# 1275468127/Medical-SAM2

Measured on AMD Instinct MI355X. Metric: slices/sec @1024^2 (Hiera-S), higher is better.
Workload: dtype bf16; 1 GPU; configs[1]: sam2_hiera_s 2D (train_2d SAM2 sub-sequence, forward), b=4 x 1024x1024 per GPU, 16-entry memory bank with 4 sampled memories per slice, one click per slice; forward_image -> memory_attention -> prompt encoder -> mask decoder -> memory encoder; hip_graph=True, weights=random name-keyed init

## Files before the change

### include/msam2_hip.h

```cpp
#ifndef MSAM2_HIP_H
#define MSAM2_HIP_H

#include <stddef.h>
#include <stdint.h>

#ifdef __cplusplus
extern "C" {
#endif

const char* msam2_last_error(void);

int msam2_version(void);

int msam2_operand_is_fp16(void);

int msam2_graph_begin(void* stream);

int msam2_graph_end(void* stream, void** graph_exec_out);

int msam2_graph_launch(void* graph_exec, void* stream);

int msam2_graph_destroy(void* graph_exec);

int msam2_event_create(void** ev);

int msam2_event_record(void* ev, void* stream);

int msam2_event_elapsed_ms(void* start, void* stop, float* ms);

int msam2_event_destroy(void* ev);

int msam2_gemm_nt(const void* A, int64_t lda, const void* B, int64_t ldb, const float* bias, const void* residual, int64_t ldr, void* C, int64_t ldc, int out_is_16bit, int64_t M, int64_t N, int64_t K, void* stream);

int msam2_gemm(const void* A, int64_t lda, const void* W, int64_t ldw, const float* bias, const float* colscale, const void* residual, int64_t ldr, int res_is_16bit, int64_t res_mod, void* C, int64_t ldc, int out_is_16bit, int64_t M, int64_t N, int64_t K, int act, void* stream);

int msam2_gemm_tokens(const float* A, int64_t lda, const float* A2, int64_t add_cols, const void* W, int64_t ldw, const float* bias, const float* residual, int64_t ldr, void* C, int64_t ldc, int out_is_16bit, int64_t M, int64_t N, int64_t K, int act, void* stream);

int msam2_gemm_pool2x2(const void* A, int64_t lda, const void* W, int64_t ldw, const float* bias, float* C, int64_t ldc, int64_t B, int64_t H, int64_t Wimg, int64_t N, int64_t K, void* stream);

int msam2_gemm_qkv_pool2x2(const void* A, int64_t lda, const void* W, int64_t ldw, const float* bias, void* QKV, int64_t ldc, void* Q2, int64_t ldq, int64_t B, int64_t H, int64_t Wimg, int64_t N, int64_t K, int64_t q_cols, void* stream);

int msam2_gemm_rope(const void* A, int64_t lda, const void* W, int64_t ldw, const float* bias, void* C, int64_t ldc, int64_t M, int64_t N, int64_t K, const float* rope_cos, const float* rope_sin, int64_t rope_cols, int64_t head_dim, int64_t rows_per_batch, int64_t n_rope, int64_t n_pos, void* stream);

size_t msam2_attention_workspace_bytes(int64_t Bz, int64_t H, int64_t Lq, int64_t D, int splits);

int msam2_attention_merge(void* o, const int64_t* o_strides, int64_t B, int64_t H, int64_t Lq, int64_t Lk, int64_t D, int splits, void* workspace, size_t workspace_bytes, void* stream);

int msam2_attention_fwd(const void* q, const int64_t* q_strides, const void* k, const int64_t* k_strides, const void* v, const int64_t* v_strides, void* o, const int64_t* o_strides, int64_t B, int64_t H, int64_t Lq, int64_t Lk, int64_t D, float scale, int splits, void* workspace, size_t workspace_bytes, void* stream);

int msam2_attention_fwd_lse(const void* q, const int64_t* q_strides, const void* k, const int64_t* k_strides, const void* v, const int64_t* v_strides, void* o, const int64_t* o_strides, int64_t B, int64_t H, int64_t Lq, int64_t Lk, int64_t D, float scale, int splits, void* workspace, size_t workspace_bytes, float* lse, void* stream);

int msam2_attention_fwd_lse_dropout(const void* q, const int64_t* q_strides, const void* k, const int64_t* k_strides, const void* v, const int64_t* v_strides, void* o, const int64_t* o_strides, int64_t B, int64_t H, int64_t Lq, int64_t Lk, int64_t D, float scale, int splits, void* workspace, size_t workspace_bytes, float* lse, float p, uint64_t seed, uint64_t offset, const void* seed_dev, void* stream);

int msam2_attention_kv64_fwd(const void* q, const int64_t* q_strides, const void* k, const int64_t* k_strides, const void* v, const int64_t* v_strides, void* o, const int64_t* o_strides, int64_t B, int64_t H, int64_t Lq, int64_t Lk, float scale, int splits, void* workspace, size_t workspace_bytes, void* stream);

int msam2_attention_effective_splits(int64_t Lk, int splits);

int msam2_attention_kv64_partial(const void* q, const int64_t* q_strides, const void* k, const int64_t* k_strides, const void* v, const int64_t* v_strides, int64_t B, int64_t H, int64_t Lq, int64_t Lk, float scale, int splits, int split_begin, int split_count, void* workspace, size_t workspace_bytes, void* stream);

int msam2_attention_kv64_dyn_fwd(const void* q, const int64_t* q_strides, const void* k, const int64_t* k_strides, const void* v, const int64_t* v_strides, void* o, const int64_t* o_strides, int64_t B, int64_t H, int64_t Lq, int64_t Lk, const void* key_count_dev, float scale, int splits, void* workspace, size_t workspace_bytes, void* stream);

int msam2_attention_kv64_dyn_partial(const void* q, const int64_t* q_strides, const void* k, const int64_t* k_strides, const void* v, const int64_t* v_strides, int64_t B, int64_t H, int64_t Lq, int64_t Lk, const void* key_count_dev, float scale, int splits, int split_begin, int split_count, void* workspace, size_t workspace_bytes, void* stream);

int msam2_window_attention_fwd(const void* q, int64_t q_token_stride, int64_t q_head_stride, int64_t hq, int64_t wq, int64_t ws_q, const void* k, const void* v, int64_t kv_token_stride, int64_t kv_head_stride, int64_t hk, int64_t wk, int64_t ws_k, const float* kpad, const float* vpad, void* o, int64_t o_token_stride, int64_t o_head_stride, int64_t B, int64_t H, int64_t D, float scale, void* stream);

int msam2_attention_small_fwd(const void* q, int64_t q_bs, int64_t q_ts, const void* k, int64_t k_bs, int64_t k_ts, const void* v, int64_t v_bs, int64_t v_ts, void* o, int64_t o_bs, int64_t o_ts, int64_t B, int64_t H, int64_t Lq, int64_t Lk, int64_t D, float scale, void* stream);

size_t msam2_attention_bwd_workspace_bytes(int64_t B, int64_t H, int64_t Lq, int64_t D);

int msam2_attention_bwd(const void* q, const int64_t* q_strides, const void* k, const int64_t* k_strides, const void* v, const int64_t* v_strides, const void* o, const int64_t* o_strides, const float* lse, const float* d_o, const int64_t* do_strides, float* dq, const int64_t* dq_strides, float* dk, const int64_t* dk_strides, float* dv, const int64_t* dv_strides, void* workspace, size_t workspace_bytes, int64_t B, int64_t H, int64_t Lq, int64_t Lk, int64_t D, float scale, void* stream);

int msam2_attention_bwd_dropout(const void* q, const int64_t* q_strides, const void* k, const int64_t* k_strides, const void* v, const int64_t* v_strides, const void* o, const int64_t* o_strides, const float* lse, const float* d_o, const int64_t* do_strides, float* dq, const int64_t* dq_strides, float* dk, const int64_t* dk_strides, float* dv, const int64_t* dv_strides, void* workspace, size_t workspace_bytes, int64_t B, int64_t H, int64_t Lq, int64_t Lk, int64_t D, float scale, float p, uint64_t seed, uint64_t offset, const void* seed_dev, void* stream);

int msam2_layernorm(const void* x, int in_is_16bit, int64_t ldx, const float* weight, const float* bias, void* y, int out_is_16bit, int64_t ldy, int64_t rows, int64_t C, float eps, int act, void* stream);

int msam2_layernorm_dual(const float* x, int64_t ldx, const float* weight, const float* bias, float* y, int64_t ldy, void* y16, int64_t ldy16, int64_t rows, int64_t C, float eps, void* stream);

int msam2_add_cast(const void* a, int a_is_16bit, int64_t a_s0, int64_t a_s1, const void* b, int b_is_16bit, int64_t b_s0, int64_t b_s1, float alpha, void* out, int out_is_16bit, int64_t D0, int64_t D1, int64_t C, void* stream);

int msam2_maxpool2x2(const void* x, int in_is_16bit, int64_t ldx, void* y, int out_is_16bit, int64_t ldy, int64_t B, int64_t H, int64_t W, int64_t C, void* stream);

int msam2_upsample2x_add(void* y, const void* top, int64_t B, int64_t H, int64_t W, int64_t C, void* stream);

int msam2_rope_table(float* cos_out, float* sin_out, int64_t side, int64_t D, float theta, void* stream);

int msam2_rope_inplace(void* x, int64_t batch_stride, int64_t ld, int64_t B, int64_t L, int64_t n_rope, int64_t n_pos, int64_t D, const float* cos_t, const float* sin_t, void* stream);

int msam2_bilinear_upsample(const float* x, float* y, int64_t planes, int64_t h, int64_t w, int64_t H, int64_t W, void* stream);

int msam2_sine_pos_2d(float* out, int64_t h, int64_t w, int64_t C, float temperature, void* stream);

int msam2_fourier_pe_grid(float* out, const float* gauss, int64_t h, int64_t w, int64_t C, void* stream);

int msam2_hiera_pos_embed(float* out, const float* pos_embed, const float* pos_embed_window, int64_t C, int64_t bh, int64_t bw, int64_t h, int64_t w, int64_t window, void* stream);

int msam2_aa_downsample(const float* x, float* y, int64_t planes, int64_t H, int64_t W, int64_t factor, float in_scale, float in_bias, void* stream);

int msam2_gate_rows(float* x, const float* score, float value, int64_t B, int64_t row_len, void* stream);

int msam2_any_positive(const float* x, float* out, int64_t B, int64_t row_len, void* stream);

int msam2_image_prep(const uint8_t* img_hwc, float* out_chw, int64_t H, int64_t W, int64_t S, const float* mean3, const float* std3, void* stream);

int msam2_non_overlap(const float* masks, float* out, int64_t n_obj, int64_t pixels, void* stream);

int msam2_seg_counts(const float* pred, const float* gt, const float* thresholds, int64_t n_thresholds, int64_t planes, int64_t pixels, int* counts, void* stream);

int msam2_im2col_patch7x7s4(const float* img, void* out, int64_t B, int64_t S, void* stream);

int msam2_patch_embed7x7s4(const float* img, const void* w_perm, const float* bias, const float* pos, float* out, int64_t B, int64_t S, int64_t E, void* stream);

int msam2_im2col3x3s2(const void* x, void* out, int64_t B, int64_t H, int64_t W, int64_t C, int64_t ld, void* stream);

int msam2_conv3x3s2_ln_gelu(const void* x, int in_is_16bit, const float* weight, const float* bias, const float* ln_w, const float* ln_b, void* y, int64_t B, int64_t H, int64_t W, int64_t Cin, int64_t Cout, int mask_mode, float mask_scale, float mask_bias, void* stream);

int msam2_dwconv7x7_ln(const float* x, const float* weight_tap_major, const float* bias, const float* ln_w, const float* ln_b, void* y, int64_t B, int64_t H, int64_t W, int64_t C, void* stream);

int msam2_convt2x2_shuffle(const void* gemm_out, const float* bias, const void* skip, const float* ln_w, const float* ln_b, void* y, int64_t B, int64_t h, int64_t w, int64_t C, void* stream);

int msam2_convt2x2_shuffle_f32skip(const void* gemm_out, const float* bias, const float* skip, const float* ln_w, const float* ln_b, void* y, int64_t B, int64_t h, int64_t w, int64_t C, void* stream);

int msam2_convt2x2_shuffle_shared(const void* gemm_out, const float* bias, const void* skip, int skip_is_16bit, const float* ln_w, const float* ln_b, void* y, int64_t B, int64_t h, int64_t w, int64_t C, int64_t skip_batch_stride, void* stream);

int msam2_hyper_masks(const float* hyper, const void* upscaled, float* masks, int64_t n, int64_t K, int64_t P, int64_t C, void* stream);

int msam2_prompt_points(const float* xy, const int* labels, const float* gauss, const float* point_emb, const float* not_a_point, float* out, int64_t n_points, int64_t C, float image_size, void* stream);

int msam2_prompt_points_padded(const float* xy, const int* labels, const float* gauss, const float* point_emb, const float* not_a_point, float* out, int64_t n_sets, int64_t P, int64_t n_pad, int64_t C, float image_size, void* stream);

int msam2_select_mask(const float* masks, const float* ious, const float* obj_scores, float* low_res, int* sel, float* iou_sel, int64_t n, int64_t P, int multimask, int dynamic_stability, float delta, float thresh, void* stream);

int msam2_gather_rows(const float* x, const int* sel, float* y, int64_t n, int64_t T, int64_t C, int64_t offset, void* stream);

int msam2_obj_ptr_mix(float* ptr, const float* obj_scores, const float* no_obj_ptr, int64_t n, int64_t C, void* stream);

int msam2_space_to_depth(const void* x, int in_is_16bit, void* out, int64_t B, int64_t H, int64_t W, int64_t C, int64_t k, int64_t ld, void* stream);

int msam2_token_mlp3(const float* hs, int64_t hs_batch_stride, int64_t hs_token_stride, const int* token_index, const void* w1, const float* b1, const void* w2, const float* b2, const void* w3, const float* b3, const int* out_dim, const int* sigmoid_flag, float* out, int64_t G, int64_t B, int64_t C, void* stream);

int msam2_token_mlp3_packed(const float* hs, int64_t hs_batch_stride, int64_t hs_token_stride, const int* token_index, const void* w1, const float* b1, const void* w2, const float* b2, const void* w3, const float* b3, const int* out_dim, const int* sigmoid_flag, float* out, const int* out_offset, const int* out_stride, int64_t G, int64_t B, int64_t C, void* stream);

size_t msam2_cc_workspace_bytes(int64_t N, int64_t H, int64_t W);

int msam2_cc_label(const uint8_t* img, int32_t* labels, int32_t* counts, int64_t N, int64_t H, int64_t W, void* workspace, size_t workspace_bytes, void* stream);

size_t msam2_fill_holes_workspace_bytes(int64_t N, int64_t H, int64_t W);

int msam2_fill_components(float* mask, int64_t N, int64_t H, int64_t W, int max_area, float threshold, int above, float fill_value, void* workspace, size_t workspace_bytes, void* stream);

int msam2_fill_holes(float* mask, int64_t N, int64_t H, int64_t W, int max_area, void* workspace, size_t workspace_bytes, void* stream);

int msam2_transpose16(const void* in, int64_t ldi, void* out, int64_t ldo, int64_t rows, int64_t cols, void* stream);

int msam2_gemm_tt(const void* A, int64_t lda, const void* B, int64_t ldb, float* C, int64_t ldc, float* a_colsum, int64_t M, int64_t N, int64_t K, void* stream);

int msam2_gemm_tt_acc(const void* A, int64_t lda, const void* B, int64_t ldb, float* C, int64_t ldc, float* a_colsum, int64_t M, int64_t N, int64_t K, void* stream);

int msam2_colsum(const void* x, int x_is_16bit, int64_t ldx, float* out, int64_t rows, int64_t cols, void* stream);

int msam2_act_bwd(const void* pre, int pre_is_16bit, const void* dy, int dy_is_16bit, void* out, int64_t n, int act, void* stream);

int msam2_layernorm_bwd(const float* x, int64_t ldx, const void* dy, int dy_is_16bit, int64_t ldd, const float* gamma, float* dx, int64_t ldo, float* dgamma, float* dbeta, int64_t rows, int64_t C, float eps, const float* add, int64_t ld_add, void* stream);

int msam2_softmax_rows(const float* s, int64_t ld_s, void* p, int64_t ld_p, int64_t rows, int64_t cols, float scale, void* stream);

int msam2_softmax_bwd_rows(const void* p, int64_t ld_p, const float* dp, int64_t ld_dp, void* ds, int64_t ld_ds, int64_t rows, int64_t cols, float scale, void* stream);

int msam2_convt2x2_gather(const void* gemm_out, const float* bias, const void* skip, float* z, int64_t B, int64_t h, int64_t w, int64_t C, void* stream);

int msam2_convt2x2_scatter_grad(const void* dz, int dz_is_16bit, void* dg, int64_t B, int64_t h, int64_t w, int64_t C, void* stream);

int msam2_dwconv7x7(const float* x, const float* w_tap_major, const float* bias, float* y, int64_t B, int64_t H, int64_t W, int64_t C, int flip, void* stream);

int msam2_dwconv7x7_wgrad(const float* x, const float* dy, float* dw_tap_major, int64_t B, int64_t H, int64_t W, int64_t C, void* stream);

int msam2_col2im3x3s2(const float* dcols, int64_t ld, float* dx, int64_t B, int64_t H, int64_t W, int64_t C, void* stream);

int msam2_bilinear_upsample_bwd(const float* dy, float* dx, int64_t planes, int64_t h, int64_t w, int64_t H, int64_t W, void* stream);

int msam2_bce_logits(const float* logits, const float* target, float* dlogits, float* loss, int64_t n, float pos_weight, void* stream);

int msam2_adam_step(float* param, const float* grad, float* exp_avg, float* exp_avg_sq, int64_t n, float lr, float beta1, float beta2, float eps, int64_t step, void* stream);

int msam2_adam_step_multi(void* const* params, const void* const* grads, void* const* exp_avg, void* const* exp_avg_sq, const int64_t* numel, int64_t count, float lr, float beta1, float beta2, float eps, int64_t step, float grad_scale, float weight_decay, void* step_counter, void* skipped_counter, void* stream);

int msam2_attention_small_bwd(const void* q, int64_t q_bs, int64_t q_ts, const void* k, int64_t k_bs, int64_t k_ts, const void* v, int64_t v_bs, int64_t v_ts, const float* d_o, float* dq, float* dk, float* dv, int64_t B, int64_t H, int64_t Lq, int64_t Lk, int64_t D, float scale, void* stream);

int msam2_maxpool2x2_bwd(const void* x, int x_is_16bit, int64_t ldx, const float* dy, int64_t lddy, float* dx, int64_t lddx, int64_t B, int64_t H, int64_t W, int64_t C, void* stream);

int msam2_window_move(void* img, int64_t ld_img, void* win, const void* fill, int64_t B, int64_t H, int64_t W, int64_t heads, int64_t D, int64_t ws, int elem_bytes, int to_windows, void* stream);

int msam2_window_unpartition_cvt(void* img16, int64_t ld_img, const float* win, int64_t B, int64_t H, int64_t W, int64_t heads, int64_t D, int64_t ws, void* stream);

int msam2_window_pad_colsum(const float* win, float* out, int64_t B, int64_t H, int64_t W, int64_t heads, int64_t D, int64_t ws, void* stream);

int msam2_sumpool2x2(const float* dy, float* out, int64_t B, int64_t H, int64_t W, int64_t C, void* stream);

size_t msam2_hiera_pos_embed_bwd_workspace_bytes(int64_t C, int64_t bw, int64_t h, int64_t window);

int msam2_hiera_pos_embed_bwd(const float* d_table, float* d_pos_embed, float* d_pos_embed_window, int64_t C, int64_t bh, int64_t bw, int64_t h, int64_t w, int64_t window, void* workspace, size_t workspace_bytes, void* stream);

int msam2_dropout(const void* x, int x_is_16bit, int64_t ldx, const float* residual, int64_t ldr, void* y, int y_is_16bit, int64_t ldy, int64_t rows, int64_t cols, float p, uint64_t seed, uint64_t offset, const void* seed_dev, void* stream);

int msam2_counter_bump(void* counter_u64, void* snapshot_u64, void* stream);

int msam2_mlp_fused_permute_w2(const void* w2, void* w2p, int64_t dim, int64_t hidden, void* stream);

int msam2_ln_mlp_residual_supported(int64_t dim);

int msam2_ln_mlp_residual_fwd(const float* x, int64_t T, int64_t dim, const float* ln_w, const float* ln_b, float eps, const void* w1, const float* b1, const void* w2p, const float* b2, float* out, void* stream);

int msam2_ln_mlp_residual_fwd_dual(const float* x, int64_t T, int64_t dim, const float* ln_w, const float* ln_b, float eps, const void* w1, const float* b1, const void* w2p, const float* b2, float* out, void* out16, void* stream);

size_t msam2_mask_stats_workspace_bytes(int64_t M);

int msam2_mask_stats(const float* logits, int64_t M, int64_t lh, int64_t lw, int64_t h, int64_t w, float thr, float thr_hi, float thr_lo, int* counts, int* boxes, void* workspace, size_t workspace_bytes, void* stream);

int msam2_mask_rle_runs(const float* logits, int64_t M, int64_t lh, int64_t lw, int64_t h, int64_t w, int64_t x0, int64_t y0, int64_t H, int64_t W, float thr, int* runs, void* stream);

int msam2_mask_rle(const float* logits, int64_t M, int64_t lh, int64_t lw, int64_t h, int64_t w, int64_t x0, int64_t y0, int64_t H, int64_t W, float thr, const int64_t* offsets, int* counts, void* stream);

size_t msam2_box_nms_workspace_bytes(int64_t K);

int msam2_box_nms(const float* boxes, const float* scores, int64_t K, float iou_thr, int64_t* keep, int* n_keep, void* workspace, size_t workspace_bytes, void* stream);

int msam2_bank_dots_chain(int64_t K, int vec);

size_t msam2_bank_dots_workspace_bytes(int64_t R, int64_t Cn);

int msam2_bank_dots(const float* x, const int64_t* x_strides, int64_t R, const float* ya, const int64_t* ya_strides, int64_t rows_a, const float* yb, const int64_t* yb_strides, int64_t rows_b, int64_t n_ch, int64_t n_px, float* dots, float* xx, float* yy, void* workspace, size_t workspace_bytes, void* stream);

// ... 37 lines not shown
```

### medical-sam2_amd/_lib.py

```python
from __future__ import annotations

import ctypes
import os
import subprocess

_HERE = os.path.dirname(os.path.abspath(__file__))
LIB_PATH = os.environ.get("MSAM2_LIB_PATH") or os.path.join(_HERE, "libmsam2_hip.so")

c_p = ctypes.c_void_p
c_i = ctypes.c_int
c_l = ctypes.c_int64
c_f = ctypes.c_float
c_z = ctypes.c_size_t
c_d = ctypes.c_double

SIGNATURES = {
    "msam2_version": (c_i, []),
    "msam2_last_error": (ctypes.c_char_p, []),
    "msam2_operand_is_fp16": (c_i, []),
    "msam2_gemm": (c_i, [c_p, c_l, c_p, c_l, c_p, c_p, c_p, c_l, c_i, c_l, c_p, c_l, c_i, c_l, c_l, c_l, c_i, c_p]),
    "msam2_gemm_pool2x2": (c_i, [c_p, c_l, c_p, c_l, c_p, c_p, c_l, c_l, c_l, c_l, c_l, c_l, c_p]),
    "msam2_gemm_qkv_pool2x2": (c_i, [c_p, c_l, c_p, c_l, c_p, c_p, c_l, c_p, c_l, c_l, c_l, c_l, c_l, c_l, c_l, c_p]),
    "msam2_gemm_tokens": (c_i, [c_p, c_l, c_p, c_l, c_p, c_l, c_p, c_p, c_l, c_p, c_l, c_i, c_l, c_l, c_l, c_i, c_p]),
    "msam2_gemm_rope": (c_i, [c_p, c_l, c_p, c_l, c_p, c_p, c_l, c_l, c_l, c_l, c_p, c_p, c_l, c_l, c_l, c_l, c_l, c_p]),
    "msam2_ln_mlp_residual_supported": (c_i, [c_l]),
    "msam2_mlp_fused_permute_w2": (c_i, [c_p, c_p, c_l, c_l, c_p]),
    "msam2_ln_mlp_residual_fwd": (c_i, [c_p, c_l, c_l, c_p, c_p, c_f, c_p, c_p, c_p, c_p, c_p, c_p]),
    "msam2_ln_mlp_residual_fwd_dual": (c_i, [c_p, c_l, c_l, c_p, c_p, c_f, c_p, c_p, c_p, c_p, c_p, c_p, c_p]),
    "msam2_layernorm": (c_i, [c_p, c_i, c_l, c_p, c_p, c_p, c_i, c_l, c_l, c_l, c_f, c_i, c_p]),
    "msam2_layernorm_dual": (c_i, [c_p, c_l, c_p, c_p, c_p, c_l, c_p, c_l, c_l, c_l, c_f, c_p]),
    "msam2_attention_workspace_bytes": (c_z, [c_l, c_l, c_l, c_l, c_i]),
    "msam2_attention_fwd": (c_i, [c_p, c_p, c_p, c_p, c_p, c_p, c_p, c_p, c_l, c_l, c_l, c_l, c_l, c_f, c_i, c_p, c_z, c_p]),
    "msam2_attention_fwd_lse": (c_i, [c_p, c_p, c_p, c_p, c_p, c_p, c_p, c_p, c_l, c_l, c_l, c_l, c_l, c_f, c_i, c_p, c_z, c_p, c_p]),
    "msam2_attention_fwd_lse_dropout": (c_i, [c_p, c_p, c_p, c_p, c_p, c_p, c_p, c_p, c_l, c_l, c_l, c_l, c_l, c_f, c_i, c_p, c_z, c_p, c_f,
                                              ctypes.c_uint64, ctypes.c_uint64, c_p, c_p]),
    "msam2_attention_kv64_fwd": (c_i, [c_p, c_p, c_p, c_p, c_p, c_p, c_p, c_p, c_l, c_l, c_l, c_l, c_f, c_i, c_p, c_z, c_p]),
    "msam2_attention_kv64_partial": (c_i, [c_p, c_p, c_p, c_p, c_p, c_p, c_l, c_l, c_l, c_l, c_f, c_i, c_i, c_i, c_p, c_z, c_p]),
    "msam2_attention_kv64_dyn_fwd": (c_i, [c_p, c_p, c_p, c_p, c_p, c_p, c_p, c_p, c_l, c_l, c_l, c_l, c_p, c_f, c_i, c_p, c_z, c_p]),
    "msam2_attention_kv64_dyn_partial": (c_i, [c_p, c_p, c_p, c_p, c_p, c_p, c_l, c_l, c_l, c_l, c_p, c_f, c_i, c_i, c_i, c_p, c_z, c_p]),
    "msam2_attention_effective_splits": (c_i, [c_l, c_i]),
    "msam2_attention_merge": (c_i, [c_p, c_p, c_l, c_l, c_l, c_l, c_l, c_i, c_p, c_z, c_p]),
    "msam2_window_attention_fwd": (c_i, [c_p, c_l, c_l, c_l, c_l, c_l, c_p, c_p, c_l, c_l, c_l, c_l, c_l, c_p, c_p, c_p, c_l, c_l,
                                         c_l, c_l, c_l, c_f, c_p]),
    "msam2_attention_small_fwd": (c_i, [c_p, c_l, c_l, c_p, c_l, c_l, c_p, c_l, c_l, c_p, c_l, c_l, c_l, c_l, c_l, c_l, c_l, c_f,
                                        c_p]),
    "msam2_add_cast": (c_i, [c_p, c_i, c_l, c_l, c_p, c_i, c_l, c_l, c_f, c_p, c_i, c_l, c_l, c_l, c_p]),
    "msam2_maxpool2x2": (c_i, [c_p, c_i, c_l, c_p, c_i, c_l, c_l, c_l, c_l, c_l, c_p]),
    "msam2_upsample2x_add": (c_i, [c_p, c_p, c_l, c_l, c_l, c_l, c_p]),
    "msam2_rope_table": (c_i, [c_p, c_p, c_l, c_l, c_f, c_p]),
    "msam2_rope_inplace": (c_i, [c_p, c_l, c_l, c_l, c_l, c_l, c_l, c_l, c_p, c_p, c_p]),
    "msam2_bilinear_upsample": (c_i, [c_p, c_p, c_l, c_l, c_l, c_l, c_l, c_p]),
    "msam2_sine_pos_2d": (c_i, [c_p, c_l, c_l, c_l, c_f, c_p]),
    "msam2_fourier_pe_grid": (c_i, [c_p, c_p, c_l, c_l, c_l, c_p]),
    "msam2_hiera_pos_embed": (c_i, [c_p, c_p, c_p, c_l, c_l, c_l, c_l, c_l, c_l, c_p]),
    "msam2_im2col_patch7x7s4": (c_i, [c_p, c_p, c_l, c_l, c_p]),
    "msam2_patch_embed7x7s4": (c_i, [c_p, c_p, c_p, c_p, c_p, c_l, c_l, c_l, c_p]),
    "msam2_im2col3x3s2": (c_i, [c_p, c_p, c_l, c_l, c_l, c_l, c_l, c_p]),
    "msam2_conv3x3s2_ln_gelu": (c_i, [c_p, c_i, c_p, c_p, c_p, c_p, c_p, c_l, c_l, c_l, c_l, c_l, c_i, c_f, c_f, c_p]),
    "msam2_dwconv7x7_ln": (c_i, [c_p, c_p, c_p, c_p, c_p, c_p, c_l, c_l, c_l, c_l, c_p]),
    "msam2_convt2x2_shuffle": (c_i, [c_p, c_p, c_p, c_p, c_p, c_p, c_l, c_l, c_l, c_l, c_p]),
    "msam2_convt2x2_shuffle_f32skip": (c_i, [c_p, c_p, c_p, c_p, c_p, c_p, c_l, c_l, c_l, c_l, c_p]),
    "msam2_space_to_depth": (c_i, [c_p, c_i, c_p, c_l, c_l, c_l, c_l, c_l, c_l, c_p]),
    "msam2_aa_downsample": (c_i, [c_p, c_p, c_l, c_l, c_l, c_l, c_f, c_f, c_p]),
    "msam2_gate_rows": (c_i, [c_p, c_p, c_f, c_l, c_l, c_p]),
    "msam2_any_positive": (c_i, [c_p, c_p, c_l, c_l, c_p]),
    "msam2_transpose16": (c_i, [c_p, c_l, c_p, c_l, c_l, c_l, c_p]),
    "msam2_colsum": (c_i, [c_p, c_i, c_l, c_p, c_l, c_l, c_p]),
    "msam2_act_bwd": (c_i, [c_p, c_i, c_p, c_i, c_p, c_l, c_i, c_p]),
    "msam2_layernorm_bwd": (c_i, [c_p, c_l, c_p, c_i, c_l, c_p, c_p, c_l, c_p, c_p, c_l, c_l, c_f, c_p, c_l, c_p]),
    "msam2_softmax_rows": (c_i, [c_p, c_l, c_p, c_l, c_l, c_l, c_f, c_p]),
    "msam2_softmax_bwd_rows": (c_i, [c_p, c_l, c_p, c_l, c_p, c_l, c_l, c_l, c_f, c_p]),
    "msam2_convt2x2_gather": (c_i, [c_p, c_p, c_p, c_p, c_l, c_l, c_l, c_l, c_p]),
    "msam2_convt2x2_scatter_grad": (c_i, [c_p, c_i, c_p, c_l, c_l, c_l, c_l, c_p]),
    "msam2_bce_logits": (c_i, [c_p, c_p, c_p, c_p, c_l, c_f, c_p]),
    "msam2_attention_bwd_workspace_bytes": (c_z, [c_l, c_l, c_l, c_l]),
    "msam2_attention_bwd": (c_i, [c_p, c_p, c_p, c_p, c_p, c_p, c_p, c_p, c_p, c_p, c_p, c_p, c_p, c_p, c_p, c_p, c_p, c_p, c_z,
                                  c_l, c_l, c_l, c_l, c_l, c_f, c_p]),
    "msam2_attention_bwd_dropout": (c_i, [c_p, c_p, c_p, c_p, c_p, c_p, c_p, c_p, c_p, c_p, c_p, c_p, c_p, c_p, c_p, c_p, c_p, c_p, c_z,
                                          c_l, c_l, c_l, c_l, c_l, c_f, c_f, ctypes.c_uint64, ctypes.c_uint64, c_p, c_p]),
    "msam2_dwconv7x7": (c_i, [c_p, c_p, c_p, c_p, c_l, c_l, c_l, c_l, c_i, c_p]),
    "msam2_dwconv7x7_wgrad": (c_i, [c_p, c_p, c_p, c_l, c_l, c_l, c_l, c_p]),
    "msam2_col2im3x3s2": (c_i, [c_p, c_l, c_p, c_l, c_l, c_l, c_l, c_p]),
    "msam2_gemm_nt": (c_i, [c_p, c_l, c_p, c_l, c_p, c_p, c_l, c_p, c_l, c_i, c_l, c_l, c_l, c_p]),
    "msam2_gemm_tt": (c_i, [c_p, c_l, c_p, c_l, c_p, c_l, c_p, c_l, c_l, c_l, c_p]),
    "msam2_window_unpartition_cvt": (c_i, [c_p, c_l, c_p, c_l, c_l, c_l, c_l, c_l, c_l, c_p]),
    "msam2_window_pad_colsum": (c_i, [c_p, c_p, c_l, c_l, c_l, c_l, c_l, c_l, c_p]),
    "msam2_gemm_tt_acc": (c_i, [c_p, c_l, c_p, c_l, c_p, c_l, c_p, c_l, c_l, c_l, c_p]),
    "msam2_bilinear_upsample_bwd": (c_i, [c_p, c_p, c_l, c_l, c_l, c_l, c_l, c_p]),
    "msam2_maxpool2x2_bwd": (c_i, [c_p, c_i, c_l, c_p, c_l, c_p, c_l, c_l, c_l, c_l, c_l, c_p]),
    "msam2_window_move": (c_i, [c_p, c_l, c_p, c_p, c_l, c_l, c_l, c_l, c_l, c_l, c_i, c_i, c_p]),
    "msam2_sumpool2x2": (c_i, [c_p, c_p, c_l, c_l, c_l, c_l, c_p]),
    "msam2_hiera_pos_embed_bwd": (c_i, [c_p, c_p, c_p, c_l, c_l, c_l, c_l, c_l, c_l, c_p, c_z, c_p]),
    "msam2_hiera_pos_embed_bwd_workspace_bytes": (c_z, [c_l, c_l, c_l, c_l]),
    "msam2_dropout": (c_i, [c_p, c_i, c_l, c_p, c_l, c_p, c_i, c_l, c_l, c_l, c_f, ctypes.c_uint64, ctypes.c_uint64, c_p, c_p]),
    "msam2_counter_bump": (c_i, [c_p, c_p, c_p]),
    "msam2_adam_step": (c_i, [c_p, c_p, c_p, c_p, c_l, c_f, c_f, c_f, c_f, c_l, c_p]),
    "msam2_adam_step_multi": (c_i, [c_p, c_p, c_p, c_p, c_p, c_l, c_f, c_f, c_f, c_f, c_l, c_f, c_f, c_p, c_p, c_p]),
    "msam2_attention_small_bwd": (c_i, [c_p, c_l, c_l, c_p, c_l, c_l, c_p, c_l, c_l, c_p, c_p, c_p, c_p, c_l, c_l, c_l, c_l, c_l, c_f, c_p]),
    "msam2_seg_counts": (c_i, [c_p, c_p, c_p, c_l, c_l, c_l, c_p, c_p]),
    "msam2_non_overlap": (c_i, [c_p, c_p, c_l, c_l, c_p]),
    "msam2_token_mlp3": (c_i, [c_p, c_l, c_l, c_p, c_p, c_p, c_p, c_p, c_p, c_p, c_p, c_p, c_p, c_l, c_l, c_l, c_p]),
    "msam2_hyper_masks": (c_i, [c_p, c_p, c_p, c_l, c_l, c_l, c_l, c_p]),
    "msam2_prompt_points": (c_i, [c_p, c_p, c_p, c_p, c_p, c_p, c_l, c_l, c_f, c_p]),
    "msam2_prompt_points_padded": (c_i, [c_p, c_p, c_p, c_p, c_p, c_p, c_l, c_l, c_l, c_l, c_f, c_p]),
    "msam2_token_mlp3_packed": (c_i, [c_p, c_l, c_l, c_p, c_p, c_p, c_p, c_p, c_p, c_p, c_p, c_p, c_p, c_p, c_p, c_l, c_l, c_l, c_p]),
    "msam2_select_mask": (c_i, [c_p, c_p, c_p, c_p, c_p, c_p, c_l, c_l, c_i, c_i, c_f, c_f, c_p]),
    "msam2_gather_rows": (c_i, [c_p, c_p, c_p, c_l, c_l, c_l, c_l, c_p]),
    "msam2_obj_ptr_mix": (c_i, [c_p, c_p, c_p, c_l, c_l, c_p]),
    "msam2_convt2x2_shuffle_shared": (c_i, [c_p, c_p, c_p, c_i, c_p, c_p, c_p, c_l, c_l, c_l, c_l, c_l, c_p]),
    "msam2_mask_stats_workspace_bytes": (c_z, [c_l]),
    "msam2_mask_stats": (c_i, [c_p, c_l, c_l, c_l, c_l, c_l, c_f, c_f, c_f, c_p, c_p, c_p, c_z, c_p]),
    "msam2_mask_rle_runs": (c_i, [c_p, c_l, c_l, c_l, c_l, c_l, c_l, c_l, c_l, c_l, c_f, c_p, c_p]),
    "msam2_mask_rle": (c_i, [c_p, c_l, c_l, c_l, c_l, c_l, c_l, c_l, c_l, c_l, c_f, c_p, c_p, c_p]),
    "msam2_box_nms_workspace_bytes": (c_z, [c_l]),
    "msam2_box_nms": (c_i, [c_p, c_p, c_l, c_f, c_p, c_p, c_p, c_z, c_p]),
    "msam2_bank_dots_chain": (c_i, [c_l, c_i]),
    "msam2_bank_dots_workspace_bytes": (c_z, [c_l, c_l]),
    "msam2_bank_dots": (c_i, [c_p, c_p, c_l, c_p, c_p, c_l, c_p, c_p, c_l, c_l, c_l, c_p, c_p, c_p, c_p, c_z, c_p]),
    "msam2_bank_sample": (c_i, [c_p, c_l, c_p, c_p, c_p, c_l, c_l, c_p, c_l, c_l, c_p, c_p, c_p]),
    "msam2_bank_gather": (c_i, [c_p, c_p, c_p, c_p, c_l, c_l, c_l, c_l, c_l, c_l, c_p, c_p, c_p]),
    "msam2_bank_decide": (c_i, [c_p, c_p, c_p, c_l, c_l, c_p, c_p, c_l, c_l, c_i, c_p, c_p, c_p, c_p]),
    "msam2_bank_commit": (c_i, [c_p, c_l, c_p, c_p, c_p, c_p, c_l, c_p, c_p, c_l, c_l, c_l, c_p, c_p, c_p, c_p]),
    "msam2_label_slices": (c_i, [c_p, c_p, c_l, c_l, c_l, c_l, c_l, c_l, c_f, c_p, c_l, c_p, c_i, c_p, c_p, c_p]),
    "msam2_label_stats": (c_i, [c_p, c_p, c_l, c_l, c_l, c_l, c_p, c_p, c_p]),
    "msam2_label_pick": (c_i, [c_p, c_p, c_p, c_p, c_p, c_p, c_l, c_l, c_l, c_l, c_p, c_p]),
    "msam2_label_components_workspace_bytes": (c_z, [c_l, c_l, c_l]),
    "msam2_label_components": (c_i, [c_p, c_l, c_l, c_l, c_i, c_p, c_p, c_p, c_z, c_p]),
    "msam2_label_clean_workspace_bytes": (c_z, [c_l]),
    "msam2_label_clean": (c_i, [c_p, c_p, c_p, c_p, c_l, c_p, ctypes.c_uint32, c_p, c_p, c_p, c_z, c_l, c_l, c_l, c_p]),
    "msam2_label_overlap": (c_i, [c_p, c_p, c_p, c_l, c_l, c_l, c_l, c_p, c_p]),
    "msam2_label_edt_workspace_bytes": (c_z, [c_l, c_l, c_l]),
    "msam2_label_edt": (c_i, [c_p, c_l, c_l, c_l, c_i, c_i, c_p, c_d, c_d, c_d, c_p, c_p, c_z, c_p]),
    "msam2_label_surface_distances_workspace_bytes": (c_z, [c_p, c_l]),
    "msam2_label_surface_distances": (c_i, [c_p, c_p, c_l, c_l, c_l, c_p, c_p, c_p, c_p, c_l, c_d, c_d, c_d, c_p, c_l, c_p, c_p, c_z, c_p]),
    "msam2_cc_workspace_bytes": (c_z, [c_l, c_l, c_l]),
    "msam2_cc_label": (c_i, [c_p, c_p, c_p, c_l, c_l, c_l, c_p, c_z, c_p]),
    "msam2_fill_holes_workspace_bytes": (c_z, [c_l, c_l, c_l]),
    "msam2_fill_holes": (c_i, [c_p, c_l, c_l, c_l, c_i, c_p, c_z, c_p]),
    "msam2_fill_components": (c_i, [c_p, c_l, c_l, c_l, c_i, c_f, c_i, c_f, c_p, c_z, c_p]),
    "msam2_image_prep": (c_i, [c_p, c_p, c_l, c_l, c_l, ctypes.POINTER(c_f), ctypes.POINTER(c_f), c_p]),
    "msam2_graph_begin": (c_i, [c_p]),
    "msam2_graph_end": (c_i, [c_p, ctypes.POINTER(c_p)]),
    "msam2_graph_launch": (c_i, [c_p, c_p]),
    "msam2_graph_destroy": (c_i, [c_p]),
    "msam2_event_create": (c_i, [ctypes.POINTER(c_p)]),
    "msam2_event_record": (c_i, [c_p, c_p]),
    "msam2_event_elapsed_ms": (c_i, [c_p, c_p, ctypes.POINTER(c_f)]),
    "msam2_event_destroy": (c_i, [c_p]),
}


def build(force: bool = False) -> str:
    if force and os.path.exists(LIB_PATH):
        os.remove(LIB_PATH)
    subprocess.check_call(["make", "-s", "-C", os.path.join(_HERE, "csrc")])
    return LIB_PATH


_lib = None


def lib() -> ctypes.CDLL:
    global _lib
    if _lib is None:
        if not os.path.exists(LIB_PATH):
            raise RuntimeError(
                f"{LIB_PATH} is missing: the MI355X HIP library is the only compute path of this package. "
                "Build it with `python -c 'import __graft_entry__ as g; g.build()'` (or `make -C medical-sam2_amd/csrc`).")
        L = ctypes.CDLL(LIB_PATH)
        for name, (res, args) in SIGNATURES.items():
            fn = getattr(L, name)
            fn.restype = res
            fn.argtypes = args
        _lib = L
    return _lib


class Msam2Error(RuntimeError):
    pass


def check(rc: int) -> None:
    if rc != 0:
        raise Msam2Error(lib().msam2_last_error().decode())
```

### medical-sam2_amd/csrc/elementwise.hip

```cpp
#include "common.h"
#include <type_traits>

template <typename T>
struct Vec4 {};
template <>
struct Vec4<float> {
  typedef f32x4 type;
};
template <>
struct Vec4<op16> {
  typedef op16x4 type;
};

template <typename TI, typename TO, int CHUNKS>
__global__ void layernorm_kernel(const TI* __restrict__ x, int64_t ldx, const float* __restrict__ w, const float* __restrict__ b,
                                 TO* __restrict__ y, int64_t ldy, int64_t rows, int C, float eps, int act, op16* __restrict__ y2 = nullptr,
                                 int64_t ldy2 = 0) {
  typedef typename Vec4<TI>::type VI;
  typedef typename Vec4<TO>::type VO;
  const int64_t row = (((int64_t)blockIdx.x * blockDim.x + threadIdx.x) >> 4);
  const int l16 = threadIdx.x & 15;
  const bool live = row < rows;
  const int nch = C >> 2;
  const TI* xr = x + (live ? row : 0) * ldx;
// ... 71 lines not shown
}

template <typename TI, typename TO>
__global__ void layernorm_scalar_kernel(const TI* __restrict__ x, int64_t ldx, const float* __restrict__ w,
                                        const float* __restrict__ b, TO* __restrict__ y, int64_t ldy, int64_t rows, int C,
                                        float eps, int act) {
  const int64_t row = ((int64_t)blockIdx.x * blockDim.x + threadIdx.x) >> 6;
  const int lane = threadIdx.x & 63;
  if (row >= rows) return;
  const TI* xr = x + row * ldx;
  float v[16];
  float s = 0.f;
#pragma unroll
  for (int i = 0; i < 16; ++i) {
    const int c = lane + i * 64;
    v[i] = (c < C) ? (float)xr[c] : 0.f;
    s += v[i];
  }
  const float mean = wave_sum(s) / C;
  float q = 0.f;
#pragma unroll
  for (int i = 0; i < 16; ++i) {
    const int c = lane + i * 64;
    const float d = (c < C) ? v[i] - mean : 0.f;
    q += d * d;
  }
  const float rstd = 1.0f / sqrtf(wave_sum(q) / C + eps);
  TO* yr = y + row * ldy;
#pragma unroll
  for (int i = 0; i < 16; ++i) {
    const int c = lane + i * 64;
    if (c < C) {
      float o = (v[i] - mean) * rstd * w[c] + b[c];
      if (act == 1) o = gelu_erf_as(o);
      yr[c] = f2out<TO>(o);
    }
  }
}

template <typename TI, typename TO>
static void layernorm_vec_launch(const TI* x, int64_t ldx, const float* w, const float* b, TO* y, int64_t ldy, int64_t rows, int C, float eps, int act,
                                 op16* y2, int64_t ldy2, hipStream_t s) {
  const dim3 grid(cdiv(rows * 16, 256)), block(256);
  const int chunks = (C / 4 + 15) / 16;
  auto launch = [&](auto ch) {
    hipLaunchKernelGGL((layernorm_kernel<TI, TO, decltype(ch)::value>), grid, block, 0, s, x, ldx, w, b, y, ldy, rows, C, eps, act, y2, ldy2);
  };
  if (chunks <= 2) launch(std::integral_constant<int, 2>{});
  else if (chunks <= 4) launch(std::integral_constant<int, 4>{});
  else if (chunks <= 6) launch(std::integral_constant<int, 6>{});
  else if (chunks <= 12) launch(std::integral_constant<int, 12>{});
  else launch(std::integral_constant<int, 16>{});
}

extern "C" int msam2_layernorm(const void* x, int in_is_16bit, int64_t ldx, const float* weight, const float* bias, void* y,
                               int out_is_16bit, int64_t ldy, int64_t rows, int64_t C, float eps, int act, void* stream) {
  MSAM2_REQUIRE(x && y && weight && bias, "layernorm: null tensor");
  MSAM2_REQUIRE(rows > 0 && C > 0 && C <= 1024, "layernorm: rows=%lld C=%lld unsupported (C<=1024)", (long long)rows, (long long)C);
  hipStream_t s = (hipStream_t)stream;
  const bool vec = (C % 4 == 0) && vec_ok(4, in_is_16bit ? 2 : 4, ldx, x) && vec_ok(4, out_is_16bit ? 2 : 4, ldy, y) && vec_ok(4, 4, weight, bias);
  with_type(in_is_16bit, [&](auto ti) {
    with_type(out_is_16bit, [&](auto to) {
      using TI = decltype(ti);
      using TO = decltype(to);
      if (vec) {
        layernorm_vec_launch((const TI*)x, ldx, weight, bias, (TO*)y, ldy, rows, (int)C, eps, act, nullptr, 0, s);
      } else {
        hipLaunchKernelGGL((layernorm_scalar_kernel<TI, TO>), dim3(cdiv(rows * 64, 256)), dim3(256), 0, s, (const TI*)x, ldx, weight, bias, (TO*)y, ldy,
                           rows, (int)C, eps, act);
      }
    });
  });
  return msam2_check_launch("layernorm");
}

extern "C" int msam2_layernorm_dual(const float* x, int64_t ldx, const float* weight, const float* bias, float* y, int64_t ldy, void* y16,
                                    int64_t ldy16, int64_t rows, int64_t C, float eps, void* stream) {
  MSAM2_REQUIRE(x && y && y16 && weight && bias, "layernorm_dual: null tensor");
  MSAM2_REQUIRE(rows > 0 && C > 0 && C <= 1024 && C % 4 == 0 && vec_ok(4, 4, ldx, ldy) && vec_ok(4, 2, ldy16),
                "layernorm_dual: rows=%lld C=%lld unsupported (C <= 1024, multiples of 4)", (long long)rows, (long long)C);
  MSAM2_REQUIRE(vec_ok(4, 4, x, y, weight, bias) && vec_ok(4, 2, y16), "layernorm_dual: alignment");
  layernorm_vec_launch(x, ldx, weight, bias, y, ldy, rows, (int)C, eps, 0, (op16*)y16, ldy16, (hipStream_t)stream);
  return msam2_check_launch("layernorm_dual");
}

template <typename TA, typename TB, typename TO>
__global__ void add_cast_kernel(const TA* __restrict__ a, int64_t a_s0, int64_t a_s1, const TB* __restrict__ b, int64_t b_s0,
                                int64_t b_s1, float alpha, TO* __restrict__ out, int64_t D0, int64_t D1, int C) {
  const int64_t total = D0 * D1 * C;
  for (int64_t i = (int64_t)blockIdx.x * blockDim.x + threadIdx.x; i < total; i += (int64_t)gridDim.x * blockDim.x) {
    const int c = i % C;
    const int64_t rj = i / C;
    const int64_t j = rj % D1, r = rj / D1;
    float v = (float)a[r * a_s0 + j * a_s1 + c];
    if (b) v += alpha * (float)b[r * b_s0 + j * b_s1 + c];
    out[i] = f2out<TO>(v);
  }
}

template <typename TA, typename TB, typename TO>
__global__ void add_cast_vec_kernel(const TA* __restrict__ a, int64_t a_s0, int64_t a_s1, const TB* __restrict__ b, int64_t b_s0,
                                    int64_t b_s1, float alpha, TO* __restrict__ out, unsigned D0, unsigned D1, unsigned C4) {
  typedef typename Vec4<TA>::type VA;
  typedef typename Vec4<TB>::type VB;
  typedef typename Vec4<TO>::type VO;
  const unsigned rows = D0 * D1;
  const unsigned total = rows * C4;
  for (unsigned i = blockIdx.x * blockDim.x + threadIdx.x; i < total; i += gridDim.x * blockDim.x) {
    const unsigned g = i % C4, rj = i / C4;
    const unsigned j = rj % D1, r = rj / D1;
    const VA va = *reinterpret_cast<const VA*>(a + r * a_s0 + j * a_s1 + g * 4);
    float v[4];
#pragma unroll
    for (int e = 0; e < 4; ++e) v[e] = (float)va[e];
    if (b) {
      const VB vb = *reinterpret_cast<const VB*>(b + r * b_s0 + j * b_s1 + g * 4);
#pragma unroll
      for (int e = 0; e < 4; ++e) v[e] += alpha * (float)vb[e];
    }
    VO o;
#pragma unroll
    for (int e = 0; e < 4; ++e) o[e] = f2out<TO>(v[e]);
    *reinterpret_cast<VO*>(out + (int64_t)i * 4) = o;
  }
}

extern "C" int msam2_add_cast(const void* a, int a_is_16bit, int64_t a_s0, int64_t a_s1, const void* b, int b_is_16bit, int64_t b_s0,
                              int64_t b_s1, float alpha, void* out, int out_is_16bit, int64_t D0, int64_t D1, int64_t C,
                              void* stream) {
  MSAM2_REQUIRE(a && out, "add_cast: null tensor");
  MSAM2_REQUIRE(D0 > 0 && D1 > 0 && C > 0, "add_cast: empty volume");
  const int64_t total = D0 * D1 * C;
  hipStream_t s = (hipStream_t)stream;
  const bool vec = (C % 4 == 0) && total / 4 < (1ll << 31) && vec_ok(4, a_is_16bit ? 2 : 4, a_s0, a_s1, a) && vec_ok(4, out_is_16bit ? 2 : 4, out) &&
                   (!b || vec_ok(4, b_is_16bit ? 2 : 4, b_s0, b_s1, b));
  with_type(a_is_16bit, [&](auto ta) {
    with_type(b_is_16bit, [&](auto tb) {
      with_type(out_is_16bit, [&](auto to) {
        using TA = decltype(ta);
        using TB = decltype(tb);
        using TO = decltype(to);
        if (vec)
          hipLaunchKernelGGL((add_cast_vec_kernel<TA, TB, TO>), dim3(grid1d(total / 4, 16384)), dim3(256), 0, s, (const TA*)a, a_s0, a_s1, (const TB*)b,
                             b_s0, b_s1, alpha, (TO*)out, (unsigned)D0, (unsigned)D1, (unsigned)(C / 4));
        else
          hipLaunchKernelGGL((add_cast_kernel<TA, TB, TO>), dim3(grid1d(total, 8192)), dim3(256), 0, s, (const TA*)a, a_s0, a_s1, (const TB*)b, b_s0,
                             b_s1, alpha, (TO*)out, D0, D1, (int)C);
      });
    });
  });
  return msam2_check_launch("add_cast");
}

template <typename TI, typename TO>
__global__ void maxpool2x2_kernel(const TI* __restrict__ x, int64_t ldx, TO* __restrict__ y, int64_t ldy, int B, int H, int W,
                                  int C) {
  const int Ho = H / 2, Wo = W / 2;
  const int64_t total = (int64_t)B * Ho * Wo * C;
  for (int64_t i = (int64_t)blockIdx.x * blockDim.x + threadIdx.x; i < total; i += (int64_t)gridDim.x * blockDim.x) {
    const int c = i % C;
    int64_t t = i / C;
    const int xo = t % Wo;
    t /= Wo;
    const int yo = t % Ho;
    const int b = t / Ho;
    const int64_t base = ((int64_t)b * H + 2 * yo) * W + 2 * xo;
    const float v0 = (float)x[base * ldx + c], v1 = (float)x[(base + 1) * ldx + c];
    const float v2 = (float)x[(base + W) * ldx + c], v3 = (float)x[(base + W + 1) * ldx + c];
    y[(((int64_t)b * Ho + yo) * Wo + xo) * ldy + c] = f2out<TO>(fmaxf(fmaxf(v0, v1), fmaxf(v2, v3)));
  }
}

extern "C" int msam2_maxpool2x2(const void* x, int in_is_16bit, int64_t ldx, void* y, int out_is_16bit, int64_t ldy, int64_t B,
                                int64_t H, int64_t W, int64_t C, void* stream) {
  MSAM2_REQUIRE(x && y, "maxpool2x2: null tensor");
  MSAM2_REQUIRE(B > 0 && C > 0 && H > 0 && W > 0 && H % 2 == 0 && W % 2 == 0, "maxpool2x2: H, W must be even");
  const int64_t total = B * (H / 2) * (W / 2) * C;
  with_type(in_is_16bit, [&](auto ti) {
    with_type(out_is_16bit, [&](auto to) {
      using TI = decltype(ti);
      using TO = decltype(to);
      hipLaunchKernelGGL((maxpool2x2_kernel<TI, TO>), dim3(grid1d(total, 8192)), dim3(256), 0, (hipStream_t)stream, (const TI*)x, ldx, (TO*)y, ldy, (int)B,
                         (int)H, (int)W, (int)C);
    });
  });
  return msam2_check_launch("maxpool2x2");
}

__global__ void upsample2x_add_kernel(float* __restrict__ y, const float* __restrict__ top, int B, int H, int W, int C) {
  const int64_t total = (int64_t)B * H * W * C;
  for (int64_t i = (int64_t)blockIdx.x * blockDim.x + threadIdx.x; i < total; i += (int64_t)gridDim.x * blockDim.x) {
    const int c = i % C;
    int64_t t = i / C;
    const int xx = t % W;
    t /= W;
    const int yy = t % H;
    const int b = t / H;
    y[i] += top[(((int64_t)b * (H / 2) + yy / 2) * (W / 2) + xx / 2) * C + c];
  }
}

__global__ void upsample2x_add4_kernel(float* __restrict__ y, const float* __restrict__ top, unsigned B, unsigned H, unsigned W, unsigned C4) {
  const unsigned total = B * H * W * C4;
  for (unsigned i = blockIdx.x * blockDim.x + threadIdx.x; i < total; i += gridDim.x * blockDim.x) {
    const unsigned t0 = i / C4, c = i - t0 * C4;
    const unsigned t1 = t0 / W, xx = t0 - t1 * W;
    const unsigned b = t1 / H, yy = t1 - b * H;
    const f32x4 a = *reinterpret_cast<const f32x4*>(y + (int64_t)i * 4);
    const f32x4 tp = *reinterpret_cast<const f32x4*>(top + ((int64_t)(b * (H / 2) + yy / 2) * (W / 2) + xx / 2) * (C4 * 4) + c * 4);
    *reinterpret_cast<f32x4*>(y + (int64_t)i * 4) = a + tp;
  }
}

extern "C" int msam2_upsample2x_add(void* y, const void* top, int64_t B, int64_t H, int64_t W, int64_t C, void* stream) {
  MSAM2_REQUIRE(y && top, "upsample2x_add: null tensor");
  MSAM2_REQUIRE(H % 2 == 0 && W % 2 == 0 && B > 0 && C > 0, "upsample2x_add: bad shape");
  const int64_t total = B * H * W * C;
  if (C % 4 == 0 && total / 4 < (1ll << 31) && vec_ok(4, 4, y, top)) {
    hipLaunchKernelGGL(upsample2x_add4_kernel, dim3(grid1d(total / 4, 16384)), dim3(256), 0, (hipStream_t)stream,
                       (float*)y, (const float*)top, (unsigned)B, (unsigned)H, (unsigned)W, (unsigned)(C / 4));
    return msam2_check_launch("upsample2x_add");
  }
  hipLaunchKernelGGL(upsample2x_add_kernel, dim3(grid1d(total, 8192)), dim3(256), 0,
                     (hipStream_t)stream, (float*)y, (const float*)top, (int)B, (int)H, (int)W, (int)C);
  return msam2_check_launch("upsample2x_add");
}

__global__ void rope_table_kernel(float* __restrict__ cs, float* __restrict__ sn, int side, int D, float theta) {
  const int n_pairs = D / 2, nq = D / 4;
  const int64_t total = (int64_t)side * side * n_pairs;
  for (int64_t i = (int64_t)blockIdx.x * blockDim.x + threadIdx.x; i < total; i += (int64_t)gridDim.x * blockDim.x) {
    const int pr = i % n_pairs;
    const int pos = i / n_pairs;
    const int f = pr % nq;
    const float freq = 1.0f / powf(theta, (float)(4 * f) / (float)D);
    const float t = (pr < nq) ? (float)(pos % side) : (float)(pos / side);
    const float ang = t * freq;
    cs[i] = cosf(ang);
    sn[i] = sinf(ang);
  }
}

extern "C" int msam2_rope_table(float* cos_out, float* sin_out, int64_t side, int64_t D, float theta, void* stream) {
  MSAM2_REQUIRE(cos_out && sin_out && side > 0 && D % 4 == 0, "rope_table: bad arguments");
  hipLaunchKernelGGL(rope_table_kernel, dim3(256), dim3(256), 0, (hipStream_t)stream, cos_out, sin_out, (int)side, (int)D, theta);
  return msam2_check_launch("rope_table");
}

__global__ void rope_inplace_kernel(op16* __restrict__ x, int64_t bs, int64_t ld, int B, int L, int n_rope, int n_pos, int D,
                                    const float* __restrict__ cs, const float* __restrict__ sn) {
  const int hp = D / 2;
  const int64_t total = (int64_t)B * n_rope * hp;
  for (int64_t i = (int64_t)blockIdx.x * blockDim.x + threadIdx.x; i < total; i += (int64_t)gridDim.x * blockDim.x) {
    const int pr = i % hp;
    int64_t t = i / hp;
    const int l = t % n_rope;
    const int b = t / n_rope;
    op16x2* px = reinterpret_cast<op16x2*>(x + b * bs + (int64_t)l * ld) + pr;
    const op16x2 v = *px;
    const float re = (float)v[0], im = (float)v[1];
    const int pos = l % n_pos;
    const float c = cs[(int64_t)pos * hp + pr], s = sn[(int64_t)pos * hp + pr];
    op16x2 o;
    o[0] = f2op(re * c - im * s);
    o[1] = f2op(re * s + im * c);
    *px = o;
  }
}

extern "C" int msam2_rope_inplace(void* x, int64_t batch_stride, int64_t ld, int64_t B, int64_t L, int64_t n_rope, int64_t n_pos,
                                  int64_t D, const float* cos_t, const float* sin_t, void* stream) {
  MSAM2_REQUIRE(x && cos_t && sin_t, "rope: null tensor");
  MSAM2_REQUIRE(D % 4 == 0 && ld % 2 == 0 && batch_stride % 2 == 0 && n_rope >= 0 && n_rope <= L && n_pos > 0, "rope: bad shape");
  if (n_rope == 0) return MSAM2_OK;
  const int64_t total = B * n_rope * (D / 2);
  hipLaunchKernelGGL(rope_inplace_kernel, dim3(grid1d(total, 8192)), dim3(256), 0,
                     (hipStream_t)stream, (op16*)x, batch_stride, ld, (int)B, (int)L, (int)n_rope, (int)n_pos, (int)D, cos_t, sin_t);
  return msam2_check_launch("rope_inplace");
}

__device__ __forceinline__ float bilerp(float p00, float p01, float p10, float p11, float lx, float ly) {
  const float top = __builtin_fmaf(lx, p01, (1.f - lx) * p00);
  const float bot = __builtin_fmaf(lx, p11, (1.f - lx) * p10);
  return __builtin_fmaf(1.f - ly, top, ly * bot);
}

__global__ void bilinear_kernel(const float* __restrict__ x, float* __restrict__ y, int P, int h, int w, int H, int W) {
  const float sy = (float)h / H, sx = (float)w / W;
  const int64_t total = (int64_t)P * H * W;
  for (int64_t i = (int64_t)blockIdx.x * blockDim.x + threadIdx.x; i < total; i += (int64_t)gridDim.x * blockDim.x) {
    const int X = i % W;
    int64_t t = i / W;
    const int Y = t % H;
    const int pl = t / H;
    float fy = fmaxf((Y + 0.5f) * sy - 0.5f, 0.f), fx = fmaxf((X + 0.5f) * sx - 0.5f, 0.f);
    const int y0 = (int)fy, x0 = (int)fx;
    const int y1 = min(y0 + 1, h - 1), x1 = min(x0 + 1, w - 1);
    const float ly = fy - y0, lx = fx - x0;
    const float* p = x + (int64_t)pl * h * w;
    y[i] = bilerp(p[y0 * w + x0], p[y0 * w + x1], p[y1 * w + x0], p[y1 * w + x1], lx, ly);
  }
}

__global__ void bilinear4_kernel(const float* __restrict__ x, float* __restrict__ y, int P, int h, int w, int H, int W) {
  const float sy = (float)h / H, sx = (float)w / W;
  const int W4 = W >> 2;
// ... 276 lines not shown
```

### medical-sam2_amd/csrc/gemm.hip

```cpp
#include "common.h"
#include <stdlib.h>

struct GemmParams {
  const op16* A;
  const op16* W;
  const float* bias;
  const float* colscale;
  const void* res;
  void* C;
  int64_t lda, ldw, ldr, ldc;
  int64_t res_mod;
  int M, N, K;
  int act;
  int res_is_16bit;
  int out_is_16bit;
  const float* rope_cos;
  const float* rope_sin;
  int rope_cols, rope_D, rope_period, rope_n, rope_npos;
  int pool_H, pool_W;
  void* Q2;
  int64_t ldq;
  int poolq_cols;
  const float* A32;
  const float* A2;
// ... 1392 lines not shown
        const int su = min(st + u, s1 - 1);
        a[u] = load_a(su);
        w[u] = *reinterpret_cast<const op16x8*>(wp + su * 16);
      }
#pragma unroll
      for (int u = 0; u < U; ++u)
        if (st + u < s1) acc = MSAM2_MFMA_32x32x16(a[u], w[u], acc, 0, 0, 0);
    }
  };
  if (per <= 4) run(std::integral_constant<int, 4>{});
  else run(std::integral_constant<int, 8>{});
#pragma unroll
  for (int e = 0; e < 16; ++e) part[wave][(e & 3) + 8 * (e >> 2) + 4 * h][r] = acc[e];
  int rowv[4], colv[4];
  float bv[4], cv[4], rv[4];
#pragma unroll
  for (int t = 0; t < 4; ++t) {
    const int idx = t * 256 + tid;
    rowv[t] = idx >> 5;
    colv[t] = idx & 31;
    bv[t] = 0.f; cv[t] = 1.f; rv[t] = 0.f;
  }
  if (p.bias) {
#pragma unroll
    for (int t = 0; t < 4; ++t) bv[t] = p.bias[min(n0 + colv[t], (int64_t)p.N - 1)];
  }
  if (p.colscale) {
#pragma unroll
    for (int t = 0; t < 4; ++t) cv[t] = p.colscale[min(n0 + colv[t], (int64_t)p.N - 1)];
  }
  if (p.res) {
    int64_t at[4];
#pragma unroll
    for (int t = 0; t < 4; ++t) {
      const int rc = min(rowv[t], p.M - 1);
      const int64_t rr = p.res_mod > 0 ? (int64_t)((unsigned)rc % (unsigned)p.res_mod) : rc;
      at[t] = rr * p.ldr + min(n0 + colv[t], (int64_t)p.N - 1);
    }
    if (p.res_is_16bit) {
#pragma unroll
      for (int t = 0; t < 4; ++t) rv[t] = op2f(reinterpret_cast<const op16*>(p.res)[at[t]]);
    } else {
#pragma unroll
      for (int t = 0; t < 4; ++t) rv[t] = reinterpret_cast<const float*>(p.res)[at[t]];
    }
  }
  __syncthreads();
#pragma unroll
  for (int t = 0; t < 4; ++t) {
    const int row = rowv[t], col = colv[t];
    const int64_t n = n0 + col;
    if (row < p.M && n < p.N) {
      float x = part[0][row][col] + part[1][row][col] + part[2][row][col] + part[3][row][col] + bv[t];
      if (p.act == 1) x = gelu_erf(x);
      else if (p.act == 2) x = fmaxf(x, 0.f);
      else if (p.act == 3) x = 1.f / (1.f + __expf(-x));
      x = x * cv[t] + rv[t];
      if (p.out_is_16bit) reinterpret_cast<op16*>(p.C)[(int64_t)row * p.ldc + n] = f2op(x);
      else reinterpret_cast<float*>(p.C)[(int64_t)row * p.ldc + n] = x;
    }
  }
}

template <int BM, int BN, int WM, int WN>
static void launch_gemm(const GemmParams& p, hipStream_t s) {
  dim3 grid(cdiv(p.N, BN), cdiv(p.M, BM));
  hipLaunchKernelGGL((gemm_kernel<BM, BN, WM, WN>), grid, dim3(WM * WN * 64), 0, s, p);
}

__global__ __launch_bounds__(256) void gemm_zero_kernel(float* __restrict__ C, int64_t ldc, int M, int N) {
  const int64_t total = (int64_t)M * N;
  for (int64_t i = (int64_t)blockIdx.x * 256 + threadIdx.x; i < total; i += (int64_t)gridDim.x * 256) C[(i / N) * ldc + i % N] = 0.f;
}

static int gemm_launch(const void* A, int64_t lda, const void* W, int64_t ldw, const float* bias, const float* colscale,
                       const void* residual, int64_t ldr, int res_is_16bit, int64_t res_mod, void* C, int64_t ldc, int out_is_16bit,
                       int64_t M, int64_t N, int64_t K, int act, void* stream, const float* rope_cos, const float* rope_sin,
                       int rope_cols, int rope_D, int rope_period, int rope_n, int rope_npos, int pool_H = 0, int pool_W = 0,
                       void* Q2 = nullptr, int64_t ldq = 0, int poolq_cols = 0) {
  MSAM2_REQUIRE(A && W && C, "gemm: null operand");
  MSAM2_REQUIRE(M > 0 && N > 0 && K > 0, "gemm: empty problem M=%lld N=%lld K=%lld", (long long)M, (long long)N, (long long)K);
  MSAM2_REQUIRE(K % 8 == 0 && lda % 8 == 0 && ldw % 8 == 0, "gemm: K, lda, ldw must be multiples of 8 (16-byte rows)");
  MSAM2_REQUIRE(((uintptr_t)A & 15) == 0 && ((uintptr_t)W & 15) == 0, "gemm: A and W must be 16-byte aligned");
  MSAM2_REQUIRE(M < (1ll << 31) && N < (1ll << 31), "gemm: M/N too large");
  MSAM2_REQUIRE(act >= 0 && act <= 3, "gemm: bad activation %d", act);
  GemmParams p;
  p.A = (const op16*)A; p.W = (const op16*)W; p.bias = bias; p.colscale = colscale; p.res = residual; p.C = C;
  p.lda = lda; p.ldw = ldw; p.ldr = ldr; p.ldc = ldc; p.res_mod = res_mod;
  p.M = (int)M; p.N = (int)N; p.K = (int)K; p.act = act; p.res_is_16bit = res_is_16bit; p.out_is_16bit = out_is_16bit;
  p.rope_cos = rope_cos; p.rope_sin = rope_sin; p.rope_cols = rope_cols; p.rope_D = rope_D; p.rope_period = rope_period;
  p.rope_n = rope_n; p.rope_npos = rope_npos;
  p.pool_H = pool_H; p.pool_W = pool_W;
  p.Q2 = Q2; p.ldq = ldq; p.poolq_cols = poolq_cols;
  p.A32 = nullptr; p.A2 = nullptr; p.add_cols = 0;
  p.ksplit_tiles = 0;
  {
    const char* e = getenv("MSAM2_NT_BYTES");
    const long long thr = e ? atoll(e) : (30ll << 20);
    const char* e32 = getenv("MSAM2_NT_BYTES_F32");
    const long long thr32 = e32 ? atoll(e32) : (1ll << 60);
    p.store_nt = out_is_16bit ? ((long long)M * N * 2 > thr) : ((long long)M * N * 4 > thr32);
  }
  hipStream_t s = (hipStream_t)stream;
  const char* force = getenv("MSAM2_GEMM_V1");
  const char* var = getenv("MSAM2_GEMM_VARIANT");
  const bool dma_ok = !(force && force[0] == '1') && M >= 256 && N >= 96 && (N % 128 == 0 || N >= 256 || N % 64 != 0 || K >= 192) &&
                      M * lda * 2 < (1ll << 31) && N * ldw * 2 < (1ll << 31);
  const int tiles = cdiv(p.N, 128) * cdiv(p.M, 128);
  if (!out_is_16bit && act == 0 && !colscale && !residual && !rope_cos && pool_W == 0 &&
      (int64_t)cdiv(p.M, 128) * cdiv(p.N, 128) <= 32 && K >= 4096 && !getenv("MSAM2_NO_SPLITK")) {
    const int nk_all = cdiv(p.K, GEMM_BK);
    int splits = (int)min((int64_t)64, (int64_t)(512 / (cdiv(p.M, 128) * cdiv(p.N, 128))));
    splits = max(1, min(splits, nk_all / 8));
    if (splits > 1) {
      p.ksplit_tiles = cdiv(nk_all, splits);
      hipLaunchKernelGGL(gemm_zero_kernel, dim3((unsigned)min((int64_t)1024, cdiv((int64_t)M * N, (int64_t)256))), dim3(256), 0, s, (float*)C, ldc,
                         (int)M, (int)N);
      dim3 grid(cdiv(p.N, 128), cdiv(p.M, 128), cdiv(nk_all, p.ksplit_tiles));
      hipLaunchKernelGGL((gemm_kernel<128, 128, 2, 2>), grid, dim3(256), 0, s, p);
      return msam2_check_launch("gemm(split-K)");
    }
  }
  {
    const char* ew = getenv("MSAM2_GEMM_WSTAT");
    const int wstat_mode = ew ? atoi(ew) : -1;
    const bool want = wstat_mode == 1 || wstat_mode == 2 || wstat_mode < 0 || (wstat_mode == 3 && (act == 0 || act == 2));
    if (want && !var && dma_ok && wstat_mode < 0 && gemm_try_wstat256(p, s)) return msam2_check_launch("gemm(w-stationary, 256 rows)");
    if (want && !var && dma_ok && gemm_try_wstat(p, s, wstat_mode == 2)) return msam2_check_launch("gemm(w-stationary)");
  }
  const int vv = var ? atoi(var) : (tiles <= 256 && K >= 1024 ? 8 : (K % 64 == 0 && K >= 384 ? 2 : 5));
  if (dma_ok && K % 32 == 0 && vv == 6) {
    hipLaunchKernelGGL((gemm_wide_kernel<256, 128, 3, 2>), dim3(cdiv(p.N, 128) * cdiv(p.M, 256)), dim3(256), 0, s, p);
  } else if (dma_ok && K % 32 == 0 && vv == 8) {
    hipLaunchKernelGGL((gemm_wide_kernel<128, 128, 3, 3>), dim3(tiles), dim3(256), 0, s, p);
  } else if (dma_ok && K % 32 == 0 && vv == 9) {
    hipLaunchKernelGGL((gemm_wide_kernel<256, 128, 2, 2>), dim3(cdiv(p.N, 128) * cdiv(p.M, 256)), dim3(256), 0, s, p);
  } else if (dma_ok && K % 32 == 0 && vv == 10) {
    hipLaunchKernelGGL((gemm_wide_kernel<128, 128, 2, 4>), dim3(tiles), dim3(256), 0, s, p);
  } else if (dma_ok && K % 32 == 0 && vv == 11) {
    hipLaunchKernelGGL((gemm_wide_kernel<128, 128, 4, 2>), dim3(tiles), dim3(256), 0, s, p);
  } else if (dma_ok && K % 64 == 0 && vv == 2) {
    hipLaunchKernelGGL(gemm_glds_kernel, dim3(tiles), dim3(256), 0, s, p);
  } else if (dma_ok && K % 32 == 0) {
    hipLaunchKernelGGL((gemm_glds32_kernel<2, 4>), dim3(tiles), dim3(256), 0, s, p);
  } else if (M <= 32 && K % 16 == 0) {
    hipLaunchKernelGGL((gemm_skinny_kernel<false>), dim3(cdiv(p.N, 32)), dim3(256), 0, s, p);
  } else if (M <= 32) launch_gemm<32, 128, 1, 4>(p, s);
  else if (N <= 32) launch_gemm<128, 32, 4, 1>(p, s);
  else if (N <= 64 || (N % 128 != 0 && N % 64 == 0 && N < 512)) launch_gemm<128, 64, 2, 2>(p, s);
  else launch_gemm<128, 128, 2, 2>(p, s);
  return msam2_check_launch("gemm");
}

__global__ __launch_bounds__(256, 2) void gemm_nt_kernel(GemmParams p) {
  constexpr int BM = 128, BN = 128, BK = 64, A_BYTES = BM * BK * 2, STAGE_BYTES = A_BYTES + BK * BN * 2;
  __shared__ __attribute__((aligned(1024))) unsigned char lds[2 * STAGE_BYTES];
  const int tid = threadIdx.x;
  const int wave = __builtin_amdgcn_readfirstlane(tid >> 6), lane = tid & 63;
  const int wm = wave >> 1, wn = wave & 1;
  const int r = lane & 31, h = lane >> 5, li = lane & 15;
  const int n_tiles_n = (p.N + BN - 1) / BN, n_tiles_m = (p.M + BM - 1) / BM;
  const int nwg = n_tiles_n * n_tiles_m;
  const int bid = xcd_tile_order(blockIdx.x, nwg);
  const int64_t m0 = (int64_t)(bid / n_tiles_n) * BM;
  const int n0 = (bid % n_tiles_n) * BN;

  const auto a_rsrc = raw_rsrc(p.A);
  const auto w_rsrc = raw_rsrc(p.W);
  unsigned offsA[4], offsW[4];
#pragma unroll
  for (int i = 0; i < 4; ++i) {
    const int row = Img128::piece_row(wave * 4 + i, lane), chunk = Img128::src_chunk(row, lane);
    offsA[i] = (unsigned)(min(m0 + row, (int64_t)p.M - 1) * p.lda * 2 + chunk * 16);
    const int krow = 4 * (4 * wave + i) + (lane >> 4);
    const int col = ((lane & 15) ^ ((krow & 3) << 2)) * 8;
    offsW[i] = (unsigned)(krow * p.ldw * 2 + (n0 + (n0 + col < p.N ? col : 0)) * 2);
  }
  auto issue_piece = [&](int kt, int stage, int i) {
    unsigned char* base = lds + stage * STAGE_BYTES + wave * 4096;
    if (i < 4)
      glds16(a_rsrc, base + i * 1024, offsA[i], (unsigned)kt * BK * 2);
    else
      glds16(w_rsrc, base + A_BYTES + (i - 4) * 1024, offsW[i - 4], (unsigned)kt * BK * (unsigned)p.ldw * 2u);
  };

  f32x16 acc[2][2];
  zero_acc(acc);

  int offA[2], swzA[2];
#pragma unroll
  for (int i = 0; i < 2; ++i) {
    const int ra = wm * 64 + i * 32 + r;
    offA[i] = ra * Img128::ROW_BYTES;
    swzA[i] = Img128::swz(ra);
  }
  const int vq = li >> 2, vp = li & 3, cgrp = (lane >> 4) & 1;
  const int t_row = (8 * h + vq) * 256 + ((vp & 1) << 3);
  const int t_sw = vq << 2, t_c0 = 2 * cgrp + (vp >> 1);
  auto bfrag = [&](const unsigned char* slab, int ks, int cb) -> op16x8 {
    return lds_read_tr16_pair(slab + t_row + (16 * ks) * 256 + (((cb * 4 + t_c0) ^ t_sw) << 4), 4 * 256);
  };

  const int nk = p.K / BK;
#pragma unroll
  for (int i = 0; i < 8; ++i) issue_piece(0, 0, i);
  for (int kt = 0; kt < nk; ++kt) {
    const int st = kt & 1;
    wait_vmcnt<0>();
    __builtin_amdgcn_s_barrier();
    const unsigned char* sa = lds + st * STAGE_BYTES;
    const unsigned char* sb = sa + A_BYTES;
    op16x8 af[4][2], bfr[4][2];
#pragma unroll
    for (int ks = 0; ks < 4; ++ks) {
      const int c = 2 * ks + h;
#pragma unroll
      for (int i = 0; i < 2; ++i) {
        af[ks][i] = *reinterpret_cast<const op16x8*>(sa + offA[i] + ((c ^ swzA[i]) << 4));
        bfr[ks][i] = bfrag(sb, ks, wn * 2 + i);
      }
    }
    __builtin_amdgcn_sched_barrier(0);
#pragma unroll
    for (int ks = 0; ks < 4; ++ks) {
#pragma unroll
      for (int i = 0; i < 2; ++i)
#pragma unroll
        for (int j = 0; j < 2; ++j) acc[i][j] = MSAM2_MFMA_32x32x16(af[ks][i], bfr[ks][j], acc[i][j], 0, 0, 0);
      if (kt + 1 < nk) {
        issue_piece(kt + 1, st ^ 1, 2 * ks);
        issue_piece(kt + 1, st ^ 1, 2 * ks + 1);
      }
      __builtin_amdgcn_sched_barrier(0);
    }
  }
  __builtin_amdgcn_s_barrier();
  gemm_epilogue<2, 2>(p, acc, reinterpret_cast<float*>(lds) + wave * 32 * 68, m0 + wm * 64, n0 + wn * 64, lane);
}

extern "C" int msam2_gemm_nt(const void* A, int64_t lda, const void* B, int64_t ldb, const float* bias, const void* residual, int64_t ldr,
                             void* C, int64_t ldc, int out_is_16bit, int64_t M, int64_t N, int64_t K, void* stream) {
  MSAM2_REQUIRE(A && B && C && M > 0 && N > 0 && K > 0, "gemm_nt: bad arguments");
  MSAM2_REQUIRE(K % 64 == 0 && N % 8 == 0 && lda % 8 == 0 && ldb % 8 == 0 && ((uintptr_t)A & 15) == 0 && ((uintptr_t)B & 15) == 0,
                "gemm_nt: K %% 64 == 0, N / lda / ldb multiples of 8 and 16-byte aligned operands");
  MSAM2_REQUIRE(M * lda * 2 < (1ll << 31) && K * ldb * 2 < (1ll << 31) && lda >= K && ldb >= N && ldc >= N, "gemm_nt: bad sizes");
  GemmParams p = {};
  p.A = (const op16*)A; p.W = (const op16*)B; p.bias = bias; p.res = residual; p.C = C;
  p.lda = lda; p.ldw = ldb; p.ldr = ldr; p.ldc = ldc;
  p.M = (int)M; p.N = (int)N; p.K = (int)K; p.out_is_16bit = out_is_16bit;
  p.rope_period = 1; p.rope_npos = 1;
  hipLaunchKernelGGL(gemm_nt_kernel, dim3((unsigned)(cdiv(N, 128) * cdiv(M, 128))), dim3(256), 0, (hipStream_t)stream, p);
  return msam2_check_launch("gemm_nt");
}

extern "C" int msam2_gemm(const void* A, int64_t lda, const void* W, int64_t ldw, const float* bias, const float* colscale,
                          const void* residual, int64_t ldr, int res_is_16bit, int64_t res_mod, void* C, int64_t ldc, int out_is_16bit,
                          int64_t M, int64_t N, int64_t K, int act, void* stream) {
  return gemm_launch(A, lda, W, ldw, bias, colscale, residual, ldr, res_is_16bit, res_mod, C, ldc, out_is_16bit, M, N, K, act, stream,
                     nullptr, nullptr, 0, 0, 1, 0, 1);
}

extern "C" int msam2_gemm_tokens(const float* A, int64_t lda, const float* A2, int64_t add_cols, const void* W, int64_t ldw,
                                 const float* bias, const float* residual, int64_t ldr, void* C, int64_t ldc, int out_is_16bit,
                                 int64_t M, int64_t N, int64_t K, int act, void* stream) {
  MSAM2_REQUIRE(A && W && C, "gemm_tokens: null operand");
  MSAM2_REQUIRE(M > 0 && M <= 32 && N > 0 && K > 0 && K % 16 == 0, "gemm_tokens: needs 1 <= M <= 32 rows and K %% 16 == 0");
  MSAM2_REQUIRE(lda % 4 == 0 && ((uintptr_t)A & 15) == 0 && (!A2 || ((uintptr_t)A2 & 15) == 0) && ldw % 8 == 0 && ((uintptr_t)W & 15) == 0,
                "gemm_tokens: 16-byte aligned rows");
  MSAM2_REQUIRE(add_cols >= 0 && (add_cols % 32 == 0 || add_cols >= N) && act >= 0 && act <= 3,
                "gemm_tokens: add_cols must be a multiple of 32 (or >= N: every column)");
  GemmParams p = {};
  p.A32 = A; p.A2 = A2; p.add_cols = (int)(add_cols > N ? N + 31 : add_cols); p.lda = lda;
  p.W = (const op16*)W; p.ldw = ldw; p.bias = bias; p.res = residual; p.ldr = ldr; p.C = C; p.ldc = ldc;
  p.M = (int)M; p.N = (int)N; p.K = (int)K; p.act = act; p.out_is_16bit = out_is_16bit;
  hipLaunchKernelGGL((gemm_skinny_kernel<true>), dim3(cdiv(p.N, 32)), dim3(256), 0, (hipStream_t)stream, p);
  return msam2_check_launch("gemm_tokens");
}

extern "C" int msam2_gemm_pool2x2(const void* A, int64_t lda, const void* W, int64_t ldw, const float* bias, float* C, int64_t ldc,
                                  int64_t B, int64_t H, int64_t Wimg, int64_t N, int64_t K, void* stream) {
  MSAM2_REQUIRE(B > 0 && H > 0 && Wimg > 0 && H % 2 == 0 && Wimg % 2 == 0, "gemm_pool2x2: H and W must be even");
  const int64_t M = B * H * Wimg;
  MSAM2_REQUIRE(M >= 256 && (M / 4) * ldc * 4 < (1ll << 31) && M * lda * 2 < (1ll << 31), "gemm_pool2x2: problem out of the 32-bit offset range");
  return gemm_launch(A, lda, W, ldw, bias, nullptr, nullptr, 0, 0, 0, C, ldc, 0, M, N, K, 0, stream, nullptr, nullptr, 0, 0, 1, 0, 1,
                     (int)H, (int)Wimg);
}

extern "C" int msam2_gemm_qkv_pool2x2(const void* A, int64_t lda, const void* W, int64_t ldw, const float* bias, void* QKV, int64_t ldc,
                                      void* Q2, int64_t ldq, int64_t B, int64_t H, int64_t Wimg, int64_t N, int64_t K, int64_t q_cols,
                                      void* stream) {
  MSAM2_REQUIRE(QKV && Q2, "gemm_qkv_pool2x2: null output");
  MSAM2_REQUIRE(B > 0 && H > 0 && Wimg > 0 && H % 2 == 0 && Wimg % 2 == 0, "gemm_qkv_pool2x2: H and W must be even");
  MSAM2_REQUIRE(q_cols > 0 && q_cols % 32 == 0 && q_cols <= N && N % 2 == 0 && ldc % 2 == 0 && ldq % 2 == 0 &&
                    ((uintptr_t)QKV & 3) == 0 && ((uintptr_t)Q2 & 3) == 0,
                "gemm_qkv_pool2x2: q_cols must be a multiple of 32; outputs 4-byte aligned with even strides");
  const int64_t M = B * H * Wimg;
  MSAM2_REQUIRE(M >= 256 && M * ldc * 2 < (1ll << 31) && M * lda * 2 < (1ll << 31), "gemm_qkv_pool2x2: problem out of the 32-bit offset range");
  return gemm_launch(A, lda, W, ldw, bias, nullptr, nullptr, 0, 0, 0, QKV, ldc, 1, M, N, K, 0, stream, nullptr, nullptr, 0, 0, 1, 0, 1,
                     (int)H, (int)Wimg, Q2, ldq, (int)q_cols);
}

extern "C" int msam2_gemm_rope(const void* A, int64_t lda, const void* W, int64_t ldw, const float* bias, void* C, int64_t ldc,
                               int64_t M, int64_t N, int64_t K, const float* rope_cos, const float* rope_sin, int64_t rope_cols,
                               int64_t head_dim, int64_t rows_per_batch, int64_t n_rope, int64_t n_pos, void* stream) {
  MSAM2_REQUIRE(rope_cos && rope_sin, "gemm_rope: null table");
  MSAM2_REQUIRE(head_dim > 0 && head_dim % 4 == 0 && rope_cols >= 0 && rope_cols <= N && rope_cols % head_dim == 0,
// ... 10 lines not shown
```

### medical-sam2_amd/modeling/memory.py

```python
from __future__ import annotations

import copy
import math
from typing import Optional, Tuple

import torch
import torch.nn as nn

from .. import ops
from .common import OP16, F32, WeightCache, attn_splits, nchw_view, to_bf16, tokens_of, v_f32, w_bf16
from .encoder import MLP


import os as _os
_FUSED_ROPE = _os.environ.get("MSAM2_NO_FUSED_ROPE") is None
_FOLD_V = _os.environ.get("MSAM2_NO_VALUE_FOLD") is None
_BATCH_K_PROJ = _os.environ.get("MSAM2_BATCHED_KPROJ") is not None


class LayerNorm2d(nn.Module):

    def __init__(self, num_channels: int, eps: float = 1e-6) -> None:
        super().__init__()
        self.weight = nn.Parameter(torch.ones(num_channels))
# ... 58 lines not shown
        self._tables = {}

    def table(self, n_q: int, device) -> Tuple[torch.Tensor, torch.Tensor]:
        side = int(round(math.sqrt(n_q)))
        assert side * side == n_q, "RoPE attention expects a square token grid"
        key = (side, str(device))
        if key not in self._tables:
            self._tables[key] = ops.rope_table(side, self.internal_dim // self.num_heads, float(self.rope_theta), device)
        return self._tables[key]

    def proj_rope(self, which: str, x_bf16: torch.Tensor, B: int, rows_per_batch: int, n_rope: int, tab, out: Optional[torch.Tensor] = None) -> torch.Tensor:
        lin = getattr(self, which + "_proj")
        w, b = w_bf16(self._wc, which + "w", lin.weight), v_f32(self._wc, which + "b", lin.bias)
        M = x_bf16.shape[0]
        if _FUSED_ROPE and M >= 256 and rows_per_batch >= 128 and tab[0].shape[0] >= 128 and n_rope > 0 and M * self.internal_dim * 4 < 2 ** 31:
            return ops.gemm_rope(x_bf16, w, b, tab, rope_cols=self.internal_dim, head_dim=self.internal_dim // self.num_heads,
                                 rows_per_batch=rows_per_batch, n_rope=n_rope, out=out).view(B, rows_per_batch, -1)
        y = ops.gemm(x_bf16, w, b, out=out).view(B, rows_per_batch, -1)
        ops.rope_(y, n_rope, tab)
        return y

    def proj_rope_key_range(self, mem_k: torch.Tensor, n_ptr_tokens: int, tab, valid_keys: int, eff: int, share: Tuple[int, int]) -> torch.Tensor:
        B, Nk, _ = mem_k.shape
        n_pos = tab[0].shape[0]
        tiles_total = -(-valid_keys // 32)
        tiles_per = -(-tiles_total // eff)
        k0 = min(share[0] * tiles_per * 32, valid_keys)
        k1 = min(share[1] * tiles_per * 32, valid_keys)
        r0, r1 = (k0 // n_pos) * n_pos, min(-(-k1 // n_pos) * n_pos, Nk)
        kk = torch.empty(B, Nk, self.internal_dim, dtype=OP16, device=mem_k.device)
        if r1 > r0:
            n_rope = max(0, min(Nk - n_ptr_tokens, r1) - r0)
            for b in range(B):
                self.proj_rope("k", mem_k[b, r0:r1], 1, r1 - r0, n_rope, tab, out=kk[b, r0:r1])
        return kk

    def folds_values(self) -> bool:
        return _FOLD_V and self.kv_in_dim == 64 and self.internal_dim == 256 and self.num_heads == 1

    def out_folded(self, o64: torch.Tensor, residual: Optional[torch.Tensor], out_dtype=F32) -> torch.Tensor:
        ps = [self.out_proj.weight, self.out_proj.bias, self.v_proj.weight, self.v_proj.bias]
        w = self._wc.get("ovw", ps, lambda: (self.out_proj.weight.detach().float() @ self.v_proj.weight.detach().float()).to(OP16).contiguous())
        b = self._wc.get("ovb", ps, lambda: (self.out_proj.weight.detach().float() @ self.v_proj.bias.detach().float()
                                             + self.out_proj.bias.detach().float()).contiguous())
        return ops.gemm(o64, w, b, residual=residual, out_dtype=out_dtype)

    def core_folded(self, q: torch.Tensor, k: torch.Tensor, mem_v: torch.Tensor, key_count: Optional[torch.Tensor] = None) -> torch.Tensor:
        from .. import parallel
        B, Lq, C = q.shape
        Lk = k.shape[1]
        q4, k4, v4 = (q.view(B, Lq, 1, C).permute(0, 2, 1, 3), k.view(B, Lk, 1, C).permute(0, 2, 1, 3),
                      mem_v.reshape(B, Lk, 1, 64).permute(0, 2, 1, 3))
        splits = attn_splits(B, 1, Lq, Lk)
        kvs = parallel.current_kv_split()
        eff = ops.attention_effective_splits(Lk, splits) if kvs is not None else 1
        if eff > 1:
            ws = ops.attention_workspace(B, 1, Lq, 64, eff, q.device)
            s0, s1 = kvs.share(eff)
            ops.attention_kv64_partial(q4, k4, v4, splits=eff, split_begin=s0, split_count=s1 - s0, workspace=ws, key_count=key_count)
            kvs.exchange(ws, eff, B * Lq)
            o = torch.empty(B, Lq, 1, 64, dtype=OP16, device=q.device).permute(0, 2, 1, 3)
            ops.attention_merge(o, Lk, eff, ws)
        else:
            o = ops.attention_kv64(q4, k4, v4, splits=splits, key_count=key_count)
        return o.permute(0, 2, 1, 3).reshape(B * Lq, 64)

    def forward(self, q: torch.Tensor, k: torch.Tensor, v: torch.Tensor, num_k_exclude_rope: int = 0) -> torch.Tensor:
        assert not (self.training and self.dropout_p > 0.0), "attention dropout (train mode) is outside the forward hot path"
        B, Lq, _ = q.shape
        Lk = k.shape[1]
        if Lq != Lk:
            assert self.rope_k_repeat
        flat = lambda t: to_bf16(t.reshape(-1, t.shape[-1]).contiguous())
        tab = self.table(Lq, q.device)
        qp = self.proj_rope("q", flat(q), B, Lq, Lq, tab)
        kp = self.proj_rope("k", flat(k), B, Lk, Lk - num_k_exclude_rope, tab)
        vp = self.proj("v", flat(v)).view(B, Lk, -1)
        return self.out(self.core(qp, kp, vp), None).view(B, Lq, -1)


class MemoryAttentionLayer(nn.Module):

    def __init__(self, activation: str, cross_attention: nn.Module, d_model: int, dim_feedforward: int, dropout: float,
                 pos_enc_at_attn: bool, pos_enc_at_cross_attn_keys: bool, pos_enc_at_cross_attn_queries: bool,
                 self_attention: nn.Module):
        super().__init__()
        assert activation == "relu" and not pos_enc_at_attn and pos_enc_at_cross_attn_keys and not pos_enc_at_cross_attn_queries, \
            "HIP path implements the YAML's layer wiring (relu; pos enc only on cross-attn keys)"
        self.d_model, self.dim_feedforward, self.dropout_value = d_model, dim_feedforward, dropout
        self.self_attn = self_attention
        self.cross_attn_image = cross_attention
        self.linear1 = nn.Linear(d_model, dim_feedforward)
        self.dropout = nn.Dropout(dropout)
        self.linear2 = nn.Linear(dim_feedforward, d_model)
        self.norm1, self.norm2, self.norm3 = nn.LayerNorm(d_model), nn.LayerNorm(d_model), nn.LayerNorm(d_model)
        self.dropout1, self.dropout2, self.dropout3 = nn.Dropout(dropout), nn.Dropout(dropout), nn.Dropout(dropout)
        self.activation_str = activation
        self.pos_enc_at_attn = pos_enc_at_attn
        self.pos_enc_at_cross_attn_queries = pos_enc_at_cross_attn_queries
        self.pos_enc_at_cross_attn_keys = pos_enc_at_cross_attn_keys
        self._wc = WeightCache()

    def _ln(self, name: str, x: torch.Tensor) -> torch.Tensor:
        n = getattr(self, name)
        return ops.layernorm(x, v_f32(self._wc, name + "w", n.weight), v_f32(self._wc, name + "b", n.bias), n.eps)

    def run(self, x: torch.Tensor, mem_k: torch.Tensor, mem_v: torch.Tensor, B: int, L: int, n_ptr_tokens: int,
            key_count: Optional[torch.Tensor] = None, kk: Optional[torch.Tensor] = None) -> torch.Tensor:
        wc, sa, ca = self._wc, self.self_attn, self.cross_attn_image
        C = self.d_model
        Nk = mem_k.shape[1]
        tab = sa.table(L, x.device)
        t = self._ln("norm1", x)
        w_qkv = w_bf16(wc, "sqkv", sa.q_proj.weight, sa.k_proj.weight, sa.v_proj.weight)
        b_qkv = v_f32(wc, "sqkvb", sa.q_proj.bias, sa.k_proj.bias, sa.v_proj.bias)
        fused_rope = _FUSED_ROPE and B * L >= 256 and L >= 128 and sa.num_heads == 1 and B * L * 3 * C * 4 < 2 ** 31
        if fused_rope:
            qkv = ops.gemm_rope(t, w_qkv, b_qkv, tab, rope_cols=2 * C, head_dim=C, rows_per_batch=L, n_rope=L).view(B, L, 3 * C)
        else:
            qkv = ops.gemm(t, w_qkv, b_qkv).view(B, L, 3 * C)
        q, k, v = qkv[:, :, :C], qkv[:, :, C:2 * C], qkv[:, :, 2 * C:]
        if not fused_rope:
            ops.rope_(q, L, tab)
            ops.rope_(k, L, tab)
        x = sa.out(sa.core(q, k, v), x)
        t = self._ln("norm2", x)
        q = ca.proj_rope("q", t, B, L, L, tab)
        from .. import parallel
        kvs = parallel.current_kv_split()
        eff = ops.attention_effective_splits(Nk, attn_splits(B, 1, L, Nk)) if (kvs is not None and ca.folds_values()) else 1
        valid = Nk if key_count is None else (kvs.host_key_count if kvs is not None else None)
        if kk is not None:
            pass
        elif eff > 1 and valid is not None and (Nk - n_ptr_tokens) % tab[0].shape[0] == 0:
            kk = ca.proj_rope_key_range(mem_k, n_ptr_tokens, tab, int(valid), eff, kvs.share(eff))
        else:
            kk = ca.proj_rope("k", mem_k.reshape(B * Nk, -1), B, Nk, Nk - n_ptr_tokens, tab)
        if ca.folds_values():
            x = ca.out_folded(ca.core_folded(q, kk, mem_v, key_count), x)
        else:
            if key_count is not None:
                raise RuntimeError("a padded memory bank (key_count) needs the value-folded cross-attention (MSAM2_NO_VALUE_FOLD is set)")
            vv = ca.proj("v", mem_v.reshape(B * Nk, -1)).view(B, Nk, C)
            x = ca.out(ca.core(q, kk, vv), x)
        t = self._ln("norm3", x)
        h = ops.gemm(t, w_bf16(wc, "f1", self.linear1.weight), v_f32(wc, "f1b", self.linear1.bias), act=ops.ACT_RELU)
        return ops.gemm(h, w_bf16(wc, "f2", self.linear2.weight), v_f32(wc, "f2b", self.linear2.bias), residual=x, out_dtype=F32)

    def forward(self, tgt, memory, pos: Optional[torch.Tensor] = None, query_pos: Optional[torch.Tensor] = None,
                num_k_exclude_rope: int = 0) -> torch.Tensor:
        assert not self.training or self.dropout_value == 0.0, \
            "train-mode dropout runs through MemoryAttention.forward / training.* (backward.memory_attention_forward_saved), not a bare layer"
        B, L, C = tgt.shape
        mem_k = ops.add_cast(memory, pos, 1.0, OP16)
        mem_v = ops.add_cast(memory, None, 1.0, OP16)
        x = ops.add_cast(tgt, None, 1.0, F32).reshape(B * L, C)
        return self.run(x, mem_k, mem_v, B, L, num_k_exclude_rope).view(B, L, C)


class MemoryAttention(nn.Module):

    def __init__(self, d_model: int, pos_enc_at_input: bool, layer: nn.Module, num_layers: int, batch_first: bool = True):
        super().__init__()
        assert batch_first
        self.d_model = d_model
        self.layers = nn.ModuleList([copy.deepcopy(layer) for _ in range(num_layers)])
        self.num_layers = num_layers
        self.norm = nn.LayerNorm(d_model)
        self.pos_enc_at_input = pos_enc_at_input
        self.batch_first = batch_first
        self._wc = WeightCache()
        self.dropout_seed = 0
        self._dropout_calls = 0
        self._drop_ctr = None
        self._drop_ctr_host = -1

    def next_dropout(self):
        p = float(self.layers[0].dropout_value) if len(self.layers) else 0.0
        if not self.training or p <= 0.0:
            return None
        dev = self.norm.weight.device
        if self._drop_ctr is None or self._drop_ctr.device != dev or self._drop_ctr_host != self._dropout_calls:
            if torch.cuda.is_current_stream_capturing():
                raise RuntimeError("the first train-mode forward of a MemoryAttention must run eagerly (it creates the device-side dropout counter)")
            self._drop_ctr = torch.full((1,), int(self._dropout_calls), dtype=torch.int64, device=dev)
        snap = torch.empty(1, dtype=torch.int64, device=dev)
        ops.counter_bump(self._drop_ctr, snap)
        self._dropout_calls += 1
        self._drop_ctr_host = self._dropout_calls
        return p, ops.DeviceSeed(int(self.dropout_seed) << 32, snap)

    def _project_all_keys(self, mem_k: torch.Tensor, B: int, L: int, n_ptr_tokens: int) -> Optional[torch.Tensor]:
        from .. import parallel
        n = len(self.layers)
        Nk = mem_k.shape[1]
        cas = [l.cross_attn_image for l in self.layers]
        if not (_BATCH_K_PROJ and n > 1 and parallel.current_kv_split() is None and all(isinstance(c, RoPEAttention) and c.folds_values() for c in cas)):
            return None
        C = cas[0].internal_dim
        tab = cas[0].table(L, mem_k.device)
        M = B * Nk
        if not (_FUSED_ROPE and M >= 256 and Nk >= 128 and tab[0].shape[0] >= 128 and Nk - n_ptr_tokens > 0 and M * n * C * 4 < 2 ** 31
                and len({(c.rope_theta, c.num_heads) for c in cas}) == 1):
            return None
        w = w_bf16(self._wc, "kall", *[c.k_proj.weight for c in cas])
        b = v_f32(self._wc, "kallb", *[c.k_proj.bias for c in cas])
        out = ops.gemm_rope(mem_k.reshape(M, -1), w, b, tab, rope_cols=n * C, head_dim=C // cas[0].num_heads, rows_per_batch=Nk,
                            n_rope=Nk - n_ptr_tokens)
        return out.view(B, Nk, n, C)

    def forward(self, curr: torch.Tensor, memory: torch.Tensor, curr_pos: Optional[torch.Tensor] = None,
                memory_pos: Optional[torch.Tensor] = None, num_obj_ptr_tokens: int = 0, key_count: Optional[torch.Tensor] = None):
        if isinstance(curr, list):
            assert isinstance(curr_pos, list) and len(curr) == len(curr_pos) == 1
            curr, curr_pos = curr[0], curr_pos[0]
        assert curr.shape[1] == memory.shape[1], "Batch size must be the same for curr and memory"
        L, B, C = curr.shape
        from .. import autograd as ag
        if ag.active(self) and key_count is None:
            pos = curr_pos if (curr_pos is not None and self.pos_enc_at_input) else torch.zeros_like(curr)
            return ag.memory_attention(self, curr, pos, memory, memory_pos, num_obj_ptr_tokens)
        drop = self.next_dropout()
        if drop is not None:
            from .. import backward as bwd
            assert key_count is None, "padded memory banks are an inference-path feature"
            zero = torch.zeros_like(curr) if curr_pos is None or not self.pos_enc_at_input else curr_pos
            return bwd.memory_attention_forward_saved(self, curr, zero, memory, memory_pos, num_obj_ptr_tokens, dropout=drop)[0]
        use_pos = self.pos_enc_at_input and curr_pos is not None
        x = ops.add_cast(curr.transpose(0, 1), curr_pos.transpose(0, 1) if use_pos else None, 0.1, F32).reshape(B * L, C)
        mem_bf = memory.transpose(0, 1)
        mem_k = ops.add_cast(mem_bf, memory_pos.transpose(0, 1), 1.0, OP16)
        mem_v = ops.add_cast(mem_bf, None, 1.0, OP16)
        kk_all = self._project_all_keys(mem_k, B, L, num_obj_ptr_tokens)
        for i, layer in enumerate(self.layers):
            x = layer.run(x, mem_k, mem_v, B, L, num_obj_ptr_tokens, key_count, None if kk_all is None else kk_all[:, :, i])
        y = ops.layernorm(x, v_f32(self._wc, "nw", self.norm.weight), v_f32(self._wc, "nb", self.norm.bias), self.norm.eps,
                          out_dtype=F32)
        return y.view(B, L, C).transpose(0, 1)


class MaskDownSampler(nn.Module):

    def __init__(self, embed_dim=256, kernel_size=4, stride=4, padding=0, total_stride=16, activation=nn.GELU):
        super().__init__()
        assert (kernel_size, stride, padding, total_stride) == (3, 2, 1, 16) and activation is nn.GELU, \
            "HIP path implements the YAML's k3/s2/p1 mask down-sampler"
        num_layers = int(math.log2(total_stride) // math.log2(stride))
        self.encoder = nn.Sequential()
        cin = 1
        for _ in range(num_layers):
            cout = cin * (stride ** 2)
            self.encoder.append(nn.Conv2d(cin, cout, kernel_size=kernel_size, stride=stride, padding=padding))
            self.encoder.append(LayerNorm2d(cout))
            self.encoder.append(activation())
            cin = cout
        self.encoder.append(nn.Conv2d(cin, embed_dim, kernel_size=1))
        self._wc = WeightCache()

    def run(self, mask: torch.Tensor, mode: int, scale: float, bias: float) -> torch.Tensor:
        n, _, S, _ = mask.shape
        wc, enc = self._wc, self.encoder
        f = lambda key, p: v_f32(wc, key, p)
        h = mask.to(F32).contiguous().reshape(n * S * S, 1)
        conv, ln = enc[0], enc[1]
        h = ops.conv3x3s2_ln_gelu(h, n, S, S, wc.get("cw0", [conv.weight], lambda: conv.weight.detach().float().contiguous()),
                                  f("cb0", conv.bias), f("lw0", ln.weight), f("lb0", ln.bias), mode, scale, bias)
        side = S // 2
        for j in range(1, 4):
            conv, ln = enc[3 * j], enc[3 * j + 1]
            cols = ops.im2col3x3s2(h, n, side, side)

            def pack(c=conv, ld=cols.shape[1]):
                w = c.weight.detach().permute(0, 2, 3, 1).reshape(c.weight.shape[0], -1)
                out = torch.zeros(w.shape[0], ld, dtype=OP16, device=w.device)
                out[:, : w.shape[1]] = w.to(OP16)
                return out
            g = ops.gemm(cols, wc.get(f"cw{j}", [conv.weight], pack), f(f"cb{j}", conv.bias), out_dtype=F32)
            h = ops.layernorm(g, f(f"lw{j}", ln.weight), f(f"lb{j}", ln.bias), ln.eps, act=ops.ACT_GELU)
            side //= 2
        return ops.gemm(h, w_bf16(wc, "pw", enc[12].weight), f("pb", enc[12].bias), out_dtype=F32)

    def forward(self, x: torch.Tensor) -> torch.Tensor:
        n, _, S, _ = x.shape
        return nchw_view(self.run(x, 0, 0.0, 0.0), n, S // 16, S // 16)


class CXBlock(nn.Module):

    def __init__(self, dim, kernel_size=7, padding=3, drop_path=0.0, layer_scale_init_value=1e-6, use_dwconv=True):
        super().__init__()
        assert kernel_size == 7 and padding == 3 and use_dwconv and drop_path == 0.0 and layer_scale_init_value > 0
        self.dwconv = nn.Conv2d(dim, dim, kernel_size=7, padding=3, groups=dim)
        self.norm = LayerNorm2d(dim, eps=1e-6)
        self.pwconv1 = nn.Linear(dim, 4 * dim)
        self.act = nn.GELU()
        self.pwconv2 = nn.Linear(4 * dim, dim)
        self.gamma = nn.Parameter(layer_scale_init_value * torch.ones(dim), requires_grad=True)
        self._wc = WeightCache()

    def run(self, x: torch.Tensor, n: int, H: int, W: int) -> torch.Tensor:
        wc = self._wc
        C = x.shape[1]
        wt = wc.get("dw", [self.dwconv.weight], lambda: self.dwconv.weight.detach().reshape(C, 49).t().float().contiguous())
        h = ops.dwconv7x7_ln(x, n, H, W, wt, v_f32(wc, "dwb", self.dwconv.bias), v_f32(wc, "lw", self.norm.weight),
                             v_f32(wc, "lb", self.norm.bias))
        h = ops.gemm(h, w_bf16(wc, "w1", self.pwconv1.weight), v_f32(wc, "b1", self.pwconv1.bias), act=ops.ACT_GELU)
        return ops.gemm(h, w_bf16(wc, "w2", self.pwconv2.weight), v_f32(wc, "b2", self.pwconv2.bias),
                        colscale=v_f32(wc, "g", self.gamma), residual=x, out_dtype=F32)

    def forward(self, x: torch.Tensor) -> torch.Tensor:
        n, C, H, W = x.shape
        return nchw_view(self.run(tokens_of(x.to(F32)), n, H, W), n, H, W)


class Fuser(nn.Module):

    def __init__(self, layer, num_layers, dim=None, input_projection=False):
        super().__init__()
        assert not input_projection, "SAM2 configs use no input projection in the fuser"
        self.proj = nn.Identity()
        self.layers = nn.ModuleList([copy.deepcopy(layer) for _ in range(num_layers)])

    def run(self, x, n, H, W):
        for layer in self.layers:
            x = layer.run(x, n, H, W)
        return x

    def forward(self, x: torch.Tensor) -> torch.Tensor:
        n, C, H, W = x.shape
        return nchw_view(self.run(tokens_of(x.to(F32)), n, H, W), n, H, W)


class MemoryEncoder(nn.Module):

    def __init__(self, out_dim, mask_downsampler, fuser, position_encoding, in_dim=256):
        super().__init__()
        self.mask_downsampler = mask_downsampler
        self.pix_feat_proj = nn.Conv2d(in_dim, in_dim, kernel_size=1)
        self.fuser = fuser
        self.position_encoding = position_encoding
        self.out_proj = nn.Identity()
        if out_dim != in_dim:
            self.out_proj = nn.Conv2d(in_dim, out_dim, kernel_size=1)
        self._wc = WeightCache()

    def run(self, pix_tokens: torch.Tensor, mask: torch.Tensor, mode: int, scale: float, bias: float, n: int, H: int, W: int):
        wc = self._wc
        m = self.mask_downsampler.run(mask, mode, scale, bias)
        x = ops.gemm(to_bf16(pix_tokens), w_bf16(wc, "pw", self.pix_feat_proj.weight), v_f32(wc, "pb", self.pix_feat_proj.bias),
                     residual=m, out_dtype=F32)
        x = self.fuser.run(x, n, H, W)
        if isinstance(self.out_proj, nn.Identity):
            return x
        return ops.gemm(to_bf16(x), w_bf16(wc, "ow", self.out_proj.weight), v_f32(wc, "ob", self.out_proj.bias), out_dtype=F32)

    def forward(self, pix_feat: torch.Tensor, masks: torch.Tensor, skip_mask_sigmoid: bool = False):
        n, C, H, W = pix_feat.shape
        y = self.run(tokens_of(pix_feat), masks, 0 if skip_mask_sigmoid else 1, 1.0, 0.0, n, H, W)
        x = nchw_view(y, n, H, W)
        pos = self.position_encoding(x).to(x.dtype)
        return {"vision_features": x, "vision_pos_enc": [pos]}
```

### medical-sam2_amd/modeling/sam_heads.py

```python
from __future__ import annotations

from typing import List, Optional, Tuple, Type

import torch
import torch.nn as nn

from .. import ops
from .common import OP16, F32, WeightCache, nchw_view, to_bf16, tokens_of, v_f32, w_bf16
from .encoder import MLP
from .memory import Attention, LayerNorm2d
from .position import PositionEmbeddingRandom


class PromptEncoder(nn.Module):

    def __init__(self, embed_dim: int, image_embedding_size: Tuple[int, int], input_image_size: Tuple[int, int],
                 mask_in_chans: int, activation: Type[nn.Module] = nn.GELU) -> None:
        super().__init__()
        self.embed_dim = embed_dim
        self.input_image_size = input_image_size
        self.image_embedding_size = image_embedding_size
        self.pe_layer = PositionEmbeddingRandom(embed_dim // 2)
        self.num_point_embeddings: int = 4
        self.point_embeddings = nn.ModuleList([nn.Embedding(1, embed_dim) for _ in range(self.num_point_embeddings)])
# ... 41 lines not shown
        h = ops.layernorm(h, f("lw0", md[1].weight), f("lb0", md[1].bias), md[1].eps, act=ops.ACT_GELU)
        h = ops.space_to_depth(h, n, H // 2, W // 2, 2)
        h = ops.gemm(h, patch_w(md[3], "w1"), f("b1", md[3].bias), out_dtype=F32)
        h = ops.layernorm(h, f("lw1", md[4].weight), f("lb1", md[4].bias), md[4].eps, act=ops.ACT_GELU)
        return ops.gemm(h, w_bf16(wc, "w2", md[6].weight), f("b2", md[6].bias), out_dtype=F32)

    def _get_batch_size(self, points, boxes, masks) -> int:
        if points is not None:
            return points[0].shape[0]
        if boxes is not None:
            return boxes.shape[0]
        if masks is not None:
            return masks.shape[0]
        return 1

    def forward(self, points: Optional[Tuple[torch.Tensor, torch.Tensor]], boxes: Optional[torch.Tensor],
                masks: Optional[torch.Tensor], batch_size=-1) -> Tuple[torch.Tensor, torch.Tensor]:
        bs = self._get_batch_size(points, boxes, masks)
        dev = self.no_mask_embed.weight.device
        xy_parts, lab_parts = [], []
        n_pad = 0
        if points is not None:
            coords, labels = points
            xy_parts.append(coords.to(F32))
            lab_parts.append(labels.to(torch.int32))
            if boxes is None:
                n_pad = 1
        if boxes is not None:
            xy_parts.append(boxes.to(F32).reshape(-1, 2, 2))
            lab_parts.append(torch.tensor([[2, 3]], dtype=torch.int32, device=dev).expand(bs, 2))
        if len(xy_parts) == 1:
            sparse = self._points(xy_parts[0].contiguous(), lab_parts[0].contiguous(), n_pad)
        elif xy_parts:
            sparse = self._points(torch.cat(xy_parts, 1).contiguous(), torch.cat(lab_parts, 1).contiguous())
        else:
            sparse = torch.empty((bs, 0, self.embed_dim), device=dev)
        h, w = self.image_embedding_size
        if masks is not None:
            dense = nchw_view(self._embed_masks_tokens(masks), bs, h, w)
        else:
            dense = self.no_mask_embed.weight.reshape(1, -1, 1, 1).expand(bs, -1, h, w)
        return sparse, dense


def _image_side_projections(wc: WeightCache, key: str, keys_b: torch.Tensor, key_pe: torch.Tensor, L: int, lins, with_pe):
    ws = [l.weight for l in lins]
    W = w_bf16(wc, key + "w", *ws)
    b = v_f32(wc, key + "b", *[l.bias for l in lins])

    def build_pe():
        R = ops.gemm(to_bf16(key_pe.contiguous()), W, None, out_dtype=F32)
        col = 0
        for l, use in zip(lins, with_pe):
            if not use:
                R[:, col: col + l.out_features] = 0.0
            col += l.out_features
        return R
    R = wc.get(key + "pe", ws + [key_pe], build_pe)
    return ops.gemm(keys_b, W, b, residual=R, res_mod=L)


class TwoWayAttentionBlock(nn.Module):

    def __init__(self, embedding_dim: int, num_heads: int, mlp_dim: int = 2048, activation: Type[nn.Module] = nn.ReLU,
                 attention_downsample_rate: int = 2, skip_first_layer_pe: bool = False) -> None:
        super().__init__()
        self.self_attn = Attention(embedding_dim, num_heads)
        self.norm1 = nn.LayerNorm(embedding_dim)
        self.cross_attn_token_to_image = Attention(embedding_dim, num_heads, downsample_rate=attention_downsample_rate)
        self.norm2 = nn.LayerNorm(embedding_dim)
        self.mlp = MLP(embedding_dim, mlp_dim, embedding_dim, num_layers=2, activation=activation)
        self.norm3 = nn.LayerNorm(embedding_dim)
        self.norm4 = nn.LayerNorm(embedding_dim)
        self.cross_attn_image_to_token = Attention(embedding_dim, num_heads, downsample_rate=attention_downsample_rate)
        self.skip_first_layer_pe = skip_first_layer_pe
        self._wc = WeightCache()

    def _ln(self, name, x):
        n = getattr(self, name)
        return ops.layernorm(x, v_f32(self._wc, name + "w", n.weight), v_f32(self._wc, name + "b", n.bias), n.eps, out_dtype=F32)

    def run(self, queries, keys, query_pe, key_pe, B, T, L, keys_b=None):
        C = queries.shape[1]
        q3 = lambda t, n: t.view(B, n, -1)
        sa, ca, ia, wc = self.self_attn, self.cross_attn_token_to_image, self.cross_attn_image_to_token, self._wc
        fused = B * T <= 32 and C % 32 == 0 and sa.internal_dim % 32 == 0 and ia.internal_dim % 32 == 0
        if fused:
            Ci = sa.internal_dim
            qkv = ops.gemm_tokens(queries, w_bf16(wc, "sqkv", sa.q_proj.weight, sa.k_proj.weight, sa.v_proj.weight),
                                  v_f32(wc, "sqkvb", sa.q_proj.bias, sa.k_proj.bias, sa.v_proj.bias),
                                  addend=None if self.skip_first_layer_pe else query_pe, add_cols=2 * Ci).view(B, T, 3 * Ci)
            o = sa.core(qkv[:, :, :Ci], qkv[:, :, Ci:2 * Ci], qkv[:, :, 2 * Ci:])
            queries = sa.out(o, None if self.skip_first_layer_pe else queries)
        elif self.skip_first_layer_pe:
            qb = to_bf16(queries)
            queries = sa.out(sa.core(q3(sa.proj("q", qb), T), q3(sa.proj("k", qb), T), q3(sa.proj("v", qb), T)), None)
        else:
            qb = ops.add_cast(queries.view(1, B * T, C), query_pe.view(1, B * T, C), 1.0, OP16)[0]
            queries = sa.out(sa.core(q3(sa.proj("q", qb), T), q3(sa.proj("k", qb), T), q3(sa.proj("v", to_bf16(queries)), T)), queries)
        queries = self._ln("norm1", queries)
        if keys_b is None:
            keys_b = to_bf16(keys)
        Cc, Ci2 = ca.internal_dim, ia.internal_dim
        kvq = _image_side_projections(wc, "ikvq", keys_b, key_pe, L, [ca.k_proj, ca.v_proj, ia.q_proj], [True, False, True])
        k_img, v_img, q_img = kvq[:, :Cc], kvq[:, Cc:2 * Cc], kvq[:, 2 * Cc:2 * Cc + Ci2]
        if fused:
            qp = ops.gemm_tokens(queries, w_bf16(wc, "cqw", ca.q_proj.weight), v_f32(wc, "cqb", ca.q_proj.bias), addend=query_pe,
                                 add_cols=ca.internal_dim)
        else:
            qp = ca.proj("q", ops.add_cast(queries.view(1, B * T, C), query_pe.view(1, B * T, C), 1.0, OP16)[0])
        o = ca.core(q3(qp, T), q3(k_img, L), q3(v_img, L))
        queries = self._ln("norm2", ca.out(o, queries))
        if fused and self.mlp.num_layers == 2:
            l1, l2 = self.mlp.layers
            hmid = ops.gemm_tokens(queries, w_bf16(wc, "m1w", l1.weight), v_f32(wc, "m1b", l1.bias), act=self.mlp._act_code)
            queries = self._ln("norm3", ops.gemm(hmid, w_bf16(wc, "m2w", l2.weight), v_f32(wc, "m2b", l2.bias), residual=queries, out_dtype=F32))
        else:
            queries = self._ln("norm3", self.mlp.run(to_bf16(queries), residual=queries, out_dtype=F32))
        if fused:
            Cd = ia.internal_dim
            kv = ops.gemm_tokens(queries, w_bf16(wc, "ikv", ia.k_proj.weight, ia.v_proj.weight), v_f32(wc, "ikvb", ia.k_proj.bias, ia.v_proj.bias),
                                 addend=query_pe, add_cols=Cd).view(B, T, 2 * Cd)
            o = ia.core(q3(q_img, L), kv[:, :, :Cd], kv[:, :, Cd:])
        else:
            qb = ops.add_cast(queries.view(1, B * T, C), query_pe.view(1, B * T, C), 1.0, OP16)[0]
            o = ia.core(q3(q_img, L), q3(ia.proj("k", qb), T), q3(ia.proj("v", to_bf16(queries)), T))
        n4 = self.norm4
        keys, keys16 = ops.layernorm_dual(ia.out(o, keys), v_f32(wc, "norm4w", n4.weight), v_f32(wc, "norm4b", n4.bias), n4.eps)
        return queries, keys, keys16

    def forward(self, queries, keys, query_pe, key_pe):
        B, T, C = queries.shape
        L = keys.shape[1]
        assert key_pe.shape[0] == 1 or B == 1, "key_pe is the batch-shared dense position encoding"
        q, k, _ = self.run(queries.to(F32).reshape(B * T, C).contiguous(), keys.to(F32).reshape(B * L, C).contiguous(),
                           query_pe.to(F32).reshape(B * T, C).contiguous(), key_pe.to(F32).reshape(-1, C)[:L].contiguous(), B, T, L)
        return q.view(B, T, C), k.view(B, L, C)


class TwoWayTransformer(nn.Module):

    def __init__(self, depth: int, embedding_dim: int, num_heads: int, mlp_dim: int, activation: Type[nn.Module] = nn.ReLU,
                 attention_downsample_rate: int = 2) -> None:
        super().__init__()
        self.depth, self.embedding_dim, self.num_heads, self.mlp_dim = depth, embedding_dim, num_heads, mlp_dim
        self.layers = nn.ModuleList([
            TwoWayAttentionBlock(embedding_dim=embedding_dim, num_heads=num_heads, mlp_dim=mlp_dim, activation=activation,
                                 attention_downsample_rate=attention_downsample_rate, skip_first_layer_pe=(i == 0))
            for i in range(depth)])
        self.final_attn_token_to_image = Attention(embedding_dim, num_heads, downsample_rate=attention_downsample_rate)
        self.norm_final_attn = nn.LayerNorm(embedding_dim)
        self._wc = WeightCache()

    def run(self, keys, key_pe, tokens, B, T, L):
        C = tokens.shape[1]
        queries, qpe = tokens, tokens
        keys16 = None
        for layer in self.layers:
            queries, keys, keys16 = layer.run(queries, keys, qpe, key_pe, B, T, L, keys16)
        if keys16 is None:
            keys16 = to_bf16(keys)
        self._keys16 = keys16
        fa = self.final_attn_token_to_image
        kv_img = _image_side_projections(self._wc, "fkv", keys16, key_pe, L, [fa.k_proj, fa.v_proj], [True, False])
        Cf = fa.internal_dim
        q3 = lambda t, n: t.view(B, n, -1)
        if B * T <= 32 and fa.internal_dim % 32 == 0:
            qp = ops.gemm_tokens(queries, w_bf16(self._wc, "fqw", fa.q_proj.weight), v_f32(self._wc, "fqb", fa.q_proj.bias), addend=qpe,
                                 add_cols=fa.internal_dim)
        else:
            qp = fa.proj("q", ops.add_cast(queries.view(1, B * T, C), qpe.view(1, B * T, C), 1.0, OP16)[0])
        o = fa.core(q3(qp, T), q3(kv_img[:, :Cf], L), q3(kv_img[:, Cf:], L))
        n = self.norm_final_attn
        queries = ops.layernorm(fa.out(o, queries), v_f32(self._wc, "nw", n.weight), v_f32(self._wc, "nb", n.bias), n.eps, out_dtype=F32)
        return queries, keys

    def forward(self, image_embedding, image_pe, point_embedding):
        B, C, h, w = image_embedding.shape
        T = point_embedding.shape[1]
        keys = tokens_of(image_embedding.to(F32))
        pe = tokens_of(image_pe.to(F32))[: h * w]
        q, k = self.run(keys, pe, point_embedding.to(F32).reshape(B * T, C).contiguous(), B, T, h * w)
        return q.view(B, T, C), k.view(B, h * w, C)


class MaskDecoder(nn.Module):

    def __init__(self, *, transformer_dim: int, transformer: nn.Module, num_multimask_outputs: int = 3,
                 activation: Type[nn.Module] = nn.GELU, iou_head_depth: int = 3, iou_head_hidden_dim: int = 256,
                 use_high_res_features: bool = False, iou_prediction_use_sigmoid=False, dynamic_multimask_via_stability=False,
                 dynamic_multimask_stability_delta=0.05, dynamic_multimask_stability_thresh=0.98, pred_obj_scores: bool = False,
                 pred_obj_scores_mlp: bool = False, use_multimask_token_for_obj_ptr: bool = False) -> None:
        super().__init__()
        assert num_multimask_outputs == 3 and use_high_res_features and pred_obj_scores and pred_obj_scores_mlp, \
            "HIP path implements the SAM2 YAML decoder (3 multimasks, high-res skips, object-score MLP)"
        self.transformer_dim, self.transformer = transformer_dim, transformer
        self.num_multimask_outputs = num_multimask_outputs
        self.iou_token = nn.Embedding(1, transformer_dim)
        self.num_mask_tokens = num_multimask_outputs + 1
        self.mask_tokens = nn.Embedding(self.num_mask_tokens, transformer_dim)
        self.pred_obj_scores = pred_obj_scores
        self.obj_score_token = nn.Embedding(1, transformer_dim)
        self.use_multimask_token_for_obj_ptr = use_multimask_token_for_obj_ptr
        self.output_upscaling = nn.Sequential(
            nn.ConvTranspose2d(transformer_dim, transformer_dim // 4, kernel_size=2, stride=2), LayerNorm2d(transformer_dim // 4),
            activation(), nn.ConvTranspose2d(transformer_dim // 4, transformer_dim // 8, kernel_size=2, stride=2), activation())
        self.use_high_res_features = use_high_res_features
        self.conv_s0 = nn.Conv2d(transformer_dim, transformer_dim // 8, kernel_size=1, stride=1)
        self.conv_s1 = nn.Conv2d(transformer_dim, transformer_dim // 4, kernel_size=1, stride=1)
        self.output_hypernetworks_mlps = nn.ModuleList(
            [MLP(transformer_dim, transformer_dim, transformer_dim // 8, 3) for _ in range(self.num_mask_tokens)])
        self.iou_prediction_head = MLP(transformer_dim, iou_head_hidden_dim, self.num_mask_tokens, iou_head_depth,
                                       sigmoid_output=iou_prediction_use_sigmoid)
        self.pred_obj_score_head = MLP(transformer_dim, transformer_dim, 1, 3)
        self.dynamic_multimask_via_stability = dynamic_multimask_via_stability
        self.dynamic_multimask_stability_delta = dynamic_multimask_stability_delta
        self.dynamic_multimask_stability_thresh = dynamic_multimask_stability_thresh
        self._wc = WeightCache()

    def conv_s(self, which: int, tokens_bf16: torch.Tensor, out_dtype=OP16) -> torch.Tensor:
        c = self.conv_s0 if which == 0 else self.conv_s1
        return ops.gemm(tokens_bf16, w_bf16(self._wc, f"cs{which}w", c.weight), v_f32(self._wc, f"cs{which}b", c.bias), out_dtype=out_dtype)

    def predict_masks_tokens(self, src_tokens: torch.Tensor, pe_tokens: torch.Tensor, sparse: torch.Tensor, feat_s0: torch.Tensor,
                             feat_s1: torch.Tensor, B: int, h: int, w: int, shared_skips: bool = False):
        wc = self._wc
        C = self.transformer_dim
        out_tok = wc.get("otok", [self.obj_score_token.weight, self.iou_token.weight, self.mask_tokens.weight],
                         lambda: torch.cat([self.obj_score_token.weight, self.iou_token.weight, self.mask_tokens.weight], 0).detach().float())
        T = out_tok.shape[0] + sparse.shape[1]
        tokens = torch.cat([out_tok.unsqueeze(0).expand(B, -1, -1), sparse], 1)
        hs, keys = self.transformer.run(src_tokens, pe_tokens, tokens.view(B * T, C), B, T, h * w)
        hs = hs.view(B, T, C)
        up = self.output_upscaling
        dc1_w = wc.get("dc1", [up[0].weight], lambda: up[0].weight.detach().permute(2, 3, 1, 0).reshape(-1, C).to(OP16).contiguous())
        keys16 = getattr(self.transformer, "_keys16", None)
        if keys16 is None or keys16.shape != keys.shape:
            keys16 = to_bf16(keys)
        self.transformer._keys16 = None
        g = ops.gemm(keys16, dc1_w)
        shuffle = ops.convt2x2_shuffle_shared if shared_skips else ops.convt2x2_shuffle
        u = shuffle(g, v_f32(wc, "dc1b", up[0].bias), feat_s1, v_f32(wc, "lnw", up[1].weight), v_f32(wc, "lnb", up[1].bias), B, h, w)
        dc2_w = wc.get("dc2", [up[3].weight], lambda: up[3].weight.detach().permute(2, 3, 1, 0).reshape(-1, C // 4).to(OP16).contiguous())
        g = ops.gemm(u, dc2_w)
        u = shuffle(g, v_f32(wc, "dc2b", up[3].bias), feat_s0, None, None, B, 2 * h, 2 * w)
        heads = list(self.output_hypernetworks_mlps) + [self.iou_prediction_head, self.pred_obj_score_head]
        fusable = C == 256 and self.pred_obj_scores and all(
            m.num_layers == 3 and m._act_code == ops.ACT_RELU and m.layers[0].in_features == C and m.layers[0].out_features == C
            and m.layers[1].out_features == C and m.layers[2].out_features <= C for m in heads)
        if fusable:
            G = len(heads)
            params = [t for m in heads for l in m.layers for t in (l.weight, l.bias)]

            def pack():
                dev = hs.device
                w1 = torch.stack([m.layers[0].weight.detach() for m in heads]).to(OP16).contiguous()
                w2 = torch.stack([m.layers[1].weight.detach() for m in heads]).to(OP16).contiguous()
                w3 = torch.zeros(G, C, C, dtype=OP16, device=dev)
                b3 = torch.zeros(G, C, dtype=F32, device=dev)
                for gi, m in enumerate(heads):
                    n = m.layers[2].out_features
                    w3[gi, :n] = m.layers[2].weight.detach().to(OP16)
                    b3[gi, :n] = m.layers[2].bias.detach().float()
                b1 = torch.stack([m.layers[0].bias.detach() for m in heads]).float().contiguous()
                b2 = torch.stack([m.layers[1].bias.detach() for m in heads]).float().contiguous()
                return w1, b1, w2, b2, w3, b3

            def consts():
                dev = hs.device
                nm_ = self.num_mask_tokens
                return (torch.tensor([2 + i for i in range(nm_)] + [1, 0], dtype=torch.int32, device=dev),
                        torch.tensor([m.layers[2].out_features for m in heads], dtype=torch.int32, device=dev),
                        torch.tensor([int(m.sigmoid_output) for m in heads], dtype=torch.int32, device=dev))
            tok, od, sg = wc.get("heads_const", [], consts)
            w1, b1, w2, b2, w3, b3 = wc.get("heads", params, pack)
            nm = self.num_mask_tokens
            n_hyper, n_iou, n_obj = C // 8, heads[nm].layers[2].out_features, heads[nm + 1].layers[2].out_features

            def layout():
                dev = hs.device
                off = [g * n_hyper for g in range(nm)] + [B * nm * n_hyper, B * nm * n_hyper + B * n_iou]
                ld = [nm * n_hyper] * nm + [n_iou, n_obj]
                return torch.tensor(off, dtype=torch.int32, device=dev), torch.tensor(ld, dtype=torch.int32, device=dev)
            off, ld = wc.get(f"heads_layout{B}", [], layout)
            y = ops.token_mlp3(hs, tok, w1, b1, w2, b2, w3, b3, od, sg, packed=(off, ld, B * (nm * n_hyper + n_iou + n_obj)))
            hyper = y[: B * nm * n_hyper].view(B, nm, n_hyper)
            iou = y[B * nm * n_hyper: B * (nm * n_hyper + n_iou)].view(B, n_iou)
            obj = y[B * (nm * n_hyper + n_iou):].view(B, n_obj)
        else:
            hyper = torch.empty(B, self.num_mask_tokens, C // 8, dtype=F32, device=u.device)
            for i, m in enumerate(self.output_hypernetworks_mlps):
                hyper[:, i] = m.run(to_bf16(hs[:, 2 + i].contiguous()))
            iou = self.iou_prediction_head.run(to_bf16(hs[:, 1].contiguous()))
            obj = self.pred_obj_score_head.run(to_bf16(hs[:, 0].contiguous()))
        masks = ops.hyper_masks(hyper, u, B, 16 * h * w).view(B, self.num_mask_tokens, 4 * h, 4 * w)
        return masks, iou, hs[:, 2:2 + self.num_mask_tokens], obj

    def predict_masks(self, image_embeddings, image_pe, sparse_prompt_embeddings, dense_prompt_embeddings, repeat_image,
                      cell_nums=None, high_res_features=None):
        n_sets = sparse_prompt_embeddings.shape[0]
        from .. import autograd as ag
        shared = (n_sets > 1 and image_embeddings.shape[0] == 1 and high_res_features is not None
                  and all(f.shape[0] == 1 for f in high_res_features) and self.transformer_dim // 8 in (32, 64)
                  and (cell_nums is None or torch.as_tensor(cell_nums).reshape(-1).tolist() == [n_sets]) and not ag.active(self))
        if shared:
            _, C, h, w = image_embeddings.shape
            B = n_sets
            e3 = tokens_of(image_embeddings.to(F32)).view(1, h * w, C).expand(B, h * w, C)
            dense = dense_prompt_embeddings.to(F32).expand(B, C, h, w)
            if dense.stride(2) == 0 and dense.stride(3) == 0:
                d3 = dense[:, :, 0, 0].unsqueeze(1).expand(B, h * w, C)
            else:
                d3 = tokens_of(dense).view(B, h * w, C)
            src = ops.add_cast(e3, d3, 1.0, F32).view(B * h * w, C)
            pe = tokens_of(image_pe.to(F32))[: h * w]
            f0, f1 = high_res_features
            skip = lambda f: tokens_of(f) if (f.dtype == F32 and f.shape[1] in (32, 64)) else to_bf16(tokens_of(f))
            return self.predict_masks_tokens(src, pe, sparse_prompt_embeddings.to(F32), skip(f0), skip(f1), B, h, w, shared_skips=True)
        if image_embeddings.shape[0] != n_sets:
            if cell_nums is not None:
                cn = torch.as_tensor(cell_nums, device=image_embeddings.device).reshape(-1).long()
                if cn.numel() != image_embeddings.shape[0] or int(cn.sum()) != n_sets:
                    raise RuntimeError(f"cell_nums {cn.tolist()} does not split {n_sets} prompt sets over {image_embeddings.shape[0]} images")
                image_embeddings = torch.repeat_interleave(image_embeddings, cn, dim=0)
            elif image_embeddings.shape[0] == 1:
                image_embeddings = image_embeddings.expand(n_sets, -1, -1, -1)
            else:
                raise RuntimeError(f"The size of tensor a ({image_embeddings.shape[0]}) must match the size of tensor b ({n_sets}) at non-singleton dimension 0")
            hr = []
            for f in high_res_features:
                if f.shape[0] == 1:
                    f = f.expand(n_sets, -1, -1, -1)
                elif f.shape[0] != n_sets:
                    raise RuntimeError(f"The size of tensor a ({n_sets}) must match the size of tensor b ({f.shape[0]}) at non-singleton dimension 0")
                hr.append(f)
            high_res_features = hr
        B, C, h, w = image_embeddings.shape
        assert sparse_prompt_embeddings.shape[0] == B, "one prompt set per (repeated) image embedding"
        if ag.active(self):
            src = tokens_of(image_embeddings.to(F32)).view(B, h * w, C) + tokens_of(dense_prompt_embeddings.to(F32).expand(B, C, h, w)).view(B, h * w, C)
            f0, f1 = high_res_features
            return ag.mask_decoder(self, src.reshape(B * h * w, C), tokens_of(image_pe.to(F32))[: h * w].detach(), sparse_prompt_embeddings.to(F32),
                                   tokens_of(f0), tokens_of(f1), B, h, w)
        emb = image_embeddings.to(F32)
        dense = dense_prompt_embeddings.to(F32).expand(B, C, h, w)
        e3 = tokens_of(emb).view(B, h * w, C)
        if dense.stride(2) == 0 and dense.stride(3) == 0:
            d3 = dense[:, :, 0, 0].unsqueeze(1).expand(B, h * w, C)
        else:
            d3 = tokens_of(dense).view(B, h * w, C)
        src = ops.add_cast(e3, d3, 1.0, F32).view(B * h * w, C)
        pe = tokens_of(image_pe.to(F32))[: h * w]
        f0, f1 = high_res_features
        skip = lambda f: tokens_of(f) if (f.dtype == F32 and f.shape[1] in (32, 64)) else to_bf16(tokens_of(f))
        return self.predict_masks_tokens(src, pe, sparse_prompt_embeddings.to(F32), skip(f0), skip(f1), B, h, w)

    def forward(self, image_embeddings, image_pe, sparse_prompt_embeddings, dense_prompt_embeddings, multimask_output: bool,
                repeat_image: bool, cell_nums=None, high_res_features: Optional[List[torch.Tensor]] = None):
        masks, iou_pred, mask_tokens_out, object_score_logits = self.predict_masks(
            image_embeddings, image_pe, sparse_prompt_embeddings, dense_prompt_embeddings, repeat_image, cell_nums, high_res_features)
        if multimask_output:
            masks, iou_pred = masks[:, 1:, :, :], iou_pred[:, 1:]
        elif self.dynamic_multimask_via_stability and not self.training:
            nb = object_score_logits.shape[0]
            obj_pos = self._wc.get(f"ones{nb}", [], lambda: torch.ones(nb, dtype=F32, device=object_score_logits.device))
            low, sel, iou_sel = ops.select_mask(masks.contiguous(), iou_pred.contiguous(), obj_pos, False, True,
                                                self.dynamic_multimask_stability_delta, self.dynamic_multimask_stability_thresh)
            masks, iou_pred = low, iou_sel
        else:
            masks, iou_pred = masks[:, 0:1, :, :], iou_pred[:, 0:1]
        if multimask_output and self.use_multimask_token_for_obj_ptr:
            sam_tokens_out = mask_tokens_out[:, 1:]
        else:
            sam_tokens_out = mask_tokens_out[:, 0:1]
        return masks, iou_pred, sam_tokens_out, object_score_logits
```

### medical-sam2_amd/ops.py

```python
from __future__ import annotations

import ctypes
import math
from typing import Optional, Tuple

import torch

from ._lib import check, lib

OP16 = torch.float16 if lib().msam2_operand_is_fp16() else torch.bfloat16

F32 = torch.float32
ACT_NONE, ACT_GELU, ACT_RELU, ACT_SIGMOID = 0, 1, 2, 3


def _stream() -> int:
    return torch.cuda.current_stream().cuda_stream


def _p(t: Optional[torch.Tensor]):
    return None if t is None else t.data_ptr()


def _is_bf16(t: torch.Tensor) -> int:
    if t.dtype == OP16:
        return 1
    if t.dtype == F32:
        return 0
    raise TypeError(f"expected {OP16} or fp32 tensor, got {t.dtype}")


def _req(cond: bool, msg: str):
    if not cond:
        raise ValueError(msg)


def gemm(a: torch.Tensor, w: torch.Tensor, bias: Optional[torch.Tensor] = None, *, act: int = ACT_NONE,
         colscale: Optional[torch.Tensor] = None, residual: Optional[torch.Tensor] = None, res_mod: int = 0,
         out_dtype: torch.dtype = OP16, out: Optional[torch.Tensor] = None) -> torch.Tensor:
    _req(a.dim() == 2 and w.dim() == 2 and a.shape[1] == w.shape[1], f"gemm shapes {tuple(a.shape)} x {tuple(w.shape)}")
    _req(a.dtype == OP16 and w.dtype == OP16, "gemm operands must be 16-bit (ops.OP16)")
    _req(a.stride(1) == 1 and w.stride(1) == 1, "gemm operands must be K-contiguous")
    M, K = a.shape
    N = w.shape[0]
    if out is None:
        out = torch.empty(M, N, dtype=out_dtype, device=a.device)
    _req(out.stride(1) == 1 and out.shape == (M, N), "gemm out must be [M,N] row-major")
    if residual is not None:
        _req(residual.dim() == 2 and residual.stride(1) == 1 and residual.shape[1] == N, "gemm residual must be [*,N]")
    check(lib().msam2_gemm(_p(a), a.stride(0), _p(w), w.stride(0), _p(bias), _p(colscale), _p(residual),
                                residual.stride(0) if residual is not None else 0,
                                _is_bf16(residual) if residual is not None else 0, res_mod, _p(out), out.stride(0),
                                _is_bf16(out), M, N, K, act, _stream()))
    return out


def gemm_tokens(a: torch.Tensor, w: torch.Tensor, bias: Optional[torch.Tensor] = None, *, addend: Optional[torch.Tensor] = None,
                add_cols: int = 0, act: int = ACT_NONE, residual: Optional[torch.Tensor] = None, out_dtype: torch.dtype = OP16) -> torch.Tensor:
    _req(a.dim() == 2 and a.dtype == F32 and a.stride(1) == 1 and a.shape[0] <= 32, "gemm_tokens: a must be fp32 [M<=32, K]")
    _req(w.dtype == OP16 and w.stride(1) == 1 and w.shape[1] == a.shape[1], "gemm_tokens: w must be 16-bit [N, K]")
    if addend is not None:
        _req(addend.dtype == F32 and addend.shape == a.shape and addend.stride(1) == 1 and addend.stride(0) == a.stride(0),
             "gemm_tokens: addend must match a")
    M, K = a.shape
    N = w.shape[0]
    out = torch.empty(M, N, dtype=out_dtype, device=a.device)
    if residual is not None:
        _req(residual.dtype == F32 and residual.shape == (M, N) and residual.stride(1) == 1, "gemm_tokens: residual must be fp32 [M,N]")
    check(lib().msam2_gemm_tokens(_p(a), a.stride(0), _p(addend), add_cols if addend is not None else 0, _p(w), w.stride(0), _p(bias),
                                  _p(residual), residual.stride(0) if residual is not None else 0, _p(out), out.stride(0), _is_bf16(out),
                                  M, N, K, act, _stream()))
    return out


def gemm_pool2x2(a: torch.Tensor, w: torch.Tensor, bias: Optional[torch.Tensor], B: int, H: int, W: int) -> torch.Tensor:
    _req(a.dim() == 2 and w.dim() == 2 and a.shape[1] == w.shape[1] and a.shape[0] == B * H * W, "gemm_pool2x2 shapes")
    _req(a.dtype == OP16 and w.dtype == OP16 and a.stride(1) == 1 and w.stride(1) == 1, "gemm_pool2x2 operands: 16-bit, K-contiguous")
    N, K = w.shape
    out = torch.empty(B * (H // 2) * (W // 2), N, dtype=F32, device=a.device)
    check(lib().msam2_gemm_pool2x2(_p(a), a.stride(0), _p(w), w.stride(0), _p(bias), _p(out), out.stride(0), B, H, W, N, K, _stream()))
    return out


def gemm_qkv_pool2x2(a: torch.Tensor, w: torch.Tensor, bias: Optional[torch.Tensor], B: int, H: int, W: int, q_cols: int):
    _req(a.dim() == 2 and w.dim() == 2 and a.shape[1] == w.shape[1] and a.shape[0] == B * H * W, "gemm_qkv_pool2x2 shapes")
    _req(a.dtype == OP16 and w.dtype == OP16 and a.stride(1) == 1 and w.stride(1) == 1, "gemm_qkv_pool2x2 operands: 16-bit, K-contiguous")
    N, K = w.shape
    qkv = torch.empty(B * H * W, N, dtype=OP16, device=a.device)
    q2 = torch.empty(B * (H // 2) * (W // 2), q_cols, dtype=OP16, device=a.device)
    check(lib().msam2_gemm_qkv_pool2x2(_p(a), a.stride(0), _p(w), w.stride(0), _p(bias), _p(qkv), qkv.stride(0), _p(q2), q2.stride(0),
                                       B, H, W, N, K, q_cols, _stream()))
    return qkv, q2


def gemm_rope(a: torch.Tensor, w: torch.Tensor, bias: Optional[torch.Tensor], table: Tuple[torch.Tensor, torch.Tensor], *,
              rope_cols: int, head_dim: int, rows_per_batch: int, n_rope: int, out: Optional[torch.Tensor] = None) -> torch.Tensor:
    _req(a.dim() == 2 and w.dim() == 2 and a.shape[1] == w.shape[1], f"gemm_rope shapes {tuple(a.shape)} x {tuple(w.shape)}")
    _req(a.dtype == OP16 and w.dtype == OP16 and a.stride(1) == 1 and w.stride(1) == 1, "gemm_rope operands: 16-bit, K-contiguous")
    cs, sn = table
    _req(cs.dtype == F32 and cs.is_contiguous() and sn.is_contiguous() and cs.shape == sn.shape and cs.shape[1] * 2 == head_dim,
         "gemm_rope: table must be cos/sin fp32 [n_pos, head_dim/2]")
    M, K = a.shape
    N = w.shape[0]
    if out is None:
        out = torch.empty(M, N, dtype=OP16, device=a.device)
    _req(out.dtype == OP16 and out.shape == (M, N) and out.stride(1) == 1, "gemm_rope: out must be 16-bit [M, N] row-major")
    check(lib().msam2_gemm_rope(_p(a), a.stride(0), _p(w), w.stride(0), _p(bias), _p(out), out.stride(0), M, N, K, _p(cs), _p(sn),
                                rope_cols, head_dim, rows_per_batch, n_rope, cs.shape[0], _stream()))
    return out


def layernorm(x: torch.Tensor, weight: torch.Tensor, bias: torch.Tensor, eps: float, *, act: int = ACT_NONE,
              out_dtype: torch.dtype = OP16) -> torch.Tensor:
    C = x.shape[-1]
    x2 = x.reshape(-1, C)
    _req(x2.stride(1) == 1, "layernorm input rows must be contiguous")
    y = torch.empty(x2.shape, dtype=out_dtype, device=x.device)
    check(lib().msam2_layernorm(_p(x2), _is_bf16(x2), x2.stride(0), _p(weight), _p(bias), _p(y), _is_bf16(y), y.stride(0),
                                x2.shape[0], C, eps, act, _stream()))
    return y.reshape(x.shape)


def layernorm_dual(x: torch.Tensor, weight: torch.Tensor, bias: torch.Tensor, eps: float):
    C = x.shape[-1]
    x2 = x.reshape(-1, C)
    _req(x2.dtype == F32 and x2.stride(1) == 1 and C % 4 == 0, "layernorm_dual: fp32 rows, C % 4 == 0")
    y = torch.empty(x2.shape, dtype=F32, device=x.device)
    y16 = torch.empty(x2.shape, dtype=OP16, device=x.device)
    check(lib().msam2_layernorm_dual(_p(x2), x2.stride(0), _p(weight), _p(bias), _p(y), y.stride(0), _p(y16), y16.stride(0), x2.shape[0], C, eps,
                                     _stream()))
    return y.reshape(x.shape), y16.reshape(x.shape)


def ln_mlp_residual_supported(dim: int) -> bool:
    return bool(lib().msam2_ln_mlp_residual_supported(dim))


def mlp_fused_permute_w2(w2: torch.Tensor) -> torch.Tensor:
    _req(w2.dim() == 2 and w2.dtype == OP16 and w2.is_contiguous() and w2.shape[1] % 32 == 0, "mlp_fused_permute_w2: 16-bit [dim, hidden]")
    out = torch.empty_like(w2)
    check(lib().msam2_mlp_fused_permute_w2(_p(w2), _p(out), w2.shape[0], w2.shape[1], _stream()))
    return out


def ln_mlp_residual(x: torch.Tensor, ln_w: torch.Tensor, ln_b: torch.Tensor, eps: float, w1: torch.Tensor, b1: torch.Tensor, w2p: torch.Tensor,
                    b2: torch.Tensor, also16: bool = False):
    T, dim = x.shape
    _req(x.dtype == F32 and x.is_contiguous() and w1.dtype == OP16 and w2p.dtype == OP16 and w1.shape == (4 * dim, dim) and w2p.shape == (dim, 4 * dim)
         and w1.is_contiguous() and w2p.is_contiguous(), "ln_mlp_residual: x fp32 [T, dim], w1 [4 dim, dim], w2p [dim, 4 dim] 16-bit contiguous")
    out = torch.empty_like(x)
    if also16:
        out16 = torch.empty(x.shape, dtype=OP16, device=x.device)
        check(lib().msam2_ln_mlp_residual_fwd_dual(_p(x), T, dim, _p(ln_w), _p(ln_b), float(eps), _p(w1), _p(b1), _p(w2p), _p(b2), _p(out), _p(out16),
                                                   _stream()))
        return out, out16
    check(lib().msam2_ln_mlp_residual_fwd(_p(x), T, dim, _p(ln_w), _p(ln_b), float(eps), _p(w1), _p(b1), _p(w2p), _p(b2), _p(out), _stream()))
    return out


def _strides3(t: torch.Tensor) -> "ctypes.Array":
    return (ctypes.c_int64 * 3)(t.stride(0), t.stride(1), t.stride(2))


def attention(q: torch.Tensor, k: torch.Tensor, v: torch.Tensor, *, splits: int = 1,
              out: Optional[torch.Tensor] = None, scale: Optional[float] = None, workspace: Optional[torch.Tensor] = None,
              defer_merge: bool = False, lse: Optional[torch.Tensor] = None, dropout: Optional[tuple] = None) -> torch.Tensor:
    B, H, Lq, D = q.shape
    Lk = k.shape[2]
    for t in (q, k, v):
        _req(t.dtype == OP16 and t.stride(3) == 1, "attention tensors must be 16-bit (ops.OP16) with contiguous head dim")
    if out is None:
        out = torch.empty(B, Lq, H, D, dtype=OP16, device=q.device).permute(0, 2, 1, 3)
    if lse is not None:
        _req(lse.dtype == F32 and lse.is_contiguous() and lse.numel() == B * H * Lq and not defer_merge, "attention: lse must be fp32 [B,H,Lq]")
        splits = max(splits, 2)
    ws_bytes = lib().msam2_attention_workspace_bytes(B, H, Lq, D, splits)
    ws = workspace if workspace is not None else (torch.empty(max(ws_bytes, 1), dtype=torch.uint8, device=q.device) if splits > 1 else None)
    _req(not defer_merge or (workspace is not None and splits > 1), "defer_merge needs splits > 1 and a caller-owned workspace")
    _req(ws is None or ws.numel() * ws.element_size() >= ws_bytes, "attention workspace too small")
    sc = scale if scale is not None else 1.0 / math.sqrt(D)
    if dropout is not None and dropout[0] > 0:
        _req(lse is not None, "attention: dropout is a training feature (pass lse)")
        pd, seed, offset = dropout
        seed_dev = None
        if isinstance(seed, DeviceSeed):
            seed, seed_dev = seed.base, seed.dev
        check(lib().msam2_attention_fwd_lse_dropout(_p(q), _strides3(q), _p(k), _strides3(k), _p(v), _strides3(v), _p(out), _strides3(out),
                                                    B, H, Lq, Lk, D, sc, splits, _p(ws), ws_bytes if ws is not None else 0, _p(lse), float(pd),
                                                    int(seed) & (2 ** 64 - 1), int(offset) & (2 ** 64 - 1), _p(seed_dev), _stream()))
        return out
    if lse is not None:
        check(lib().msam2_attention_fwd_lse(_p(q), _strides3(q), _p(k), _strides3(k), _p(v), _strides3(v), _p(out), _strides3(out),
                                            B, H, Lq, Lk, D, sc, splits, _p(ws), ws_bytes if ws is not None else 0, _p(lse), _stream()))
        return out
    check(lib().msam2_attention_fwd(_p(q), _strides3(q), _p(k), _strides3(k), _p(v), _strides3(v), _p(out), _strides3(out),
                                    B, H, Lq, Lk, D, sc, -splits if defer_merge else splits, _p(ws), ws_bytes if ws is not None else 0, _stream()))
    return out


def attention_kv64(q: torch.Tensor, k: torch.Tensor, v: torch.Tensor, *, splits: int = 1, scale: Optional[float] = None,
                   workspace: Optional[torch.Tensor] = None, defer_merge: bool = False,
                   key_count: Optional[torch.Tensor] = None, out: Optional[torch.Tensor] = None) -> torch.Tensor:
    B, H, Lq, D = q.shape
    Lk = k.shape[2]
    _req(D == 256 and k.shape[3] == 256 and v.shape[3] == 64 and v.shape[2] == Lk, "attention_kv64: q/k rows of 256, v rows of 64")
    _req(key_count is None or (key_count.dtype == torch.int32 and key_count.numel() == 1 and key_count.device == q.device),
         "attention_kv64: key_count is one int32 on the tensors' device")
    for t in (q, k, v):
        _req(t.dtype == OP16 and t.stride(3) == 1, "attention tensors must be 16-bit (ops.OP16) with contiguous head dim")
    if out is None:
        out = torch.empty(B, Lq, H, 64, dtype=OP16, device=q.device).permute(0, 2, 1, 3)
    _req(out.dtype == OP16 and out.shape == (B, H, Lq, 64) and out.stride(3) == 1, "attention_kv64: out is a 16-bit [B,H,Lq,64] view")
    ws_bytes = lib().msam2_attention_workspace_bytes(B, H, Lq, 64, splits)
    ws = workspace if workspace is not None else (torch.empty(max(ws_bytes, 1), dtype=torch.uint8, device=q.device) if splits > 1 else None)
    _req(not defer_merge or (workspace is not None and splits > 1), "defer_merge needs splits > 1 and a caller-owned workspace")
    _req(ws is None or ws.numel() * ws.element_size() >= ws_bytes, "attention workspace too small")
    sc = scale if scale is not None else 1.0 / math.sqrt(D)
    if key_count is not None:
        check(lib().msam2_attention_kv64_dyn_fwd(_p(q), _strides3(q), _p(k), _strides3(k), _p(v), _strides3(v), _p(out), _strides3(out),
                                                 B, H, Lq, Lk, _p(key_count), sc, -splits if defer_merge else splits, _p(ws),
                                                 ws_bytes if ws is not None else 0, _stream()))
        return out
    check(lib().msam2_attention_kv64_fwd(_p(q), _strides3(q), _p(k), _strides3(k), _p(v), _strides3(v), _p(out), _strides3(out),
                                         B, H, Lq, Lk, sc, -splits if defer_merge else splits, _p(ws), ws_bytes if ws is not None else 0, _stream()))
    return out


def attention_effective_splits(Lk: int, splits: int) -> int:
    return int(lib().msam2_attention_effective_splits(Lk, splits))


def attention_kv64_partial(q: torch.Tensor, k: torch.Tensor, v: torch.Tensor, *, splits: int, split_begin: int, split_count: int,
                           workspace: torch.Tensor, scale: Optional[float] = None, key_count: Optional[torch.Tensor] = None) -> None:
    B, H, Lq, D = q.shape
    Lk = k.shape[2]
    for t in (q, k, v):
        _req(t.dtype == OP16 and t.stride(3) == 1, "attention tensors must be 16-bit (ops.OP16) with contiguous head dim")
    sc = scale if scale is not None else 1.0 / math.sqrt(D)
    if key_count is not None:
        _req(key_count.dtype == torch.int32 and key_count.numel() == 1, "attention_kv64_partial: key_count is one int32 on the device")
        check(lib().msam2_attention_kv64_dyn_partial(_p(q), _strides3(q), _p(k), _strides3(k), _p(v), _strides3(v), B, H, Lq, Lk, _p(key_count),
                                                     sc, splits, split_begin, split_count, _p(workspace),
                                                     workspace.numel() * workspace.element_size(), _stream()))
        return
    check(lib().msam2_attention_kv64_partial(_p(q), _strides3(q), _p(k), _strides3(k), _p(v), _strides3(v), B, H, Lq, Lk, sc, splits,
                                             split_begin, split_count, _p(workspace), workspace.numel() * workspace.element_size(), _stream()))


def attention_workspace(B: int, H: int, Lq: int, D: int, splits: int, device) -> torch.Tensor:
    return torch.empty(max(lib().msam2_attention_workspace_bytes(B, H, Lq, D, splits), 1), dtype=torch.uint8, device=device)


def attention_merge(out: torch.Tensor, Lk: int, splits: int, workspace: torch.Tensor) -> torch.Tensor:
    B, H, Lq, D = out.shape
    check(lib().msam2_attention_merge(_p(out), _strides3(out), B, H, Lq, Lk, D, splits, _p(workspace),
                                      workspace.numel() * workspace.element_size(), _stream()))
    return out


def window_attention(qkv: torch.Tensor, B: int, H: int, W: int, heads: int, ws: int, qkv_bias: torch.Tensor,
                     q_pooled: Optional[torch.Tensor] = None, scale: Optional[float] = None,
                     out: Optional[torch.Tensor] = None) -> torch.Tensor:
    dim_out = qkv.shape[1] // 3
    D = dim_out // heads
    _req(qkv.dtype == OP16 and qkv.stride(1) == 1, "qkv must be 16-bit (ops.OP16) row-major")
    if q_pooled is None:
        qt, q_ts, hq, wq, ws_q = qkv, qkv.stride(0), H, W, ws
    else:
        qt, q_ts, hq, wq, ws_q = q_pooled, q_pooled.stride(0), H // 2, W // 2, ws // 2
    o = out if out is not None else torch.empty(B * hq * wq, dim_out, dtype=OP16, device=qkv.device)
    _req(o.dtype == OP16 and o.shape == (B * hq * wq, dim_out) and o.stride(1) == 1, "window_attention: out is 16-bit [B*Hq*Wq, heads*D] rows")
    kpad = qkv_bias[dim_out:2 * dim_out]
    vpad = qkv_bias[2 * dim_out:]
    kptr = qkv.data_ptr() + dim_out * 2
    vptr = qkv.data_ptr() + 2 * dim_out * 2
    check(lib().msam2_window_attention_fwd(_p(qt), q_ts, D, hq, wq, ws_q, kptr, vptr, qkv.stride(0), D, H, W, ws, _p(kpad),
                                           _p(vpad), _p(o), o.stride(0), D, B, heads, D, scale if scale is not None else 1.0 / math.sqrt(D), _stream()))
    return o


def attention_small(q: torch.Tensor, k: torch.Tensor, v: torch.Tensor, heads: int, out: Optional[torch.Tensor] = None) -> torch.Tensor:
    B, Lq, C = q.shape
    Lk = k.shape[1]
    D = C // heads
    for t in (q, k, v):
        _req(t.dtype == OP16 and t.stride(2) == 1, "attention_small tensors must be 16-bit (ops.OP16), channel-contiguous")
    o = out if out is not None else torch.empty(B, Lq, C, dtype=OP16, device=q.device)
    _req(o.dtype == OP16 and o.shape == (B, Lq, C) and o.stride(2) == 1, "attention_small: out is 16-bit [B,Lq,C] with contiguous channels")
    check(lib().msam2_attention_small_fwd(_p(q), q.stride(0), q.stride(1), _p(k), k.stride(0), k.stride(1), _p(v), v.stride(0),
                                          v.stride(1), _p(o), o.stride(0), o.stride(1), B, heads, Lq, Lk, D,
                                          1.0 / math.sqrt(D), _stream()))
    return o


def add_cast(a: torch.Tensor, b: Optional[torch.Tensor] = None, alpha: float = 1.0, out_dtype: torch.dtype = OP16,
             out: Optional[torch.Tensor] = None) -> torch.Tensor:
    _req(a.dim() == 3 and (a.stride(2) == 1 or a.shape[2] == 1), "add_cast: a must be [D0,D1,C] with contiguous C")
    D0, D1, C = a.shape
    bs0 = bs1 = 0
    if b is not None:
        b = b.expand(D0, D1, C)
        _req(b.stride(2) == 1 or C == 1, "add_cast: b must have contiguous C")
        bs0, bs1 = b.stride(0), b.stride(1)
    if out is None:
        out = torch.empty(D0, D1, C, dtype=out_dtype, device=a.device)
    _req(out.is_contiguous() and out.numel() == D0 * D1 * C, "add_cast: out must be a contiguous [D0,D1,C] buffer")
    check(lib().msam2_add_cast(_p(a), _is_bf16(a), a.stride(0), a.stride(1), _p(b), _is_bf16(b) if b is not None else 0, bs0,
                               bs1, alpha, _p(out), _is_bf16(out), D0, D1, C, _stream()))
    return out


class DeviceSeed:
    __slots__ = ("base", "dev")

    def __init__(self, base: int, dev: torch.Tensor):
        assert dev.dtype == torch.int64 and dev.numel() == 1 and dev.is_cuda
        self.base, self.dev = int(base), dev


def counter_bump(counter: torch.Tensor, snapshot: Optional[torch.Tensor] = None) -> None:
    _req(counter.dtype == torch.int64 and counter.numel() == 1 and (snapshot is None or (snapshot.dtype == torch.int64 and snapshot.numel() == 1)),
         "counter_bump: int64 [1] tensors")
    check(lib().msam2_counter_bump(_p(counter), _p(snapshot), _stream()))


def dropout(x: torch.Tensor, p: float, seed, offset: int, residual: Optional[torch.Tensor] = None,
            out_dtype: Optional[torch.dtype] = None, out: Optional[torch.Tensor] = None) -> torch.Tensor:
    seed_dev = None
    if isinstance(seed, DeviceSeed):
        seed, seed_dev = seed.base, seed.dev
    _req(x.dim() == 2 and x.stride(1) == 1, "dropout: [rows, cols] row-major")
    rows, cols = x.shape
    y = out if out is not None else torch.empty(rows, cols, dtype=out_dtype or x.dtype, device=x.device)
    _req(y.shape == x.shape and y.stride(1) == 1, "dropout: out must be [rows, cols] row-major (rows may be strided)")
    if residual is not None:
        _req(residual.dtype == F32 and residual.shape == x.shape and residual.stride(1) == 1, "dropout: residual must be fp32 [rows, cols]")
    check(lib().msam2_dropout(_p(x), _is_bf16(x), x.stride(0), _p(residual), residual.stride(0) if residual is not None else 0, _p(y), _is_bf16(y),
                              y.stride(0), rows, cols, float(p), int(seed) & (2 ** 64 - 1), int(offset) & (2 ** 64 - 1), _p(seed_dev), _stream()))
    return y


def add_cast_into(out: torch.Tensor, a: torch.Tensor, b: Optional[torch.Tensor] = None, alpha: float = 1.0) -> torch.Tensor:
    return add_cast(a, b, alpha, out=out)


def gate_no_obj_(x: torch.Tensor, score: torch.Tensor, value: float) -> torch.Tensor:
    _req(x.dtype == F32 and x.is_contiguous(), "gate_no_obj: fp32 contiguous")
    B = x.shape[0]
    check(lib().msam2_gate_rows(_p(x), _p(score), value, B, x.numel() // B, _stream()))
    return x


def any_positive(x: torch.Tensor) -> torch.Tensor:
    _req(x.dtype == F32 and x.is_contiguous(), "any_positive: fp32 contiguous")
    B = x.shape[0]
    out = torch.empty(B, 1, dtype=F32, device=x.device)
    check(lib().msam2_any_positive(_p(x), _p(out), B, x.numel() // B, _stream()))
    return out


def maxpool2x2(x: torch.Tensor, B: int, H: int, W: int, out_dtype: Optional[torch.dtype] = None) -> torch.Tensor:
    C = x.shape[1]
    _req(x.stride(1) == 1, "maxpool2x2: channel dim must be contiguous")
    y = torch.empty(B * (H // 2) * (W // 2), C, dtype=out_dtype or x.dtype, device=x.device)
    check(lib().msam2_maxpool2x2(_p(x), _is_bf16(x), x.stride(0), _p(y), _is_bf16(y), y.stride(0), B, H, W, C, _stream()))
    return y


def upsample2x_add_(y: torch.Tensor, top: torch.Tensor, B: int, H: int, W: int) -> torch.Tensor:
    _req(y.dtype == F32 and top.dtype == F32 and y.is_contiguous() and top.is_contiguous(), "upsample2x_add: fp32 contiguous")
    check(lib().msam2_upsample2x_add(_p(y), _p(top), B, H, W, y.shape[-1], _stream()))
    return y


def rope_table(side: int, D: int, theta: float, device) -> Tuple[torch.Tensor, torch.Tensor]:
    cs = torch.empty(side * side, D // 2, dtype=F32, device=device)
    sn = torch.empty_like(cs)
    check(lib().msam2_rope_table(_p(cs), _p(sn), side, D, theta, _stream()))
    return cs, sn


def rope_(x: torch.Tensor, n_rope: int, table: Tuple[torch.Tensor, torch.Tensor]) -> torch.Tensor:
    B, L, D = x.shape
    _req(x.dtype == OP16 and x.stride(2) == 1, "rope: 16-bit with contiguous D")
    cs, sn = table
    check(lib().msam2_rope_inplace(_p(x), x.stride(0), x.stride(1), B, L, n_rope, cs.shape[0], D, _p(cs), _p(sn), _stream()))
    return x


def bilinear_upsample(x: torch.Tensor, H: int, W: int) -> torch.Tensor:
    _req(x.dtype == F32 and x.is_contiguous(), "bilinear: fp32 contiguous")
    h, w = x.shape[-2:]
    planes = x.numel() // (h * w)
    y = torch.empty(*x.shape[:-2], H, W, dtype=F32, device=x.device)
    check(lib().msam2_bilinear_upsample(_p(x), _p(y), planes, h, w, H, W, _stream()))
    return y


def sine_pos_2d(h: int, w: int, C: int, device, temperature: float = 10000.0) -> torch.Tensor:
    out = torch.empty(h * w, C, dtype=F32, device=device)
    check(lib().msam2_sine_pos_2d(_p(out), h, w, C, temperature, _stream()))
    return out


def fourier_pe_grid(gauss: torch.Tensor, h: int, w: int) -> torch.Tensor:
    C = 2 * gauss.shape[1]
    out = torch.empty(h * w, C, dtype=F32, device=gauss.device)
    check(lib().msam2_fourier_pe_grid(_p(out), _p(gauss.contiguous()), h, w, C, _stream()))
    return out


def hiera_pos_embed(pos_embed: torch.Tensor, pos_embed_window: torch.Tensor, h: int, w: int) -> torch.Tensor:
    _, C, bh, bw = pos_embed.shape
    out = torch.empty(h * w, C, dtype=F32, device=pos_embed.device)
    check(lib().msam2_hiera_pos_embed(_p(out), _p(pos_embed.contiguous()), _p(pos_embed_window.contiguous()), C, bh, bw, h, w,
                                      pos_embed_window.shape[-1], _stream()))
    return out


def im2col_patch(img: torch.Tensor) -> torch.Tensor:
    _req(img.dtype == F32 and img.is_contiguous() and img.shape[1] == 3 and img.shape[2] == img.shape[3], "im2col_patch: [B,3,S,S] fp32")
    B, _, S, _ = img.shape
    out = torch.empty(B * (S // 4) ** 2, 160, dtype=OP16, device=img.device)
    check(lib().msam2_im2col_patch7x7s4(_p(img), _p(out), B, S, _stream()))
    return out


def patch_embed_supported(S: int, E: int) -> bool:
    So = S // 4
    return S % 4 == 0 and So % 32 == 0 and E <= 128


def patch_embed(img: torch.Tensor, w_perm: torch.Tensor, bias: torch.Tensor, pos: Optional[torch.Tensor] = None) -> torch.Tensor:
    _req(img.dtype == F32 and img.is_contiguous() and img.shape[1] == 3 and img.shape[2] == img.shape[3], "patch_embed: [B,3,S,S] fp32")
    B, _, S, _ = img.shape
    E = bias.shape[0]
    _req(patch_embed_supported(S, E), "patch_embed: unsupported size (use im2col_patch + gemm)")
    _req(w_perm.dtype == OP16 and w_perm.is_contiguous() and tuple(w_perm.shape) == ((E + 31) // 32 * 32, 176), "patch_embed: w_perm [ceil32(E), 176] 16-bit")
    _req(bias.dtype == F32 and bias.is_contiguous(), "patch_embed: fp32 bias")
    if pos is not None:
        _req(pos.dtype == F32 and pos.is_contiguous() and tuple(pos.shape) == ((S // 4) ** 2, E), "patch_embed: pos fp32 [(S/4)^2, E]")
    out = torch.empty(B * (S // 4) ** 2, E, dtype=F32, device=img.device)
    check(lib().msam2_patch_embed7x7s4(_p(img), _p(w_perm), _p(bias), _p(pos), _p(out), B, S, E, _stream()))
    return out


def im2col3x3s2(x: torch.Tensor, B: int, H: int, W: int) -> torch.Tensor:
    C = x.shape[-1]
    _req(x.dtype == OP16 and x.is_contiguous(), "im2col3x3s2: 16-bit contiguous NHWC")
    ld = (9 * C + 7) // 8 * 8
    out = torch.empty(B * (H // 2) * (W // 2), ld, dtype=OP16, device=x.device)
    check(lib().msam2_im2col3x3s2(_p(x), _p(out), B, H, W, C, ld, _stream()))
    return out


def conv3x3s2_ln_gelu(x: torch.Tensor, B: int, H: int, W: int, weight, bias, ln_w, ln_b, mask_mode: int = 0,
                      mask_scale: float = 0.0, mask_bias: float = 0.0) -> torch.Tensor:
    cout, cin = weight.shape[0], weight.shape[1]
    _req(x.dtype == (F32 if cin == 1 else OP16) and x.is_contiguous() and x.numel() == B * H * W * cin,
         "conv3x3s2_ln_gelu: contiguous NHWC [B*H*W, cin], fp32 for cin = 1, 16-bit otherwise")
    _req(all(t.dtype == F32 and t.is_contiguous() for t in (weight, bias, ln_w, ln_b)) and tuple(weight.shape[2:]) == (3, 3)
         and bias.numel() == cout and ln_w.numel() == cout and ln_b.numel() == cout, "conv3x3s2_ln_gelu: fp32 contiguous [cout, cin, 3, 3] weight, [cout] vectors")
    y = torch.empty(B * (H // 2) * (W // 2), cout, dtype=OP16, device=x.device)
    check(lib().msam2_conv3x3s2_ln_gelu(_p(x), _is_bf16(x), _p(weight), _p(bias), _p(ln_w), _p(ln_b), _p(y), B, H, W, cin, cout,
                                        mask_mode, mask_scale, mask_bias, _stream()))
    return y


def dwconv7x7_ln(x: torch.Tensor, B: int, H: int, W: int, w_tap_major, bias, ln_w, ln_b) -> torch.Tensor:
    _req(x.dtype == F32 and x.is_contiguous(), "dwconv7x7_ln: fp32 contiguous NHWC")
    C = x.shape[-1]
    y = torch.empty(B * H * W, C, dtype=OP16, device=x.device)
    check(lib().msam2_dwconv7x7_ln(_p(x), _p(w_tap_major), _p(bias), _p(ln_w), _p(ln_b), _p(y), B, H, W, C, _stream()))
    return y


def convt2x2_shuffle(g: torch.Tensor, bias, skip: torch.Tensor, ln_w, ln_b, B: int, h: int, w: int) -> torch.Tensor:
    C = g.shape[1] // 4
    _req(g.dtype == OP16 and skip.dtype in (OP16, F32) and g.is_contiguous() and skip.is_contiguous(), "convt2x2_shuffle: contiguous 16-bit g, 16-bit / fp32 skip")
    y = torch.empty(B * 4 * h * w, C, dtype=OP16, device=g.device)
    if skip.dtype == F32:
        _req(C in (32, 64), "convt2x2_shuffle: fp32 skip features need C = 32 / 64")
        check(lib().msam2_convt2x2_shuffle_f32skip(_p(g), _p(bias), _p(skip), _p(ln_w), _p(ln_b), _p(y), B, h, w, C, _stream()))
    else:
        check(lib().msam2_convt2x2_shuffle(_p(g), _p(bias), _p(skip), _p(ln_w), _p(ln_b), _p(y), B, h, w, C, _stream()))
    return y


def convt2x2_shuffle_shared(g: torch.Tensor, bias, skip: torch.Tensor, ln_w, ln_b, B: int, h: int, w: int) -> torch.Tensor:
    C = g.shape[1] // 4
    _req(g.dtype == OP16 and skip.dtype in (OP16, F32) and g.is_contiguous() and skip.is_contiguous(), "convt2x2_shuffle_shared: contiguous 16-bit g, 16-bit / fp32 skip")
    _req(skip.numel() == 4 * h * w * C, "convt2x2_shuffle_shared: skip must be one [4hw, C] map")
# ... 595 lines not shown
```

Before: 689.5 slices/s.

## Fuse im2col into conv GEMM, fp32-A GEMM, and paired add-cast outputs

Adds an implicit-GEMM 3x3 stride-2 conv kernel that gathers input taps directly in the A-load, removing the materialised im2col buffer in the mask downsampler. Adds a GEMM variant that reads fp32 A and converts it in registers, so the memory encoder's out_proj no longer needs a separate bf16 cast. It also adds a paired add_cast kernel that writes both the sum and the casted memory (or the sum in two dtypes) in one pass. That pass is used in memory attention and in the mask decoder, where the precomputed bf16 keys are passed into the two-way transformer. Each change saves a kernel launch and a round trip through memory, at the cost of more complex load paths with per-element bounds checks.

New measurement: 695.1 slices/s (median of 6 runs). Within noise of the previous version (+0.8%).

```diff
diff --git a/include/msam2_hip.h b/include/msam2_hip.h
--- a/include/msam2_hip.h
+++ b/include/msam2_hip.h
@@ -30,6 +30,10 @@
 
 int msam2_event_destroy(void* ev);
 
+int msam2_gemm_f32a(const float* A, int64_t lda, const void* W, int64_t ldw, const float* bias, void* C, int64_t ldc, int out_is_16bit, int64_t M, int64_t N, int64_t K, void* stream);
+
+int msam2_gemm_conv3x3s2(const void* x, const void* Wp, int64_t ldw, const float* bias, float* C, int64_t ldc, int64_t B, int64_t H, int64_t W, int64_t Cin, int64_t N, int64_t K, void* stream);
+
 int msam2_gemm_nt(const void* A, int64_t lda, const void* B, int64_t ldb, const float* bias, const void* residual, int64_t ldr, void* C, int64_t ldc, int out_is_16bit, int64_t M, int64_t N, int64_t K, void* stream);
 
 int msam2_gemm(const void* A, int64_t lda, const void* W, int64_t ldw, const float* bias, const float* colscale, const void* residual, int64_t ldr, int res_is_16bit, int64_t res_mod, void* C, int64_t ldc, int out_is_16bit, int64_t M, int64_t N, int64_t K, int act, void* stream);
@@ -77,6 +81,8 @@
 int msam2_layernorm_dual(const float* x, int64_t ldx, const float* weight, const float* bias, float* y, int64_t ldy, void* y16, int64_t ldy16, int64_t rows, int64_t C, float eps, void* stream);
 
 int msam2_add_cast(const void* a, int a_is_16bit, int64_t a_s0, int64_t a_s1, const void* b, int b_is_16bit, int64_t b_s0, int64_t b_s1, float alpha, void* out, int out_is_16bit, int64_t D0, int64_t D1, int64_t C, void* stream);
+
+int msam2_add_cast_pair(const void* a, int a_is_16bit, int64_t a_s0, int64_t a_s1, const void* b, int b_is_16bit, int64_t b_s0, int64_t b_s1, float alpha, void* out, int out_is_16bit, void* out2_16bit, int second_of_sum, int64_t D0, int64_t D1, int64_t C, void* stream);
 
 int msam2_maxpool2x2(const void* x, int in_is_16bit, int64_t ldx, void* y, int out_is_16bit, int64_t ldy, int64_t B, int64_t H, int64_t W, int64_t C, void* stream);
 
diff --git a/medical-sam2_amd/_lib.py b/medical-sam2_amd/_lib.py
--- a/medical-sam2_amd/_lib.py
+++ b/medical-sam2_amd/_lib.py
@@ -19,6 +19,8 @@
     "msam2_last_error": (ctypes.c_char_p, []),
     "msam2_operand_is_fp16": (c_i, []),
     "msam2_gemm": (c_i, [c_p, c_l, c_p, c_l, c_p, c_p, c_p, c_l, c_i, c_l, c_p, c_l, c_i, c_l, c_l, c_l, c_i, c_p]),
+    "msam2_gemm_f32a": (c_i, [c_p, c_l, c_p, c_l, c_p, c_p, c_l, c_i, c_l, c_l, c_l, c_p]),
+    "msam2_gemm_conv3x3s2": (c_i, [c_p, c_p, c_l, c_p, c_p, c_l, c_l, c_l, c_l, c_l, c_l, c_l, c_p]),
     "msam2_gemm_pool2x2": (c_i, [c_p, c_l, c_p, c_l, c_p, c_p, c_l, c_l, c_l, c_l, c_l, c_l, c_p]),
     "msam2_gemm_qkv_pool2x2": (c_i, [c_p, c_l, c_p, c_l, c_p, c_p, c_l, c_p, c_l, c_l, c_l, c_l, c_l, c_l, c_l, c_p]),
     "msam2_gemm_tokens": (c_i, [c_p, c_l, c_p, c_l, c_p, c_l, c_p, c_p, c_l, c_p, c_l, c_i, c_l, c_l, c_l, c_i, c_p]),
@@ -45,6 +47,7 @@
     "msam2_attention_small_fwd": (c_i, [c_p, c_l, c_l, c_p, c_l, c_l, c_p, c_l, c_l, c_p, c_l, c_l, c_l, c_l, c_l, c_l, c_l, c_f,
                                         c_p]),
     "msam2_add_cast": (c_i, [c_p, c_i, c_l, c_l, c_p, c_i, c_l, c_l, c_f, c_p, c_i, c_l, c_l, c_l, c_p]),
+    "msam2_add_cast_pair": (c_i, [c_p, c_i, c_l, c_l, c_p, c_i, c_l, c_l, c_f, c_p, c_i, c_p, c_i, c_l, c_l, c_l, c_p]),
     "msam2_maxpool2x2": (c_i, [c_p, c_i, c_l, c_p, c_i, c_l, c_l, c_l, c_l, c_l, c_p]),
     "msam2_upsample2x_add": (c_i, [c_p, c_p, c_l, c_l, c_l, c_l, c_p]),
     "msam2_rope_table": (c_i, [c_p, c_p, c_l, c_l, c_f, c_p]),
diff --git a/medical-sam2_amd/csrc/elementwise.hip b/medical-sam2_amd/csrc/elementwise.hip
--- a/medical-sam2_amd/csrc/elementwise.hip
+++ b/medical-sam2_amd/csrc/elementwise.hip
@@ -247,6 +247,61 @@
   return msam2_check_launch("add_cast");
 }
 
+template <typename TA, typename TB, typename TO>
+__global__ void add_cast_pair_vec_kernel(const TA* __restrict__ a, int64_t a_s0, int64_t a_s1, const TB* __restrict__ b, int64_t b_s0,
+                                         int64_t b_s1, float alpha, TO* __restrict__ out, op16* __restrict__ out2, int second_of_sum,
+                                         unsigned D0, unsigned D1, unsigned C4) {
+  typedef typename Vec4<TA>::type VA;
+  typedef typename Vec4<TB>::type VB;
+  typedef typename Vec4<TO>::type VO;
+  const unsigned rows = D0 * D1;
+  const unsigned total = rows * C4;
+  for (unsigned i = blockIdx.x * blockDim.x + threadIdx.x; i < total; i += gridDim.x * blockDim.x) {
+    const unsigned g = i % C4, rj = i / C4;
+    const unsigned j = rj % D1, r = rj / D1;
+    const VA va = *reinterpret_cast<const VA*>(a + r * a_s0 + j * a_s1 + g * 4);
+    const VB vb = *reinterpret_cast<const VB*>(b + r * b_s0 + j * b_s1 + g * 4);
+    float v[4], v0[4];
+#pragma unroll
+    for (int e = 0; e < 4; ++e) v0[e] = v[e] = (float)va[e];
+#pragma unroll
+    for (int e = 0; e < 4; ++e) v[e] += alpha * (float)vb[e];
+    VO o;
+    op16x4 o2;
+#pragma unroll
+    for (int e = 0; e < 4; ++e) {
+      o[e] = f2out<TO>(v[e]);
+      o2[e] = f2out<op16>(second_of_sum ? (float)o[e] : v0[e]);
+    }
+    *reinterpret_cast<VO*>(out + (int64_t)i * 4) = o;
+    *reinterpret_cast<op16x4*>(out2 + (int64_t)i * 4) = o2;
+  }
+}
+
+extern "C" int msam2_add_cast_pair(const void* a, int a_is_16bit, int64_t a_s0, int64_t a_s1, const void* b, int b_is_16bit, int64_t b_s0,
+                                   int64_t b_s1, float alpha, void* out, int out_is_16bit, void* out2_16bit, int second_of_sum, int64_t D0,
+                                   int64_t D1, int64_t C, void* stream) {
+  MSAM2_REQUIRE(a && b && out && out2_16bit, "add_cast_pair: null tensor");
+  MSAM2_REQUIRE(D0 > 0 && D1 > 0 && C > 0, "add_cast_pair: empty volume");
+  const int64_t total = D0 * D1 * C;
+  MSAM2_REQUIRE((C % 4 == 0) && total / 4 < (1ll << 31) && vec_ok(4, a_is_16bit ? 2 : 4, a_s0, a_s1, a) && vec_ok(4, out_is_16bit ? 2 : 4, out) &&
+                    vec_ok(4, 2, out2_16bit) && vec_ok(4, b_is_16bit ? 2 : 4, b_s0, b_s1, b),
+                "add_cast_pair: C, the strides and the tensors must keep four-element groups aligned (use two msam2_add_cast calls)");
+  hipStream_t s = (hipStream_t)stream;
+  with_type(a_is_16bit, [&](auto ta) {
+    with_type(b_is_16bit, [&](auto tb) {
+      with_type(out_is_16bit, [&](auto to) {
+        using TA = decltype(ta);
+        using TB = decltype(tb);
+        using TO = decltype(to);
+        hipLaunchKernelGGL((add_cast_pair_vec_kernel<TA, TB, TO>), dim3(grid1d(total / 4, 16384)), dim3(256), 0, s, (const TA*)a, a_s0, a_s1,
+                           (const TB*)b, b_s0, b_s1, alpha, (TO*)out, (op16*)out2_16bit, second_of_sum, (unsigned)D0, (unsigned)D1, (unsigned)(C / 4));
+      });
+    });
+  });
+  return msam2_check_launch("add_cast_pair");
+}
+
 template <typename TI, typename TO>
 __global__ void maxpool2x2_kernel(const TI* __restrict__ x, int64_t ldx, TO* __restrict__ y, int64_t ldy, int B, int H, int W,
                                   int C) {
diff --git a/medical-sam2_amd/csrc/gemm.hip b/medical-sam2_amd/csrc/gemm.hip
--- a/medical-sam2_amd/csrc/gemm.hip
+++ b/medical-sam2_amd/csrc/gemm.hip
@@ -1568,6 +1568,196 @@
   return msam2_check_launch("gemm");
 }
 
+
+template <int BM, int BN, int WM, int WN, int AMODE>
+__global__ __launch_bounds__(WM* WN * 64) void gemm_aload_kernel(GemmParams p, int cH, int cW, int cshift) {
+  constexpr int NT = WM * WN * 64;
+  constexpr int TM = BM / WM, TN = BN / WN;
+  constexpr int FM = TM / 32, FN = TN / 32;
+  constexpr int A_CHUNKS = BM * 4, W_CHUNKS = BN * 4;
+  constexpr int A_PER = (A_CHUNKS + NT - 1) / NT, W_PER = (W_CHUNKS + NT - 1) / NT;
+  __shared__ __attribute__((aligned(16))) op16 lds[2 * (BM + BN) * GEMM_LDS_STRIDE];
+  op16* As = lds;
+  op16* Ws = lds + 2 * BM * GEMM_LDS_STRIDE;
+
+  const int tid = threadIdx.x;
+  const int wave = tid >> 6, lane = tid & 63;
+  const int wm = wave / WN, wn = wave % WN;
+  const int r = lane & 31, h = lane >> 5;
+  const int64_t m0 = (int64_t)blockIdx.y * BM;
+  const int64_t n0 = (int64_t)blockIdx.x * BN;
+
+  f32x16 acc[FM][FN];
+  zero_acc(acc);
+
+  uint4 ra[A_PER], rw[W_PER];
+  const int nk = (p.K + GEMM_BK - 1) / GEMM_BK;
+
+  const float* a32_row[A_PER];
+  const op16* a_img[A_PER];
+  int a_y[A_PER], a_x[A_PER];
+  const op16* w_row[W_PER];
+  int a_kc[A_PER], w_kc[W_PER];
+  bool a_in[A_PER], w_in[W_PER];
+#pragma unroll
+  for (int i = 0; i < A_PER; ++i) {
+    const int c = min(tid + i * NT, A_CHUNKS - 1);
+    const int row = c >> 2;
+    a_in[i] = tid + i * NT < A_CHUNKS && m0 + row < p.M;
+    const unsigned m = (unsigned)min(m0 + row, (int64_t)p.M - 1);
+    a_kc[i] = (c & 3) * 8;
+    if constexpr (AMODE == 1) {
+      a32_row[i] = p.A32 + (int64_t)m * p.lda;
+    } else {
+      const unsigned Wo = (unsigned)cW >> 1, Ho = (unsigned)cH >> 1;
+      const unsigned t1 = m / Wo, xo = m - t1 * Wo;
+      const unsigned b = t1 / Ho, yo = t1 - b * Ho;
+      a_img[i] = p.A + (((int64_t)b * cH * cW) << cshift);
+      a_y[i] = 2 * (int)yo - 1;
+      a_x[i] = 2 * (int)xo - 1;
+    }
+  }
+#pragma unroll
+  for (int i = 0; i < W_PER; ++i) {
+    const int c = min(tid + i * NT, W_CHUNKS - 1);
+    const int row = c >> 2;
+    w_in[i] = tid + i * NT < W_CHUNKS && n0 + row < p.N;
+    w_row[i] = p.W + min(n0 + row, (int64_t)p.N - 1) * p.ldw;
+    w_kc[i] = (c & 3) * 8;
+  }
+  auto tap_at = [&](int i, int tap, int c, bool& in) -> const op16* {
+    const int t = min(tap, 8);
+    const int y = a_y[i] + t / 3, x = a_x[i] + t % 3;
+    in = tap < 9 && y >= 0 && y < cH && x >= 0 && x < cW;
+    return a_img[i] + (((int64_t)min(max(y, 0), cH - 1) * cW + min(max(x, 0), cW - 1)) << cshift) + (tap < 9 ? c : 0);
+  };
+  auto gload = [&](int kt) {
+    const int k0 = kt * GEMM_BK;
+#pragma unroll
+    for (int i = 0; i < A_PER; ++i) {
+      const int k = k0 + a_kc[i];
+      const bool kin = k < p.K;
+      uint4 v;
+      if constexpr (AMODE == 1) {
+        const int kk = min(k, p.K - 8);
+        const f32x4 lo = *reinterpret_cast<const f32x4*>(a32_row[i] + kk), hi = *reinterpret_cast<const f32x4*>(a32_row[i] + kk + 4);
+        op16x8 o;
+#pragma unroll
+        for (int e = 0; e < 4; ++e) {
+          o[e] = f2op(lo[e]);
+          o[4 + e] = f2op(hi[e]);
+        }
+        v = __builtin_bit_cast(uint4, o);
+      } else if (cshift >= 3) {
+        bool in;
+        const op16* src = tap_at(i, k >> cshift, k & ((1 << cshift) - 1), in);
+        v = *reinterpret_cast<const uint4*>(src);
+        if (!in) v = make_uint4(0, 0, 0, 0);
+      } else {
+        bool in0, in1;
+        const op16* s0 = tap_at(i, k >> 2, 0, in0);
+        const op16* s1 = tap_at(i, (k >> 2) + 1, 0, in1);
+        const uint2 v0 = *reinterpret_cast<const uint2*>(s0), v1 = *reinterpret_cast<const uint2*>(s1);
+        v = make_uint4(in0 ? v0.x : 0u, in0 ? v0.y : 0u, in1 ? v1.x : 0u, in1 ? v1.y : 0u);
+      }
+      ra[i] = (a_in[i] && kin) ? v : make_uint4(0, 0, 0, 0);
+    }
+#pragma unroll
+    for (int i = 0; i < W_PER; ++i) {
+      const int k = k0 + w_kc[i];
+      const bool kin = k < p.K;
+      const uint4 v = *reinterpret_cast<const uint4*>(w_row[i] + min(k, p.K - 8));
+      rw[i] = (w_in[i] && kin) ? v : make_uint4(0, 0, 0, 0);
+    }
+  };
+  auto lstore = [&](int buf) {
+#pragma unroll
+    for (int i = 0; i < A_PER; ++i) {
+      const int c = tid + i * NT;
+      if (c < A_CHUNKS)
+        *reinterpret_cast<uint4*>(As + (buf * BM + (c >> 2)) * GEMM_LDS_STRIDE + (c & 3) * 8) = ra[i];
+    }
+#pragma unroll
+    for (int i = 0; i < W_PER; ++i) {
+      const int c = tid + i * NT;
+      if (c < W_CHUNKS)
+        *reinterpret_cast<uint4*>(Ws + (buf * BN + (c >> 2)) * GEMM_LDS_STRIDE + (c & 3) * 8) = rw[i];
+    }
+  };
+
+  gload(0);
+  lstore(0);
+  __syncthreads();
+  int cur = 0;
+  for (int kt = 0; kt < nk; ++kt) {
+    if (kt + 1 < nk) gload(kt + 1);
+#pragma unroll
+    for (int ks = 0; ks < 2; ++ks) {
+      op16x8 af[FM], bfr[FN];
+#pragma unroll
+      for (int i = 0; i < FM; ++i)
+        af[i] = *reinterpret_cast<const op16x8*>(As + (cur * BM + wm * TM + i * 32 + r) * GEMM_LDS_STRIDE + ks * 16 + h * 8);
+#pragma unroll
+      for (int j = 0; j < FN; ++j)
+        bfr[j] = *reinterpret_cast<const op16x8*>(Ws + (cur * BN + wn * TN + j * 32 + r) * GEMM_LDS_STRIDE + ks * 16 + h * 8);
+#pragma unroll
+      for (int i = 0; i < FM; ++i)
+#pragma unroll
+        for (int j = 0; j < FN; ++j) acc[i][j] = MSAM2_MFMA_32x32x16(af[i], bfr[j], acc[i][j], 0, 0, 0);
+    }
+    if (kt + 1 < nk) lstore(cur ^ 1);
+    __syncthreads();
+    cur ^= 1;
+  }
+  __syncthreads();
+  static_assert(WM * WN * 32 * (TN + 4) * 4 <= 2 * (BM + BN) * GEMM_LDS_STRIDE * 2, "epilogue scratch must fit the operand LDS");
+  gemm_epilogue<FM, FN>(p, acc, reinterpret_cast<float*>(lds) + wave * 32 * (TN + 4), m0 + wm * TM, n0 + wn * TN, lane);
+}
+
+template <int AMODE>
+static int gemm_aload_launch(GemmParams& p, int cH, int cW, int cshift, hipStream_t s, const char* what) {
+  p.colscale = nullptr; p.res = nullptr; p.ldr = 0; p.res_mod = 0; p.act = 0; p.res_is_16bit = 0;
+  p.rope_cos = nullptr; p.rope_sin = nullptr; p.rope_cols = 0; p.rope_D = 0; p.rope_period = 1; p.rope_n = 0; p.rope_npos = 1;
+  p.pool_H = 0; p.pool_W = 0; p.Q2 = nullptr; p.ldq = 0; p.poolq_cols = 0; p.A2 = nullptr; p.add_cols = 0; p.store_nt = 0; p.ksplit_tiles = 0;
+  if (p.N <= 32)
+    hipLaunchKernelGGL((gemm_aload_kernel<128, 32, 4, 1, AMODE>), dim3(cdiv(p.N, 32), cdiv(p.M, 128)), dim3(256), 0, s, p, cH, cW, cshift);
+  else if (p.N <= 64 || (p.N % 128 != 0 && p.N % 64 == 0 && p.N < 512))
+    hipLaunchKernelGGL((gemm_aload_kernel<128, 64, 2, 2, AMODE>), dim3(cdiv(p.N, 64), cdiv(p.M, 128)), dim3(256), 0, s, p, cH, cW, cshift);
+  else
+    hipLaunchKernelGGL((gemm_aload_kernel<128, 128, 2, 2, AMODE>), dim3(cdiv(p.N, 128), cdiv(p.M, 128)), dim3(256), 0, s, p, cH, cW, cshift);
+  return msam2_check_launch(what);
+}
+
+extern "C" int msam2_gemm_f32a(const float* A, int64_t lda, const void* W, int64_t ldw, const float* bias, void* C, int64_t ldc, int out_is_16bit,
+                               int64_t M, int64_t N, int64_t K, void* stream) {
+  MSAM2_REQUIRE(A && W && C, "gemm_f32a: null operand");
+  MSAM2_REQUIRE(M > 32 && N > 0 && K > 0 && M < (1ll << 31) && N < (1ll << 31), "gemm_f32a: bad problem M=%lld N=%lld K=%lld (M > 32)", (long long)M, (long long)N, (long long)K);
+  MSAM2_REQUIRE(K % 8 == 0 && lda % 4 == 0 && ldw % 8 == 0 && lda >= K, "gemm_f32a: K, ldw multiples of 8, lda of 4");
+  MSAM2_REQUIRE(((uintptr_t)A & 15) == 0 && ((uintptr_t)W & 15) == 0, "gemm_f32a: A and W must be 16-byte aligned");
+  GemmParams p;
+  p.A = nullptr; p.A32 = A; p.W = (const op16*)W; p.bias = bias; p.C = C; p.lda = lda; p.ldw = ldw; p.ldc = ldc;
+  p.M = (int)M; p.N = (int)N; p.K = (int)K; p.out_is_16bit = out_is_16bit;
+  return gemm_aload_launch<1>(p, 0, 0, 0, (hipStream_t)stream, "gemm_f32a");
+}
+
+extern "C" int msam2_gemm_conv3x3s2(const void* x, const void* Wp, int64_t ldw, const float* bias, float* C, int64_t ldc, int64_t B, int64_t H,
+                                    int64_t W, int64_t Cin, int64_t N, int64_t K, void* stream) {
+  MSAM2_REQUIRE(x && Wp && C, "gemm_conv3x3s2: null operand");
+  MSAM2_REQUIRE(B > 0 && H > 0 && W > 0 && H % 2 == 0 && W % 2 == 0 && N > 0, "gemm_conv3x3s2: bad map %lld x %lld x %lld", (long long)B, (long long)H, (long long)W);
+  int cshift = 0;
+  while ((1ll << cshift) < Cin) ++cshift;
+  MSAM2_REQUIRE(Cin >= 4 && (1ll << cshift) == Cin, "gemm_conv3x3s2: the channel count must be a power of two >= 4 (got %lld)", (long long)Cin);
+  MSAM2_REQUIRE(K >= 9 * Cin && K % 8 == 0 && K < 9 * Cin + 8 && ldw % 8 == 0 && ldw >= K, "gemm_conv3x3s2: K = 9 C rounded up to 8");
+  const int64_t M = B * (H / 2) * (W / 2);
+  MSAM2_REQUIRE(M < (1ll << 31) && B * H * W * Cin < (1ll << 31), "gemm_conv3x3s2: map too large");
+  MSAM2_REQUIRE(M > 32, "gemm_conv3x3s2: %lld output pixels: 33 or more (fewer: msam2_im2col3x3s2 + msam2_gemm)", (long long)M);
+  MSAM2_REQUIRE(((uintptr_t)x & (Cin >= 8 ? 15 : 7)) == 0 && ((uintptr_t)Wp & 15) == 0, "gemm_conv3x3s2: x and Wp alignment");
+  GemmParams p;
+  p.A = (const op16*)x; p.A32 = nullptr; p.W = (const op16*)Wp; p.bias = bias; p.C = C; p.lda = 0; p.ldw = ldw; p.ldc = ldc;
+  p.M = (int)M; p.N = (int)N; p.K = (int)K; p.out_is_16bit = 0;
+  return gemm_aload_launch<2>(p, (int)H, (int)W, cshift, (hipStream_t)stream, "gemm_conv3x3s2");
+}
+
 __global__ __launch_bounds__(256, 2) void gemm_nt_kernel(GemmParams p) {
   constexpr int BM = 128, BN = 128, BK = 64, A_BYTES = BM * BK * 2, STAGE_BYTES = A_BYTES + BK * BN * 2;
   __shared__ __attribute__((aligned(1024))) unsigned char lds[2 * STAGE_BYTES];
diff --git a/medical-sam2_amd/modeling/memory.py b/medical-sam2_amd/modeling/memory.py
--- a/medical-sam2_amd/modeling/memory.py
+++ b/medical-sam2_amd/modeling/memory.py
@@ -234,8 +234,10 @@
         assert not self.training or self.dropout_value == 0.0, \
             "train-mode dropout runs through MemoryAttention.forward / training.* (backward.memory_attention_forward_saved), not a bare layer"
         B, L, C = tgt.shape
-        mem_k = ops.add_cast(memory, pos, 1.0, OP16)
-        mem_v = ops.add_cast(memory, None, 1.0, OP16)
+        if pos is not None:
+            mem_k, mem_v = ops.add_cast_pair(memory, pos, 1.0, OP16)
+        else:
+            mem_k = mem_v = ops.add_cast(memory, None, 1.0, OP16)
         x = ops.add_cast(tgt, None, 1.0, F32).reshape(B * L, C)
         return self.run(x, mem_k, mem_v, B, L, num_k_exclude_rope).view(B, L, C)
 
@@ -311,8 +313,7 @@
         use_pos = self.pos_enc_at_input and curr_pos is not None
         x = ops.add_cast(curr.transpose(0, 1), curr_pos.transpose(0, 1) if use_pos else None, 0.1, F32).reshape(B * L, C)
         mem_bf = memory.transpose(0, 1)
-        mem_k = ops.add_cast(mem_bf, memory_pos.transpose(0, 1), 1.0, OP16)
-        mem_v = ops.add_cast(mem_bf, None, 1.0, OP16)
+        mem_k, mem_v = ops.add_cast_pair(mem_bf, memory_pos.transpose(0, 1), 1.0, OP16)
         kk_all = self._project_all_keys(mem_k, B, L, num_obj_ptr_tokens)
         for i, layer in enumerate(self.layers):
             x = layer.run(x, mem_k, mem_v, B, L, num_obj_ptr_tokens, key_count, None if kk_all is None else kk_all[:, :, i])
@@ -350,14 +351,19 @@
         side = S // 2
         for j in range(1, 4):
             conv, ln = enc[3 * j], enc[3 * j + 1]
-            cols = ops.im2col3x3s2(h, n, side, side)
-
-            def pack(c=conv, ld=cols.shape[1]):
+            cin, cout = conv.weight.shape[1], conv.weight.shape[0]
+            implicit = cout <= 64 and cin >= 4 and cin & (cin - 1) == 0
+            ld = (9 * cin + 7) // 8 * 8
+
+            def pack(c=conv, ld=ld):
                 w = c.weight.detach().permute(0, 2, 3, 1).reshape(c.weight.shape[0], -1)
                 out = torch.zeros(w.shape[0], ld, dtype=OP16, device=w.device)
                 out[:, : w.shape[1]] = w.to(OP16)
                 return out
-            g = ops.gemm(cols, wc.get(f"cw{j}", [conv.weight], pack), f(f"cb{j}", conv.bias), out_dtype=F32)
+            if implicit:
+                g = ops.gemm_conv3x3s2(h, n, side, side, wc.get(f"cw{j}", [conv.weight], pack), f(f"cb{j}", conv.bias))
+            else:
+                g = ops.gemm(ops.im2col3x3s2(h, n, side, side), wc.get(f"cw{j}", [conv.weight], pack), f(f"cb{j}", conv.bias), out_dtype=F32)
             h = ops.layernorm(g, f(f"lw{j}", ln.weight), f(f"lb{j}", ln.bias), ln.eps, act=ops.ACT_GELU)
             side //= 2
         return ops.gemm(h, w_bf16(wc, "pw", enc[12].weight), f("pb", enc[12].bias), out_dtype=F32)
@@ -434,7 +440,10 @@
         x = self.fuser.run(x, n, H, W)
         if isinstance(self.out_proj, nn.Identity):
             return x
-        return ops.gemm(to_bf16(x), w_bf16(wc, "ow", self.out_proj.weight), v_f32(wc, "ob", self.out_proj.bias), out_dtype=F32)
+        w, b = w_bf16(wc, "ow", self.out_proj.weight), v_f32(wc, "ob", self.out_proj.bias)
+        if x.dtype == F32 and w.shape[0] <= 64 and x.shape[0] > 32:
+            return ops.gemm_f32a(x, w, b, out_dtype=F32)
+        return ops.gemm(to_bf16(x), w, b, out_dtype=F32)
 
     def forward(self, pix_feat: torch.Tensor, masks: torch.Tensor, skip_mask_sigmoid: bool = False):
         n, C, H, W = pix_feat.shape
diff --git a/medical-sam2_amd/modeling/sam_heads.py b/medical-sam2_amd/modeling/sam_heads.py
--- a/medical-sam2_amd/modeling/sam_heads.py
+++ b/medical-sam2_amd/modeling/sam_heads.py
@@ -217,10 +217,9 @@
         self.norm_final_attn = nn.LayerNorm(embedding_dim)
         self._wc = WeightCache()
 
-    def run(self, keys, key_pe, tokens, B, T, L):
+    def run(self, keys, key_pe, tokens, B, T, L, keys16=None):
         C = tokens.shape[1]
         queries, qpe = tokens, tokens
-        keys16 = None
         for layer in self.layers:
             queries, keys, keys16 = layer.run(queries, keys, qpe, key_pe, B, T, L, keys16)
         if keys16 is None:
@@ -288,14 +287,15 @@
         return ops.gemm(tokens_bf16, w_bf16(self._wc, f"cs{which}w", c.weight), v_f32(self._wc, f"cs{which}b", c.bias), out_dtype=out_dtype)
 
     def predict_masks_tokens(self, src_tokens: torch.Tensor, pe_tokens: torch.Tensor, sparse: torch.Tensor, feat_s0: torch.Tensor,
-                             feat_s1: torch.Tensor, B: int, h: int, w: int, shared_skips: bool = False):
+                             feat_s1: torch.Tensor, B: int, h: int, w: int, shared_skips: bool = False,
+                             src_tokens16: Optional[torch.Tensor] = None):
         wc = self._wc
         C = self.transformer_dim
         out_tok = wc.get("otok", [self.obj_score_token.weight, self.iou_token.weight, self.mask_tokens.weight],
                          lambda: torch.cat([self.obj_score_token.weight, self.iou_token.weight, self.mask_tokens.weight], 0).detach().float())
         T = out_tok.shape[0] + sparse.shape[1]
         tokens = torch.cat([out_tok.unsqueeze(0).expand(B, -1, -1), sparse], 1)
-        hs, keys = self.transformer.run(src_tokens, pe_tokens, tokens.view(B * T, C), B, T, h * w)
+        hs, keys = self.transformer.run(src_tokens, pe_tokens, tokens.view(B * T, C), B, T, h * w, src_tokens16)
         hs = hs.view(B, T, C)
         up = self.output_upscaling
         dc1_w = wc.get("dc1", [up[0].weight], lambda: up[0].weight.detach().permute(2, 3, 1, 0).reshape(-1, C).to(OP16).contiguous())
@@ -414,11 +414,11 @@
             d3 = dense[:, :, 0, 0].unsqueeze(1).expand(B, h * w, C)
         else:
             d3 = tokens_of(dense).view(B, h * w, C)
-        src = ops.add_cast(e3, d3, 1.0, F32).view(B * h * w, C)
+        src, src16 = (t.view(B * h * w, C) for t in ops.add_cast_pair(e3, d3, 1.0, F32, second="sum"))
         pe = tokens_of(image_pe.to(F32))[: h * w]
         f0, f1 = high_res_features
         skip = lambda f: tokens_of(f) if (f.dtype == F32 and f.shape[1] in (32, 64)) else to_bf16(tokens_of(f))
-        return self.predict_masks_tokens(src, pe, sparse_prompt_embeddings.to(F32), skip(f0), skip(f1), B, h, w)
+        return self.predict_masks_tokens(src, pe, sparse_prompt_embeddings.to(F32), skip(f0), skip(f1), B, h, w, src_tokens16=src16)
 
     def forward(self, image_embeddings, image_pe, sparse_prompt_embeddings, dense_prompt_embeddings, multimask_output: bool,
                 repeat_image: bool, cell_nums=None, high_res_features: Optional[List[torch.Tensor]] = None):
diff --git a/medical-sam2_amd/ops.py b/medical-sam2_amd/ops.py
--- a/medical-sam2_amd/ops.py
+++ b/medical-sam2_amd/ops.py
@@ -52,6 +52,29 @@
                                 residual.stride(0) if residual is not None else 0,
                                 _is_bf16(residual) if residual is not None else 0, res_mod, _p(out), out.stride(0),
                                 _is_bf16(out), M, N, K, act, _stream()))
+    return out
+
+
+def gemm_f32a(a: torch.Tensor, w: torch.Tensor, bias: Optional[torch.Tensor] = None, *, out_dtype: torch.dtype = OP16) -> torch.Tensor:
+    _req(a.dim() == 2 and w.dim() == 2 and a.shape[1] == w.shape[1], f"gemm shapes {tuple(a.shape)} x {tuple(w.shape)}")
+    _req(a.dtype == F32 and w.dtype == OP16 and a.stride(1) == 1 and w.stride(1) == 1, "gemm_f32a: fp32 a, 16-bit w, both K-contiguous")
+    M, K = a.shape
+    N = w.shape[0]
+    if M <= 32:
+        return gemm(add_cast(a.unsqueeze(0), None, 1.0, OP16)[0], w, bias, out_dtype=out_dtype)
+    out = torch.empty(M, N, dtype=out_dtype, device=a.device)
+    check(lib().msam2_gemm_f32a(_p(a), a.stride(0), _p(w), w.stride(0), _p(bias), _p(out), out.stride(0), _is_bf16(out), M, N, K, _stream()))
+    return out
+
+
+def gemm_conv3x3s2(x: torch.Tensor, B: int, H: int, W: int, w_packed: torch.Tensor, bias: Optional[torch.Tensor] = None) -> torch.Tensor:
+    C = x.shape[1]
+    N, K = w_packed.shape
+    _req(x.dtype == OP16 and x.is_contiguous() and w_packed.dtype == OP16 and w_packed.stride(1) == 1, "gemm_conv3x3s2: 16-bit contiguous operands")
+    if B * (H // 2) * (W // 2) <= 32:
+        return gemm(im2col3x3s2(x, B, H, W), w_packed, bias, out_dtype=F32)
+    out = torch.empty(B * (H // 2) * (W // 2), N, dtype=F32, device=x.device)
+    check(lib().msam2_gemm_conv3x3s2(_p(x), _p(w_packed), w_packed.stride(0), _p(bias), _p(out), out.stride(0), B, H, W, C, N, K, _stream()))
     return out
 
 
@@ -338,6 +361,25 @@
     check(lib().msam2_dropout(_p(x), _is_bf16(x), x.stride(0), _p(residual), residual.stride(0) if residual is not None else 0, _p(y), _is_bf16(y),
                               y.stride(0), rows, cols, float(p), int(seed) & (2 ** 64 - 1), int(offset) & (2 ** 64 - 1), _p(seed_dev), _stream()))
     return y
+
+
+def add_cast_pair(a: torch.Tensor, b: torch.Tensor, alpha: float = 1.0, out_dtype: torch.dtype = OP16, second: str = "a"):
+    _req(second in ("a", "sum"), "add_cast_pair: second is 'a' or 'sum'")
+    _req(a.dim() == 3 and (a.stride(2) == 1 or a.shape[2] == 1), "add_cast: a must be [D0,D1,C] with contiguous C")
+    D0, D1, C = a.shape
+    b = b.expand(D0, D1, C)
+    _req(b.stride(2) == 1 or C == 1, "add_cast: b must have contiguous C")
+    esz = lambda t: t.element_size()
+    ok = C % 4 == 0 and D0 * D1 * C // 4 < 2 ** 31 and all(
+        t.data_ptr() % (4 * esz(t)) == 0 and t.stride(0) % 4 == 0 and t.stride(1) % 4 == 0 for t in (a, b))
+    if not ok:
+        first = add_cast(a, b, alpha, out_dtype)
+        return first, add_cast(first if second == "sum" else a, None, 1.0, OP16)
+    out = torch.empty(D0, D1, C, dtype=out_dtype, device=a.device)
+    out2 = torch.empty(D0, D1, C, dtype=OP16, device=a.device)
+    check(lib().msam2_add_cast_pair(_p(a), _is_bf16(a), a.stride(0), a.stride(1), _p(b), _is_bf16(b), b.stride(0), b.stride(1), alpha,
+                                    _p(out), _is_bf16(out), _p(out2), 1 if second == "sum" else 0, D0, D1, C, _stream()))
+    return out, out2
 
 
 def add_cast_into(out: torch.Tensor, a: torch.Tensor, b: Optional[torch.Tensor] = None, alpha: float = 1.0) -> torch.Tensor:
```
